# JuliaImageRecon/RegularizedLeastSquares.jl

Measured on AMD Instinct MI355X. Metric: CGNR iterations/sec @4096x2048 CF32; achieved HBM GB/s vs roofline, higher is better.
Workload: dtype c64 (ComplexF32 storage and arithmetic; scalar reductions accumulated in f64); 1 GPU; CGNR matrix-free normal operator, dense column-major ComplexF32 4096x2048, lambda=0, relTol=0, back-to-back solves of 32 iterations (BASELINE configs[1] shape, headline metric run of SURVEY 8d); M=4096, N=2048, problems_per_gpu=1, init_inside_region=True

## Files before the change

### regularizedleastsquares.jl_amd/csrc/api.hip

```cpp
#include "rls_common.hpp"

#include <cstdlib>
#include <map>
#include <mutex>
#include <set>
#include <vector>

namespace {
std::mutex g_mem_mutex;
std::map<const rls_ctx*, uint64_t> g_live_ctx;
uint64_t g_next_ctx_id = 1;
thread_local rls_ctx* tl_alloc_ctx = nullptr;

std::map<int, hipMemPool_t> g_pools;
hipMemPool_t device_pool(int device) {
  static std::mutex m;
  std::lock_guard<std::mutex> lk(m);
  auto it = g_pools.find(device);
  if (it != g_pools.end()) return it->second;
  hipMemPool_t pool = nullptr;
  const char* env = getenv("RLS_ALLOC");
  if (!(env && !strcmp(env, "sync"))) {
    int supported = 0;
    if (hipDeviceGetAttribute(&supported, hipDeviceAttributeMemoryPoolsSupported, device) == hipSuccess && supported) {
// ... 69 lines not shown
      __hip_atomic_store(A.dst[k] + i, A.src[k][i], __ATOMIC_RELAXED, __HIP_MEMORY_SCOPE_SYSTEM);
  rls_system_stores_done();
  if (threadIdx.x == 0) __hip_atomic_store(seq_h, seq, __ATOMIC_RELAXED, __HIP_MEMORY_SCOPE_SYSTEM);
}

int32_t rls_fetch_add(rls_ctx* ctx, const void* src_d, void* dst_pinned, size_t bytes) {
  if (!ctx->tune.status_mailbox || (bytes & 3) || ctx->nfq >= RLS_FETCH_MAX) {
    RLS_HIP(ctx, hipMemcpyAsync(dst_pinned, src_d, bytes, hipMemcpyDeviceToHost, ctx->stream));
    return 0;
  }
  ctx->fq[ctx->nfq++] = {src_d, dst_pinned, (unsigned)(bytes / 4)};
  return 0;
}

int32_t rls_fetch_wait(rls_ctx* ctx) {
  if (ctx->nfq == 0) {
    RLS_HIP(ctx, rls_stream_wait(ctx->stream));
    return 0;
  }
  fetch_args A;
  A.count = ctx->nfq;
  for (int k = 0; k < RLS_FETCH_MAX; ++k) {
    A.src[k] = k < ctx->nfq ? reinterpret_cast<const unsigned*>(ctx->fq[k].src) : nullptr;
    A.dst[k] = k < ctx->nfq ? reinterpret_cast<unsigned*>(ctx->fq[k].dst) : nullptr;
    A.n[k] = k < ctx->nfq ? ctx->fq[k].dwords : 0u;
  }
  ctx->nfq = 0;
  const unsigned seq = ++ctx->mb_seq;
  hipLaunchKernelGGL(mailbox_publish_kernel, dim3(1), dim3(64), 0, ctx->stream, A, ctx->mb_h, seq);
  RLS_HIP(ctx, hipGetLastError());
  return rls_mailbox_wait(ctx, seq);
}

rls_mailbox_slot rls_mailbox_arm(rls_ctx* ctx, void* dst_pinned) {
  rls_mailbox_slot mb;
  if (ctx->tune.status_mailbox < 2) return mb;
  mb.dst = dst_pinned;
  mb.seq_h = ctx->mb_h;
  mb.seq = ++ctx->mb_seq;
  return mb;
}

int32_t rls_mailbox_wait(rls_ctx* ctx, unsigned seq) {
  volatile unsigned* p = ctx->mb_h;
  const auto t0 = std::chrono::steady_clock::now();
  for (unsigned n = 0;; ++n) {
    if (*p == seq) {
      std::atomic_thread_fence(std::memory_order_acquire);
      return 0;
    }
    rls_cpu_relax();
    if ((n & 1023) == 1023 && std::chrono::steady_clock::now() - t0 > std::chrono::milliseconds(250)) break;
  }
  RLS_HIP(ctx, hipStreamSynchronize(ctx->stream));
  std::atomic_thread_fence(std::memory_order_acquire);
  return *p == seq ? 0 : rls_fail(ctx, RLS_E_STATE, "status mailbox: the publishing kernel did not run");
}

rls_alloc_scope::rls_alloc_scope(rls_ctx* ctx) : prev(tl_alloc_ctx) { tl_alloc_ctx = ctx; }
rls_alloc_scope::~rls_alloc_scope() { tl_alloc_ctx = prev; }
hipError_t rls_scoped_malloc(void** p, size_t bytes) { return rls_dev_alloc(tl_alloc_ctx, p, bytes); }
hipError_t rls_scoped_free(void* p) { return rls_dev_free(tl_alloc_ctx, p); }

static int32_t ctx_setup(rls_ctx* ctx) {
  RLS_HIP(ctx, hipEventCreate(&ctx->ev0));
  RLS_HIP(ctx, hipEventCreate(&ctx->ev1));
  RLS_HIP(ctx, hipMalloc((void**)&ctx->red_d, sizeof(double) * RLS_RED_SLOTS));
  RLS_HIP(ctx, hipMalloc((void**)&ctx->res_d, sizeof(float) * RLS_RES_FLOATS));
  RLS_HIP(ctx, hipHostMalloc((void**)&ctx->res_h, sizeof(float) * RLS_RES_FLOATS, hipHostMallocDefault));
  RLS_HIP(ctx, hipHostMalloc((void**)&ctx->mb_h, 64, hipHostMallocPortable | hipHostMallocMapped | hipHostMallocCoherent));
  ctx->mb_h[0] = 0;
  return 0;
}

static int32_t ctx_create_impl(int32_t device, void* stream, bool borrow, rls_ctx** out) {
  if (!out) return RLS_E_INVALID;
  *out = nullptr;
  int ndev = 0;
  hipError_t e = hipGetDeviceCount(&ndev);
  if (e != hipSuccess) return (int32_t)e;
  if (device < 0 || device >= ndev) return RLS_E_INVALID;
  e = hipSetDevice(device);
  if (e != hipSuccess) return (int32_t)e;
  rls_ctx* ctx = new rls_ctx();
  ctx->device = device;
  ctx->pools = device_pools_ok(device);
  if (borrow) {
    ctx->stream = (hipStream_t)stream;
    ctx->own_stream = false;
    ctx->tune.resident_server = 0;
  } else {
    e = hipStreamCreateWithFlags(&ctx->stream, hipStreamNonBlocking);
    if (e != hipSuccess) {
      delete ctx;
      return (int32_t)e;
    }
    ctx->own_stream = true;
  }
  int32_t st = ctx_setup(ctx);
  if (st != 0) {
    rls_ctx_destroy(ctx);
    return st;
  }
  {
    std::lock_guard<std::mutex> lk(g_mem_mutex);
    ctx->id = g_next_ctx_id++;
    g_live_ctx[ctx] = ctx->id;
  }
  *out = ctx;
  return 0;
}

extern "C" {

int32_t rls_abi_version(void) { return RLS_ABI_VERSION; }

int32_t rls_device_count(int32_t* out) {
  if (!out) return RLS_E_INVALID;
  int n = 0;
  hipError_t e = hipGetDeviceCount(&n);
  *out = (e == hipSuccess) ? n : 0;
  return (int32_t)e;
}

int32_t rls_ctx_create(int32_t device, rls_ctx** out) { return ctx_create_impl(device, nullptr, false, out); }
int32_t rls_ctx_create_on_stream(int32_t device, void* hip_stream, rls_ctx** out) {
  return ctx_create_impl(device, hip_stream, true, out);
}

int32_t rls_ctx_destroy(rls_ctx* ctx) {
  RLS_CHECK_CTX(ctx);
  {
    std::lock_guard<std::mutex> lk(g_mem_mutex);
    g_live_ctx.erase(ctx);
  }
  rls_enter(ctx);
  if (ctx->stream) rls_stream_wait(ctx->stream);
  rls_resident_forget(ctx->device, ctx->stream);
  if (ctx->ev0) hipEventDestroy(ctx->ev0);
  if (ctx->ev1) hipEventDestroy(ctx->ev1);
  if (ctx->red_d) hipFree(ctx->red_d);
  if (ctx->res_d) hipFree(ctx->res_d);
  if (ctx->res_h) hipHostFree(ctx->res_h);
  if (ctx->mb_h) hipHostFree(ctx->mb_h);
  if (ctx->own_stream && ctx->stream) hipStreamDestroy(ctx->stream);
  delete ctx;
  return 0;
}

int32_t rls_ctx_sync(rls_ctx* ctx) {
  RLS_CHECK_CTX(ctx);
  RLS_HIP(ctx, rls_enter(ctx));
  RLS_HIP(ctx, rls_stream_wait(ctx->stream));
  return 0;
}

void* rls_ctx_stream(rls_ctx* ctx) { return ctx ? (void*)ctx->stream : nullptr; }
const char* rls_last_error_string(rls_ctx* ctx) { return ctx ? ctx->err : "null context"; }

int32_t rls_tune_set(rls_ctx* ctx, const char* key, int32_t value) {
  RLS_CHECK_CTX(ctx);
  if (!key) return RLS_E_INVALID;
  if (ctx->server) rls_server_stop(ctx);
  ++ctx->tune_epoch;
  if (!strcmp(key, "gemvn_g")) ctx->tune.gemvn_g = value;
  else if (!strcmp(key, "gemvn_waves")) ctx->tune.gemvn_waves = value;
  else if (!strcmp(key, "gemvt_cols")) ctx->tune.gemvt_cols = value;
  else if (!strcmp(key, "gemvt_reverse")) ctx->tune.gemvt_reverse = value;
  else if (!strcmp(key, "graph_chunk")) ctx->tune.graph_chunk = value;
  else if (!strcmp(key, "use_graph")) ctx->tune.use_graph = value;
  else if (!strcmp(key, "fuse_level")) ctx->tune.fuse_level = value;
  else if (!strcmp(key, "fused_normal")) ctx->tune.fused_normal = value;
  else if (!strcmp(key, "cgnr_pipeline")) ctx->tune.cgnr_pipeline = value;
  else if (!strcmp(key, "batched_mfma")) ctx->tune.batched_mfma = value;
  else if (!strcmp(key, "gram_pipeline")) ctx->tune.gram_pipeline = value;
  else if (!strcmp(key, "pipe_hint_mode")) ctx->tune.pipe_hint_mode = value;
  else if (!strcmp(key, "resident")) {
    ctx->tune.resident = value;
    ctx->resident_failures = 0;
  }
  else if (!strcmp(key, "status_mailbox")) ctx->tune.status_mailbox = value;
  else if (!strcmp(key, "small")) ctx->tune.small = value;
  else if (!strcmp(key, "resident_server")) ctx->tune.resident_server = value;
  else if (!strcmp(key, "resident_ahead")) ctx->tune.resident_ahead = value ? 1 : 0;
  else if (!strcmp(key, "resident_l2_rows")) ctx->tune.resident_l2_rows = value;
  else if (!strcmp(key, "fista_defer")) ctx->tune.fista_defer = value;
  else if (!strcmp(key, "resident_server_idle_us")) {
    ctx->tune.resident_server_idle_us = value < 1 ? 1 : (value > 10000 ? 10000 : value);
  }
  else if (!strcmp(key, "resident_spin")) ctx->tune.resident_spin = value;
  else if (!strcmp(key, "resident_preclear")) ctx->tune.resident_preclear = value;
  else if (!strcmp(key, "skinny_t_waves")) ctx->tune.skinny_t_waves = value;
  else if (!strcmp(key, "skinny_v_waves")) ctx->tune.skinny_v_waves = value;
  else if (!strcmp(key, "skinny_v_splits")) ctx->tune.skinny_v_splits = value;
  else if (!strcmp(key, "kaczmarz_nt")) ctx->tune.kaczmarz_nt = value;
  else if (!strcmp(key, "skinny_t_u")) ctx->tune.skinny_t_u = value;
  else if (!strcmp(key, "skinny_v_u")) ctx->tune.skinny_v_u = value;
  else if (!strcmp(key, "skinny_half")) ctx->tune.skinny_half = value;
  else if (!strcmp(key, "skinny_t_roll")) ctx->tune.skinny_t_roll = value;
  else if (!strcmp(key, "skinny_v_roll")) ctx->tune.skinny_v_roll = value;
  else if (!strcmp(key, "skinny_g_roll")) ctx->tune.skinny_g_roll = value;
  else if (!strcmp(key, "gram_lds_kib")) ctx->tune.gram_lds = value * 1024;
  else if (!strcmp(key, "slab_g")) ctx->tune.slab_g = value;
  else if (!strcmp(key, "slab_wv")) {
    if (value != 0 && value != 8) return rls_fail(ctx, RLS_E_INVALID, "tune_set: slab_wv: only 8-wave slabs exist");
  }
  else if (!strcmp(key, "tv_fused_max_n")) ctx->tune.tv_fused_max_n = value;
  else if (!strcmp(key, "tv_fused_2d")) ctx->tune.tv_fused_2d = value;
  else if (!strcmp(key, "slab_order")) ctx->tune.slab_order = value;
  else if (!strcmp(key, "red_threads")) ctx->tune.red_threads = value;
  else if (!strcmp(key, "slab_multi")) ctx->tune.slab_multi = value ? 1 : 0;
  else if (!strcmp(key, "resident_barrier")) ctx->tune.resident_barrier = value == 1 ? 1 : 2;
  else return rls_fail(ctx, RLS_E_INVALID, "tune_set: unknown key");
  return 0;
}

int32_t rls_malloc(rls_ctx* ctx, size_t bytes, void** out) {
  RLS_CHECK_CTX(ctx);
  if (!out) return rls_fail(ctx, RLS_E_INVALID, "malloc: null out");
  *out = nullptr;
  if (bytes == 0) return 0;
  RLS_HIP(ctx, rls_enter(ctx));
  RLS_HIP(ctx, rls_dev_alloc(ctx, out, bytes));
  return 0;
}

int32_t rls_free(rls_ctx* ctx, void* p) {
  if (!p) return 0;
  if (!ctx_alive_by_address(ctx)) {
    const hipError_t e = hipFree(p);
    return e == hipSuccess ? 0 : (int32_t)e;
  }
  if (ctx->pools && ctx->server) {
    RLS_HIP(ctx, hipSetDevice(ctx->device));
    RLS_HIP(ctx, rls_dev_free(ctx, p));
    return 0;
  }
  RLS_HIP(ctx, rls_enter(ctx));
  if (!ctx->pools) RLS_HIP(ctx, rls_stream_wait(ctx->stream));
  RLS_HIP(ctx, rls_dev_free(ctx, p));
  return 0;
}

int32_t rls_memcpy_h2d(rls_ctx* ctx, void* dst, const void* src_h, size_t bytes) {
  RLS_CHECK_CTX(ctx);
  if (bytes == 0) return 0;
  if (!dst || !src_h) return rls_fail(ctx, RLS_E_INVALID, "memcpy_h2d: null pointer");
  RLS_HIP(ctx, rls_enter(ctx));
  RLS_HIP(ctx, hipMemcpyAsync(dst, src_h, bytes, hipMemcpyHostToDevice, ctx->stream));
  RLS_HIP(ctx, rls_stream_wait(ctx->stream));
  return 0;
}

int32_t rls_memcpy_d2h(rls_ctx* ctx, void* dst_h, const void* src, size_t bytes) {
  RLS_CHECK_CTX(ctx);
  if (bytes == 0) return 0;
  if (!dst_h || !src) return rls_fail(ctx, RLS_E_INVALID, "memcpy_d2h: null pointer");
  RLS_HIP(ctx, rls_enter(ctx));
  RLS_HIP(ctx, hipMemcpyAsync(dst_h, src, bytes, hipMemcpyDeviceToHost, ctx->stream));
  RLS_HIP(ctx, rls_stream_wait(ctx->stream));
  return 0;
}

int32_t rls_memcpy_d2d(rls_ctx* ctx, void* dst, const void* src, size_t bytes) {
  RLS_CHECK_CTX(ctx);
  if (bytes == 0) return 0;
  if (!dst || !src) return rls_fail(ctx, RLS_E_INVALID, "memcpy_d2d: null pointer");
  RLS_HIP(ctx, rls_enter(ctx));
  RLS_HIP(ctx, hipMemcpyAsync(dst, src, bytes, hipMemcpyDeviceToDevice, ctx->stream));
  return 0;
}

int32_t rls_timer_start(rls_ctx* ctx) {
  RLS_CHECK_CTX(ctx);
  RLS_HIP(ctx, rls_enter(ctx));
  RLS_HIP(ctx, hipEventRecord(ctx->ev0, ctx->stream));
  return 0;
}

int32_t rls_timer_stop_ms(rls_ctx* ctx, float* ms_out) {
  RLS_CHECK_CTX(ctx);
  if (!ms_out) return rls_fail(ctx, RLS_E_INVALID, "timer_stop: null out");
  RLS_HIP(ctx, rls_enter(ctx));
  RLS_HIP(ctx, hipEventRecord(ctx->ev1, ctx->stream));
  RLS_HIP(ctx, rls_event_wait(ctx->ev1));
  RLS_HIP(ctx, hipEventElapsedTime(ms_out, ctx->ev0, ctx->ev1));
  return 0;
}

int32_t rls_gemv(rls_ctx* ctx, int32_t dtype, int32_t op, int64_t M, int64_t N, float alpha_re, float alpha_im,
                 const void* A, int64_t lda, const void* x, float beta_re, float beta_im, void* y) {
  return rls_launch_gemv(ctx, dtype, op, M, N, alpha_re, alpha_im, A, lda, x, beta_re, beta_im, y, nullptr);
}

}
```

### regularizedleastsquares.jl_amd/csrc/normal.hip

```cpp
#include "rls_common.hpp"
#include "resident_sync.hpp"

#ifdef RLS_STAMPS
__device__ unsigned long long g_stamps[16 * 8];
#define STAMP(slot)                                                                         \
  do {                                                                                      \
    if (threadIdx.x == 0 && (blockIdx.x % 37) == 5 && blockIdx.x / 37 < 8)                  \
      g_stamps[(blockIdx.x / 37) * 16 + (slot)] = __builtin_amdgcn_s_memrealtime();         \
  } while (0)
#define STAMP_R(slot)                                                                    \
  do {                                                                                      \
    if (threadIdx.x == 0 && blockIdx.x == 0) g_stamps[7 * 16 + (slot)] = __builtin_amdgcn_s_memrealtime(); \
  } while (0)
#define STAMP_R_KEEP()                                                                    \
  do {                                                                                      \
    if (threadIdx.x == 0 && blockIdx.x == 5)                                                \
      for (int q = 0; q < 4; ++q) g_stamps[7 * 16 + 4 + q] = g_stamps[7 * 16 + q];          \
  } while (0)
#else
#define STAMP(slot) \
  do {              \
  } while (0)
#define STAMP_R(slot) \
  do {                \
// ... 1776 lines not shown
    constexpr int H = NVAL / 2;
    const bool up = lane & 8;
#pragma unroll
    for (int j = 0; j < H; ++j) {
      const float lo = v[j] + dpp_f(v[j], 0x140), hi = v[H + j] + dpp_f(v[H + j], 0x140);
      v[j] = up ? hi : lo;
    }
    idx += up ? H : 0;
  }
  {
    constexpr int H = NVAL / 4;
    const bool up = lane & 4;
#pragma unroll
    for (int j = 0; j < H; ++j) {
      const float lo = v[j] + dpp_f(v[j], 0x141), hi = v[H + j] + dpp_f(v[H + j], 0x141);
      v[j] = up ? hi : lo;
    }
    idx += up ? H : 0;
  }
  {
    constexpr int H = NVAL / 8;
    const bool up = lane & 2;
#pragma unroll
    for (int j = 0; j < H; ++j) {
      const float lo = v[j] + dpp_f(v[j], 0x4E), hi = v[H + j] + dpp_f(v[H + j], 0x4E);
      v[j] = up ? hi : lo;
    }
    idx += up ? H : 0;
  }
  {
    constexpr int H = NVAL / 16;
    const bool up = lane & 1;
#pragma unroll
    for (int j = 0; j < H; ++j) {
      const float lo = v[j] + dpp_f(v[j], 0xB1), hi = v[H + j] + dpp_f(v[H + j], 0xB1);
      v[j] = up ? hi : lo;
    }
    idx += up ? H : 0;
  }
  float r;
  if constexpr (NVAL == 32) {
    float a = v[0], b = v[1];
    permlane16_swap(a, b);
    r = a + b;
    idx += (lane & 16) ? 1 : 0;
  } else {
    float a = v[0], b = v[0];
    permlane16_swap(a, b);
    r = a + b;
  }
  {
    float a = r, b = r;
    permlane32_swap(a, b);
    r = a + b;
  }
  *idx_out = idx;
  return r;
}

template <typename E, int G, int K, int WV, bool FULL>
__device__ static inline void owner_products(const chunk<E, elem<E>::vec> (&a)[K], const E (&pin)[slab_cfg<E, G, K, WV>::EPT],
                                             float* red, __amdgpu_buffer_rsrc_t slab_rs, int64_t N, bool l2rows = false,
                                             const __amdgpu_buffer_rsrc_t* tt_rs = nullptr) {
  using C = slab_cfg<E, G, K, WV>;
  constexpr int NV = C::NV, EPT = C::EPT, NT = C::NT, RF = owner_cfg<E, G, K, WV>::RF;
  constexpr bool CX = elem<E>::cplx;
  const int tid = threadIdx.x, lane = tid & 63, w = tid >> 6;
  E acc[G * NV];
#pragma unroll
  for (int i = 0; i < G * NV; ++i) acc[i] = elem<E>::zero();
#pragma unroll
  for (int e = 0; e < EPT; ++e) {
    const int q = e / NV, j = e % NV;
#pragma unroll
    for (int i = 0; i < G; ++i)
#pragma unroll
      for (int r = 0; r < NV; ++r) acc[i * NV + r] = elem<E>::fma_pk(a[16 * q + j * G + i].e[r], pin[e], acc[i * NV + r]);
  }
  float v[RF];
#pragma unroll
  for (int i = 0; i < G * NV; ++i) {
    if constexpr (CX) {
      v[2 * i] = elem<E>::re(acc[i]);
      v[2 * i + 1] = elem<E>::im(acc[i]);
    } else {
      v[i] = elem<E>::re(acc[i]);
    }
  }
  int idx;
  const float part = wave_reduce_scatter<RF>(v, lane, &idx);
  if (lane < 32) red[w * RF + idx] = part;
  lds_barrier();
  const float* tw;
  float tsum = 0.f;
  if constexpr (FULL) {
    float* mine = red + (WV + w) * RF;
    if (lane < RF) {
      float sum = red[lane];
#pragma unroll
      for (int ww = 1; ww < WV; ++ww) sum += red[ww * RF + lane];
      mine[lane] = sum;
      tsum = sum;
    }
    __builtin_amdgcn_wave_barrier();
    tw = mine;
  } else {
    if (tid < RF) {
      float sum = red[tid];
#pragma unroll
      for (int ww = 1; ww < WV; ++ww) sum += red[ww * RF + tid];
      red[WV * RF + tid] = sum;
      tsum = sum;
    }
    lds_barrier();
    tw = red + WV * RF;
  }
  if (tt_rs) {
    if (w == 0) {
      const double sq = half_wave_sum((double)tsum * (double)tsum);
      if (lane == 0) {
        typedef unsigned u2 __attribute__((ext_vector_type(2)));
        if (l2rows) __builtin_amdgcn_raw_buffer_store_b64(__builtin_bit_cast(u2, sq), *tt_rs, (uint32_t)blockIdx.x * 8u, 0, 1);
        else __builtin_amdgcn_raw_buffer_store_b64(__builtin_bit_cast(u2, sq), *tt_rs, (uint32_t)blockIdx.x * 8u, 0, 16);
      }
    }
  }
  E tr[G * NV];
#pragma unroll
  for (int i = 0; i < G * NV; ++i) {
    if constexpr (CX) tr[i] = elem<E>::make(tw[2 * i], tw[2 * i + 1]);
    else tr[i] = elem<E>::make(tw[i], 0.f);
  }
#pragma unroll
  for (int q = 0; q < EPT / NV; ++q) {
    chunk<E, NV> out;
#pragma unroll
    for (int j = 0; j < NV; ++j) {
      E sum = elem<E>::zero();
#pragma unroll
      for (int i = 0; i < G; ++i)
#pragma unroll
        for (int r = 0; r < NV; ++r) sum = elem<E>::fmac_pk(a[16 * q + j * G + i].e[r], tr[i * NV + r], sum);
      out.e[j] = sum;
    }
    const int o = q * NT * NV + tid * NV;
    if (FULL || o < N) {
      const uint32_t off = (uint32_t)blockIdx.x * (uint32_t)(N * sizeof(E)) + (uint32_t)(o * sizeof(E));
      if (l2rows) __builtin_amdgcn_raw_buffer_store_b128(__builtin_bit_cast(u4, out), slab_rs, off, 0, 1);
      else __builtin_amdgcn_raw_buffer_store_b128(__builtin_bit_cast(u4, out), slab_rs, off, 0, 16);
    }
  }
}

__device__ static inline unsigned resident_xcc_id() {
  unsigned v;
  asm volatile("s_getreg_b32 %0, hwreg(HW_REG_XCC_ID)" : "=s"(v));
  return v & 0xfu;
}
__device__ static inline void resident_report_placement(resident_sync* sync) {
  if (threadIdx.x == 0 && resident_xcc_id() != (blockIdx.x % RES_GROUPS))
    __hip_atomic_store(&sync->gcnt[1], 1u, __ATOMIC_RELAXED, __HIP_MEMORY_SCOPE_AGENT);
}
__device__ static inline bool resident_rows_at_l2(resident_sync* sync) {
  return uni((int)__hip_atomic_load(&sync->gcnt[1], __ATOMIC_RELAXED, __HIP_MEMORY_SCOPE_AGENT)) == 0;
}

typedef unsigned u2v __attribute__((ext_vector_type(2)));
__device__ static inline double sc1_load_f64(__amdgpu_buffer_rsrc_t r, uint32_t byte_off) {
  return __builtin_bit_cast(double, __builtin_amdgcn_raw_buffer_load_b64(r, byte_off, 0, 16));
}
template <typename E, int G, int K, int WV, int EXCH, bool FULL, bool DPPSUM = true, bool SCAL = false, typename PC, typename PUB>
__device__ static inline bool resident_allreduce(resident_lds<E, G, K, WV>& R, resident_sync* sync,
                                                 __amdgpu_buffer_rsrc_t slab_rs, E* v, int nwg, int64_t N, unsigned& epoch,
                                                 unsigned& xchg, unsigned spin_limit,
                                                 E (&vv)[slab_cfg<E, G, K, WV>::EPT], PC&& per_column, PUB&& publish,
                                                 const __amdgpu_buffer_rsrc_t* d_rs = nullptr, double* tt = nullptr) {
  using C = slab_cfg<E, G, K, WV>;
  constexpr int NV = C::NV, EPT = C::EPT, NT = C::NT;
  const int tid = threadIdx.x;
  if constexpr (EXCH == 1) {
    if (!grid_arrive_wait(sync->cnt, ++epoch, (unsigned)nwg, spin_limit, &R.flag)) return false;
    STAMP(11);
    if constexpr (SCAL) {
      if ((tid >> 6) == WV - 1) {
        const int lane = tid & 63;
        double s = 0.0;
        for (int row = lane; row < nwg; row += 64) s += sc1_load_f64(*d_rs, (uint32_t)row * 8u);
        s = wave_sum(s);
        if (lane == 0) R.tt = s;
      }
    }
    resident_reduce_chunks<E, G, K, WV, FULL>(R, slab_rs, v, nwg, N, per_column);
    publish();
    asm volatile("s_waitcnt vmcnt(0)" ::: "memory");
    __syncthreads();
    STAMP(12);
    if (!grid_arrive_wait(sync->cnt, ++epoch, (unsigned)nwg, spin_limit, &R.flag)) return false;
    STAMP(13);
    const __amdgpu_buffer_rsrc_t v_rs = sc1_rsrc(v);
#pragma unroll
    for (int q = 0; q < EPT / NV; ++q) {
      const int o = q * NT * NV + tid * NV;
      const bool ok = FULL || o < N;
      const chunk<E, NV> c = __builtin_bit_cast(chunk<E, NV>, sc1_load16(v_rs, (uint32_t)((ok ? o : 0) * sizeof(E))));
#pragma unroll
      for (int j = 0; j < NV; ++j) vv[q * NV + j] = ok ? c.e[j] : elem<E>::zero();
    }
    if constexpr (SCAL) *tt = R.tt;
    return true;
  } else {
    const unsigned per = (unsigned)nwg / RES_GROUPS, grp = blockIdx.x % RES_GROUPS, mem = blockIdx.x / RES_GROUPS;
    const uint32_t rowb = (uint32_t)(N * sizeof(E));
    const unsigned q = (rowb / 16u) / per;
    const unsigned lq = (unsigned)__builtin_ctz(q), nrg = (unsigned)NT >> lq;
    const unsigned par = xchg & 1u;
    ++xchg;
    char* xpart = reinterpret_cast<char*>(sync) + sizeof(resident_sync) + (size_t)par * RES_GROUPS * rowb;
    const __amdgpu_buffer_rsrc_t xp_rs = sc1_rsrc(xpart);
    if (!group_arrive_wait(sync->gcnt + grp * 32, per * xchg, spin_limit, &R.flag)) return false;
    STAMP(11);
    const uint32_t gs_off = (2u - par) * RES_GROUPS * rowb + par * (RES_GROUPS * 8u);
    if constexpr (SCAL) {
      if (mem == 0u && tid < 64) {
        double s = (unsigned)tid < per ? sc1_load_f64(*d_rs, (grp + RES_GROUPS * (unsigned)tid) * 8u) : 0.0;
        s = half_wave_sum(s);
        if (tid == 0) __builtin_amdgcn_raw_buffer_store_b64(__builtin_bit_cast(u2v, s), xp_rs, gs_off + grp * 8u, 0, 16);
      }
    }
    if (DPPSUM && nrg == 16u && q == 32u && per == 32u) {
      const unsigned lane = (unsigned)tid & 63u, rg = lane & 15u, piece = 4u * ((unsigned)tid >> 6) + (lane >> 4);
      const uint32_t col = (mem * 32u + piece) * 16u;
      const f4 ta = sc1_load16(slab_rs, (grp + RES_GROUPS * rg) * rowb + col);
      const f4 tb = sc1_load16(slab_rs, (grp + RES_GROUPS * (rg + 16u)) * rowb + col);
      f4 acc = ta + tb;
#pragma unroll
      for (int c = 0; c < 4; ++c) {
        float v = acc[c];
        v += dpp_f(v, 0xB1);
        v += dpp_f(v, 0x4E);
        v += dpp_f(v, 0x141);
        v += dpp_f(v, 0x140);
        acc[c] = v;
      }
      if (rg == 0u) __builtin_amdgcn_raw_buffer_store_b128(__builtin_bit_cast(u4, acc), xp_rs, grp * rowb + (mem * 32u + piece) * 16u, 0, 16);
      asm volatile("s_waitcnt vmcnt(0)" ::: "memory");
      __syncthreads();
    } else {
      const unsigned piece = (unsigned)tid & (q - 1u), rg = (unsigned)tid >> lq;
      const uint32_t col = (mem * q + piece) * 16u;
      f4 acc = {0.f, 0.f, 0.f, 0.f};
      for (unsigned row = rg; row < per; row += 2u * nrg) {
        const unsigned rb = row + nrg;
        const f4 ta = sc1_load16(slab_rs, (grp + RES_GROUPS * row) * rowb + col);
        const f4 tb = sc1_load16(slab_rs, (grp + RES_GROUPS * (rb < per ? rb : row)) * rowb + col);
        acc += ta;
        if (rb < per) acc += tb;
      }
      f4* ex = reinterpret_cast<f4*>(&R.L.xg[0][0]);
      ex[tid] = acc;
      __syncthreads();
      if ((unsigned)tid < q) {
        f4 sum = ex[tid];
        for (unsigned g = 1; g < nrg; ++g) sum += ex[(g << lq) + tid];
        __builtin_amdgcn_raw_buffer_store_b128(__builtin_bit_cast(u4, sum), xp_rs, grp * rowb + (mem * q + (unsigned)tid) * 16u, 0, 16);
      }
      asm volatile("s_waitcnt vmcnt(0)" ::: "memory");
      if (q > 64u) __syncthreads();
    }
    STAMP(12);
    if (!grid_arrive_wait(sync->cnt, ++epoch, (unsigned)nwg, spin_limit, &R.flag)) return false;
    STAMP(13);
    if constexpr (SCAL) {
      double s = sc1_load_f64(xp_rs, gs_off + ((unsigned)tid & 7u) * 8u);
      s += dpp_d(s, 0xB1);
      s += dpp_d(s, 0x4E);
      s += dpp_d(s, 0x141);
      *tt = s;
    }
#pragma unroll
    for (int qq = 0; qq < EPT / NV; ++qq) {
      const int o = qq * NT * NV + tid * NV;
      const bool ok = FULL || o < N;
      const uint32_t off = (uint32_t)((ok ? o : 0) * sizeof(E));
      f4 t[RES_GROUPS];
#pragma unroll
      for (int g = 0; g < RES_GROUPS; ++g) t[g] = sc1_load16(xp_rs, (uint32_t)g * rowb + off);
      f4 sum = t[0];
#pragma unroll
      for (int g = 1; g < RES_GROUPS; ++g) sum += t[g];
      const chunk<E, NV> c = __builtin_bit_cast(chunk<E, NV>, sum);
#pragma unroll
      for (int j = 0; j < NV; ++j) vv[qq * NV + j] = ok ? c.e[j] : elem<E>::zero();
    }
    return true;
  }
}

template <typename E, int G, int K, int WV, int BAR, bool FULL, bool SPEC = false>
__global__ __launch_bounds__(WV * 64) void cgnr_resident_kernel(const E* __restrict__ A, int64_t lda, E* x, E* xw, E* r, E* p,
                                                                 E* v, E* slab, double* dout, cgnr_scalars* sc,
                                                                 resident_sync* sync, int64_t Mc, int64_t N, int pair,
                                                                 int n_steps, unsigned spin_limit, rls_cg_start St) {
  using C = slab_cfg<E, G, K, WV>;
  constexpr int NV = C::NV, EPT = C::EPT, NT = C::NT;
  static_assert(EPT % NV == 0, "16-byte ownership layout");
  extern __shared__ __attribute__((aligned(16))) char smem_raw[];
  resident_lds<E, G, K, WV>& R = *reinterpret_cast<resident_lds<E, G, K, WV>*>(smem_raw);
  slab_lds<E, G, K, WV>& L = R.L;
  const int tid = threadIdx.x;
  const int nwg = gridDim.x;
  STAMP(0);
  if (St.enabled && St.skip && *St.skip) {
    if (blockIdx.x == 0 && tid == 0) {
      cgnr_scalars Z = *sc;
      Z.iteration = 0;
      Z.max_iter = St.maxiter;
      Z.pending = 0;
      Z.cur = 0;
      Z.fresh = 0;
      Z.done = 1;
      *sc = Z;
      sync->completed = 1u;
    }
    return;
  }
  cgnr_scalars S = *sc;
  E pv[EPT], rv[EPT], xv[EPT];
  if constexpr (FULL) {
    load_owned_wide<E, EPT, NT>(pv, p, tid);
    load_owned_wide<E, EPT, NT>(rv, r, tid);
    load_owned_wide<E, EPT, NT>(xv, x, tid);
  } else {
    load_owned_wide_masked<E, EPT, NT>(pv, p, tid, N);
    load_owned_wide_masked<E, EPT, NT>(rv, r, tid, N);
    load_owned_wide_masked<E, EPT, NT>(xv, x, tid, N);
  }
  asm volatile("s_waitcnt vmcnt(0)" ::: "memory");
  __builtin_amdgcn_sched_barrier(0);
  chunk<E, NV> a[K];
  slab_load<E, G, K, WV, FULL>(a, A, lda, Mc, N, pair);
  __builtin_amdgcn_sched_barrier(0);
  if (!St.enabled && (S.done || n_steps <= 0)) return;
  constexpr bool OWN = owner_cfg<E, G, K, WV>::ok;
  if constexpr (OWN) owner_transpose<E, G, K, WV, FULL>(a, smem_raw, Mc, N, pair);
  STAMP(1);
  const __amdgpu_buffer_rsrc_t slab_rs = sc1_rsrc(slab), d_rs = sc1_rsrc(dout);
  unsigned epoch = 0, xchg = 0;
  bool alive = true;
  constexpr bool L2ROWS = BAR == 2 && OWN;
  bool l2rows = false, placed = !L2ROWS;
  if constexpr (L2ROWS) resident_report_placement(sync);
  if (St.enabled) {
    if constexpr (OWN) {
      owner_products<E, G, K, WV, FULL>(a, xv, R.ored, slab_rs, N);
    } else {
#pragma unroll
      for (int e = 0; e < EPT; ++e) L.xs[(int)own_index<E, EPT, NT, true>(tid, e)] = xv[e];
      slab_finish<E, G, K, WV, FULL, true>(a, L, slab, Mc, N, pair);
    }
    asm volatile("s_waitcnt vmcnt(0)" ::: "memory");
    __syncthreads();
    E cv[EPT];
    if (!resident_allreduce<E, G, K, WV, BAR, FULL>(R, sync, slab_rs, v, nwg, N, epoch, xchg, spin_limit, cv, [](int, E) {}, []() {})) {
      resident_give_up(sync, St.enabled ? St.poison : nullptr);
      return;
    }
    if (!placed) {
      l2rows = resident_rows_at_l2(sync);
      placed = true;
    }
    double rr = 0.0;
#pragma unroll
    for (int q = 0; q < EPT / NV; ++q) {
      const int o = q * NT * NV + tid * NV;
      const bool ok = FULL || o < N;
      const int oc = ok ? o : 0;
      chunk<E, NV> cc;
#pragma unroll
      for (int j = 0; j < NV; ++j) cc.e[j] = cv[q * NV + j];
      chunk<E, NV> bi;
      if (St.beta_y) {
        bi = load_chunk<E, NV>(reinterpret_cast<const E*>(St.beta_y) + oc);
        const chunk<E, NV> zc = load_chunk<E, NV>(reinterpret_cast<const E*>(St.z) + oc);
#pragma unroll
        for (int j = 0; j < NV; ++j) bi.e[j] = elem<E>::add(bi.e[j], elem<E>::scale(St.rho_admm, zc.e[j]));
        const chunk<E, NV> uc = load_chunk<E, NV>(reinterpret_cast<const E*>(St.u) + oc);
#pragma unroll
        for (int j = 0; j < NV; ++j) bi.e[j] = elem<E>::add(bi.e[j], elem<E>::scale(-St.rho_admm, uc.e[j]));
        if (blockIdx.x == 0 && ok) {
          chunk<E, NV> xc;
#pragma unroll
          for (int j = 0; j < NV; ++j) xc.e[j] = xv[q * NV + j];
          *reinterpret_cast<f4*>(reinterpret_cast<E*>(St.beta) + o) = __builtin_bit_cast(f4, bi);
          *reinterpret_cast<f4*>(reinterpret_cast<E*>(St.xold) + o) = __builtin_bit_cast(f4, xc);
        }
      } else {
        bi = load_chunk<E, NV>(reinterpret_cast<const E*>(St.b) + oc);
      }
#pragma unroll
      for (int j = 0; j < NV; ++j) {
        const E ci = elem<E>::add(cc.e[j], elem<E>::scale(St.rho, xv[q * NV + j]));
        E ri = elem<E>::sub(bi.e[j], ci);
        if (!ok) ri = elem<E>::zero();
        rv[q * NV + j] = ri;
        pv[q * NV + j] = ri;
        rr += (double)elem<E>::re(ri) * (double)elem<E>::re(ri) + (double)elem<E>::im(ri) * (double)elem<E>::im(ri);
      }
    }
    rr = block_sum_n<NT / 64>(rr, L.red);
    S.rr = rr;
    S.z0 = sqrt(rr);
    S.zeta = 0.0;
    S.alpha_re = S.alpha_im = S.beta_re = S.beta_im = 0.0;
    S.lambda = St.rho;
    S.rel_tol = St.reltol;
    S.iteration = 0;
    S.max_iter = St.maxiter;
    S.pending = 0;
    S.cur = 0;
    S.fresh = 0;
    S.done = (St.maxiter <= 0) || (rr == 0.0) || (1.0f <= St.reltol);
    if (S.done) n_steps = 0;
  }
  auto store_owned = [&](E* dst, const E (&src)[EPT]) {
#pragma unroll
    for (int q = 0; q < EPT / NV; ++q) {
      chunk<E, NV> c;
#pragma unroll
      for (int j = 0; j < NV; ++j) c.e[j] = src[q * NV + j];
      const int64_t o = (int64_t)q * (NT * NV) + (int64_t)tid * NV;
      if (FULL || o < N) *reinterpret_cast<f4*>(dst + o) = __builtin_bit_cast(f4, c);
    }
  };
  const __amdgpu_buffer_rsrc_t xw_rs = sc1_rsrc(xw);
  auto load_owned_sc1 = [&](E (&dst)[EPT], const E*) {
#pragma unroll
    for (int q = 0; q < EPT / NV; ++q) {
      const int o = q * NT * NV + tid * NV;
      const bool ok = FULL || o < N;
      const chunk<E, NV> c = __builtin_bit_cast(chunk<E, NV>, sc1_load16(xw_rs, (uint32_t)((ok ? o : 0) * sizeof(E))));
#pragma unroll
      for (int j = 0; j < NV; ++j) dst[q * NV + j] = ok ? c.e[j] : elem<E>::zero();
    }
  };
  if (blockIdx.x == 0) store_owned(xw, xv);
  rls_mailbox_slot srv_mb = St.srv_mb;
  unsigned srv_seq = St.srv_seq0;
  int credit = 0;
  bool ahead = false;
  STAMP(2);
  for (;;) {
  for (int it = SPEC ? credit : 0; it < n_steps; ++it) {
    if (S.done) break;
    STAMP(8);
#ifdef RLS_STAMPS
    if (it == 1) STAMP(5);
    if (it == 2) STAMP(6);
    if (it == 10) STAMP(7);
#endif
    if constexpr (OWN) {
      owner_products<E, G, K, WV, FULL>(a, pv, R.ored, slab_rs, N, l2rows, &d_rs);
    } else {
#pragma unroll
      for (int e = 0; e < EPT; ++e) L.xs[(int)own_index<E, EPT, NT, true>(tid, e)] = pv[e];
      const double ttw = slab_finish<E, G, K, WV, FULL, true, true>(a, L, slab, Mc, N, pair);
      if (tid == 0) __builtin_amdgcn_raw_buffer_store_b64(__builtin_bit_cast(u2v, ttw), d_rs, (uint32_t)blockIdx.x * 8u, 0, 16);
    }
    STAMP(9);
    double pp = 0.0;
    if (S.lambda > 0.f) {
      if constexpr (!OWN) {
#pragma unroll
        for (int e = 0; e < EPT; ++e) pv[e] = L.xs[(int)own_index<E, EPT, NT, true>(tid, e)];
      }
#pragma unroll
      for (int e = 0; e < EPT; ++e)
        pp += (double)elem<E>::re(pv[e]) * (double)elem<E>::re(pv[e]) + (double)elem<E>::im(pv[e]) * (double)elem<E>::im(pv[e]);
      pp = block_sum_nolead<NT / 64, 0>(pp, L.red);
    }
    asm volatile("s_waitcnt vmcnt(0)" ::: "memory");
    __syncthreads();
    STAMP(10);
    E xq[EPT];
    load_owned_sc1(xq, xw);
    E vv[EPT];
    double tt = 0.0;
    const bool ok_x = resident_allreduce<E, G, K, WV, BAR, FULL, true, true>(R, sync, slab_rs, v, nwg, N, epoch, xchg, spin_limit, vv,
                                                                             [](int, E) {}, []() {}, &d_rs, &tt);
    if (!ok_x) {
      alive = false;
      break;
    }
    if (!placed) {
      l2rows = resident_rows_at_l2(sync);
      placed = true;
    }
    if constexpr (!OWN) {
#pragma unroll
      for (int e = 0; e < EPT; ++e) pv[e] = L.xs[(int)own_index<E, EPT, NT, true>(tid, e)];
    }
    E pn[EPT], rn[EPT];
    float al;
    cgnr_scalars Sn;
#ifdef RLS_STAMPS
    asm volatile("s_waitcnt vmcnt(0)" ::: "memory");
    STAMP(14);
#endif
    const bool done = cg_update_elems_tt<E, EPT, NT, true>(S, tt, pp, pv, rv, vv, N, L.red, pn, rn, al, Sn);
#pragma unroll
    for (int e = 0; e < EPT; ++e) {
      xq[e] = elem<E>::make(fmaf(elem<E>::re(pv[e]), al, elem<E>::re(xq[e])), fmaf(elem<E>::im(pv[e]), al, elem<E>::im(xq[e])));
      rv[e] = rn[e];
      pv[e] = pn[e];
    }
    if (blockIdx.x == 0) {
#pragma unroll
      for (int q = 0; q < EPT / NV; ++q) {
        chunk<E, NV> c;
#pragma unroll
        for (int j = 0; j < NV; ++j) c.e[j] = xq[q * NV + j];
        const int o = q * NT * NV + tid * NV;
        if (FULL || o < N) __builtin_amdgcn_raw_buffer_store_b128(__builtin_bit_cast(u4, c), xw_rs, (uint32_t)(o * sizeof(E)), 0, 0);
      }
    }
    S = Sn;
    RLS_CGNR_UNIFORM(S);
    STAMP(15);
    if (done) break;
  }
  STAMP(3);
  if (!alive) {
    resident_give_up(sync, St.enabled ? St.poison : nullptr);
    if (St.srv_ctl && blockIdx.x == 0 && tid == 0) __hip_atomic_store(St.srv_ctl + 17, 2u, __ATOMIC_RELAXED, __HIP_MEMORY_SCOPE_SYSTEM);
    return;
  }
  if constexpr (SPEC) {
    if (ahead) {
      ahead = false;
      const unsigned cmd = resident_listen(St.srv_ctl, srv_seq, St.srv_idle_us, sync, epoch, (unsigned)nwg, spin_limit, &R.flag, srv_mb, srv_seq - St.srv_seq0 + 1u);
      if (cmd == RLS_SRV_EXIT) return;
      n_steps = (int)cmd;
      credit = 1;
      continue;
    }
  }
  if (blockIdx.x == 0) {
    S.pending = 0;
    S.cur = 0;
    S.fresh = 0;
    if (St.srv_ctl && tid < 64) rls_mailbox_publish(srv_mb, S, tid);
    E xf[EPT];
    load_owned_sc1(xf, xw);
    auto store_buf = [&](E* dst, const E (&src)[EPT]) {
      const __amdgpu_buffer_rsrc_t rs = __builtin_amdgcn_make_buffer_rsrc(dst, 0, 0xffffffff, 0x00020000);
#pragma unroll
      for (int q = 0; q < EPT / NV; ++q) {
        chunk<E, NV> c;
#pragma unroll
        for (int j = 0; j < NV; ++j) c.e[j] = src[q * NV + j];
        const int o = q * NT * NV + tid * NV;
        if (FULL || o < N) __builtin_amdgcn_raw_buffer_store_b128(__builtin_bit_cast(u4, c), rs, (uint32_t)(o * sizeof(E)), 0, 0);
      }
    };
    store_buf(x, xf);
    store_buf(r, rv);
    store_buf(p, pv);
    if (tid == 0) {
      *sc = S;
      sync->completed = 1u;
    }
  }
  if (!St.srv_ctl) break;
  if constexpr (SPEC) {
    credit = 0;
    if (!S.done) {
      ahead = true;
      n_steps = 1;
      continue;
    }
  }
  const unsigned cmd = resident_listen(St.srv_ctl, srv_seq, St.srv_idle_us, sync, epoch, (unsigned)nwg, spin_limit, &R.flag, srv_mb, srv_seq - St.srv_seq0 + 1u);
  if (cmd == RLS_SRV_EXIT) return;
  n_steps = (int)cmd;
  }
}


template <typename E, int K, int BAR, bool FULL, int SRV = 0>
__global__ __launch_bounds__(512) void cgnr_gram_resident_kernel(const E* __restrict__ Gm, int64_t ldg, E* x, E* r, E* p,
                                                                  E* v0, E* v1, double* dots, cgnr_scalars* sc0,
                                                                  cgnr_scalars* sc1, resident_sync* sync, int64_t Mc,
                                                                  int64_t N, int pair, int n_steps, unsigned spin_limit,
                                                                  rls_cg_start St) {
  constexpr int G = 4, WV = 8;
  using C = slab_cfg<E, G, K, WV>;
  constexpr int NV = C::NV, EPT = C::EPT, NT = C::NT;
  __shared__ gram_lds<E, G, K, WV> L;
  __shared__ int flag;
  const int tid = threadIdx.x, lane = tid & 63, w = tid >> 6;
  const int nwg = gridDim.x;
  if (St.enabled && St.skip && *St.skip) {
    if (blockIdx.x == 0 && tid == 0) {
      cgnr_scalars Z = *sc0;
      Z.iteration = 0;
      Z.max_iter = St.maxiter;
      Z.pending = 0;
      Z.cur = 0;
      Z.fresh = 0;
      Z.done = 1;
      *sc0 = Z;
      *sc1 = Z;
      sync->completed = 1u;
    }
    return;
  }
  cgnr_scalars S = *sc0;
  E pv[EPT], rv[EPT], xv[EPT], vv[EPT];
#pragma unroll
  for (int e = 0; e < EPT; ++e) {
    const int64_t i = tid + (int64_t)e * NT;
    const int64_t ic = FULL || i < N ? i : (N - 1);
    pv[e] = p[ic];
    rv[e] = r[ic];
    xv[e] = x[ic];
    vv[e] = elem<E>::zero();
    if (!FULL && i >= N) pv[e] = rv[e] = xv[e] = elem<E>::zero();
  }
  asm volatile("s_waitcnt vmcnt(0)" ::: "memory");
  __builtin_amdgcn_sched_barrier(0);
  chunk<E, NV> a[K];
  slab_load<E, G, K, WV, FULL>(a, Gm, ldg, Mc, N, pair);
  __builtin_amdgcn_sched_barrier(0);
  if (!St.enabled && (S.done || n_steps <= 0)) return;
  const __amdgpu_buffer_rsrc_t d_rs = sc1_rsrc(dots);
  unsigned epoch = 0;
  bool alive = true;
  if (St.enabled) {
#pragma unroll
    for (int e = 0; e < EPT; ++e) L.xs[tid + e * NT] = xv[e];
    gram_rows<E, G, K, WV, FULL>(a, L, Mc, N, pair);
    if (tid < G * NV) {
      const int gg = tid / NV, i = tid % NV;
      E sum = elem<E>::zero();
#pragma unroll
      for (int ww = 0; ww < WV; ++ww) sum = elem<E>::add(sum, L.part[ww][gg][i]);
      const int64_t row = (row_block_of(blockIdx.x, pair) * G + gg) * NV + i;
      if (FULL || row < N) sc1_store_elem<E>(v1 + row, sum);
    }
    asm volatile("s_waitcnt vmcnt(0)" ::: "memory");
    __syncthreads();
    if (!grid_arrive_wait(sync->cnt, ++epoch, (unsigned)nwg, spin_limit, &flag)) {
      resident_give_up(sync, St.enabled ? St.poison : nullptr);
      return;
    }
    const E* bb = reinterpret_cast<const E*>(St.b);
    const E* by = reinterpret_cast<const E*>(St.beta_y);
    const E* zz = reinterpret_cast<const E*>(St.z);
    const E* uu = reinterpret_cast<const E*>(St.u);
    double rr = 0.0;
#pragma unroll
    for (int e = 0; e < EPT; ++e) {
      const int64_t i = tid + (int64_t)e * NT;
      const bool ok = FULL || i < N;
      const int64_t ic = ok ? i : (N - 1);
      const E ci = elem<E>::add(sc1_load_elem<E>(v1 + ic), elem<E>::scale(St.rho, xv[e]));
      E bi;
      if (by) {
        bi = by[ic];
        bi = elem<E>::add(bi, elem<E>::scale(St.rho_admm, zz[ic]));
        bi = elem<E>::add(bi, elem<E>::scale(-St.rho_admm, uu[ic]));
        if (blockIdx.x == 0 && ok) {
          reinterpret_cast<E*>(St.beta)[i] = bi;
          reinterpret_cast<E*>(St.xold)[i] = xv[e];
        }
      } else {
        bi = bb[ic];
      }
      E ri = elem<E>::sub(bi, ci);
      if (!ok) ri = elem<E>::zero();
      rv[e] = ri;
      pv[e] = ri;
      rr += (double)elem<E>::re(ri) * (double)elem<E>::re(ri) + (double)elem<E>::im(ri) * (double)elem<E>::im(ri);
    }
    rr = block_sum_n<NT / 64>(rr, L.red);
    S.rr = rr;
    S.z0 = sqrt(rr);
    S.zeta = 0.0;
    S.alpha_re = S.alpha_im = S.beta_re = S.beta_im = 0.0;
    S.lambda = St.rho;
    S.rel_tol = St.reltol;
    S.iteration = 0;
    S.max_iter = St.maxiter;
    S.pending = 0;
    S.cur = 0;
    S.fresh = 0;
    S.done = (St.maxiter <= 0) || (rr == 0.0) || (1.0f <= St.reltol);
    if (S.done) n_steps = 0;
  }
  rls_mailbox_slot srv_mb = St.srv_mb;
  unsigned srv_seq = St.srv_seq0;
  unsigned itg = 0;
  int credit = 0;
  bool ahead = false;
  for (;;) {
  for (int it = SRV ? credit : 0; it < n_steps; ++it) {
    if (SRV && S.done) break;
    const int q = (int)(itg++ & 1u);
    E* vq = q ? v1 : v0;
#pragma unroll
    for (int e = 0; e < EPT; ++e) L.xs[tid + e * NT] = pv[e];
    gram_rows<E, G, K, WV, FULL>(a, L, Mc, N, pair);
    double dre = 0.0, dim_ = 0.0, pp = 0.0;
    if (tid < G * NV) {
      const int gg = tid / NV, i = tid % NV;
      E sum = elem<E>::zero();
#pragma unroll
      for (int ww = 0; ww < WV; ++ww) sum = elem<E>::add(sum, L.part[ww][gg][i]);
      const int64_t row = (row_block_of(blockIdx.x, pair) * G + gg) * NV + i;
      if (FULL || row < N) {
        sc1_store_elem<E>(vq + row, sum);
        const E pj = L.xs[row];
        dre = (double)elem<E>::re(pj) * (double)elem<E>::re(sum) + (double)elem<E>::im(pj) * (double)elem<E>::im(sum);
        dim_ = (double)elem<E>::re(pj) * (double)elem<E>::im(sum) - (double)elem<E>::im(pj) * (double)elem<E>::re(sum);
        pp = (double)elem<E>::re(pj) * (double)elem<E>::re(pj) + (double)elem<E>::im(pj) * (double)elem<E>::im(pj);
      }
    }
    if (w == 0) {
#pragma unroll
      for (int off = 8; off > 0; off >>= 1) {
        dre += __shfl_xor(dre, off, 64);
        dim_ += __shfl_xor(dim_, off, 64);
        pp += __shfl_xor(pp, off, 64);
      }
      if (lane < 3) {
        const double dv = lane == 0 ? dre : (lane == 1 ? dim_ : pp);
        __hip_atomic_store(reinterpret_cast<unsigned long long*>(dots + (size_t)q * 4 * nwg + 4 * blockIdx.x + lane),
                           __builtin_bit_cast(unsigned long long, dv), __ATOMIC_RELAXED, __HIP_MEMORY_SCOPE_AGENT);
      }
    }
// ... 984 lines not shown
    });
  });
}

template <typename E>
static int32_t fista_iteration_typed(rls_ctx* ctx, const rls_fista_pipe& P) {
  fused_cfg c;
  if (!pick_cfg<E>(ctx->tune, P.N, &c)) return rls_fail(ctx, RLS_E_UNSUPPORTED, "fista pipeline: N too large");
  const int nwg = (int)fused_nwg<E>(ctx->tune, P.M, P.N);
  const int rows = slab_grid(ctx, c.K, nwg);
  RLS_TRY(with_cfg(c, [&](auto S) { return launch_fista_a<E, S.G, S.K, S.WV>(ctx, P, nwg, rows); }));
  hipLaunchKernelGGL(fista_pipe_r_kernel<E>, dim3((unsigned)((P.N + 15) / 16)), dim3(ctx->tune.red_threads), 0, ctx->stream,
                     (const E*)P.slab, rows, P.N, (E*)P.res_raw, P.sc, P.scn);
  return launch_status(ctx);
}

template <typename E>
static int32_t fista_finish_typed(rls_ctx* ctx, const rls_fista_pipe& P) {
  return with_ept(P.N, [&](auto EPT) {
    return rls_launch<fista_pipe_f_kernel<E, EPT>>(ctx, dim3(1), dim3(FIN_THREADS), 0, (E*)P.b0, (E*)P.b1, (const E*)P.x0,
                                                   (E*)P.res, (E*)P.y0, (E*)P.y1, (const E*)P.res_raw, P.sc, P.N, P.mb);
  });
}

template <typename E>
static bool gram_pick(int64_t N, int* K) {
  const int64_t cpr = 8 * (64 / 4);
  for (int k : {8, 16, 32}) {
    if (N <= k * cpr) {
      *K = k;
      return true;
    }
  }
  return false;
}

template <typename E>
static int gram_grid(rls_ctx* ctx, int K, int nwg) {
  return elem<E>::cplx ? slab_grid(ctx, K, nwg) : nwg;
}

template <typename E, int K>
constexpr bool gram_walks() {
  return K == 32 && elem<E>::cplx;
}

template <typename E, int K>
static int32_t launch_gram(rls_ctx* ctx, const rls_gram_pipe& P, int q, int nwg) {
  using C = slab_cfg<E, 4, K, 8>;
  const int64_t Mc = P.N / C::NV;
  const int pair = slab_pairing(4, nwg);
  const int grid = gram_grid<E>(ctx, K, nwg);
  return with_bool(slab_full<E, 4, K, 8>(P.N, P.N, nwg), [&](auto FULL) {
    return with_bool(gram_walks<E, K>() && grid < nwg, [&](auto MULTI) {
      if constexpr (MULTI && !gram_walks<E, K>())
        return not_instantiated(ctx);
      else
        return rls_launch<cgnr_gram_kernel<E, 4, K, 8, FULL, MULTI>>(
            ctx, dim3(MULTI ? grid : nwg), dim3(C::NT), 0, (const E*)P.G, P.ldg, (E*)P.x, (const E*)P.r[q], (const E*)P.p[q],
            (E*)P.r[q ^ 1], (E*)P.p[q ^ 1], (const E*)P.v[q], (E*)P.v[q ^ 1], P.dots + (size_t)q * 4 * nwg,
            P.dots + (size_t)(q ^ 1) * 4 * nwg, MULTI ? grid : nwg, P.sc[q], P.sc[q ^ 1], Mc, P.N, pair, ctx->tune.slab_order, nwg);
    });
  });
}

template <typename E>
static int32_t gram_iteration_typed(rls_ctx* ctx, const rls_gram_pipe& P, int q) {
  int K = 0;
  if (!gram_pick<E>(P.N, &K)) return rls_fail(ctx, RLS_E_UNSUPPORTED, "gram pipeline: N too large");
  const int nwg = rls_gram_pipe_nwg(elem<E>::cplx ? RLS_C32 : RLS_F32, P.N);
  return rls_with<8, 16, 32>(K, [&](auto KC) { return launch_gram<E, KC>(ctx, P, q, nwg); });
}

template <typename E>
static int32_t gram_finish_typed(rls_ctx* ctx, const rls_gram_pipe& P, int q) {
  const int nwg = rls_gram_pipe_nwg(elem<E>::cplx ? RLS_C32 : RLS_F32, P.N);
  int Kp = 0;
  gram_pick<E>(P.N, &Kp);
  const int ndots = gram_grid<E>(ctx, Kp, nwg);
  return with_ept(P.N, [&](auto EPT) {
    return rls_launch<cgnr_gram_f_kernel<E, EPT>>(ctx, dim3(1), dim3(FIN_THREADS), 0, (E*)P.x, (const E*)P.r[q], (const E*)P.p[q],
                                                  (E*)P.r[0], (E*)P.p[0], (const E*)P.v[q], (E*)P.v[0], P.dots + (size_t)q * 4 * nwg,
                                                  ndots, P.sc[q], P.sc[0], P.sc[1], P.N);
  });
}

template <typename E, int K>
static int32_t launch_fista_gram(rls_ctx* ctx, const rls_fista_gram& P, int q, int nwg) {
  using C = slab_cfg<E, 4, K, 8>;
  const int64_t Mc = P.N / C::NV;
  const int pair = slab_pairing(4, nwg);
  const int grid = gram_grid<E>(ctx, K, nwg);
  return with_bool(slab_full<E, 4, K, 8>(P.N, P.N, nwg), [&](auto FULL) {
    return with_bool(P.par_hint >= 0, [&](auto HINT) {
      return with_bool(gram_walks<E, K>() && grid < nwg, [&](auto MULTI) {
        if constexpr (MULTI && !gram_walks<E, K>())
          return not_instantiated(ctx);
        else
          return rls_launch<fista_gram_kernel<E, 4, K, 8, FULL, HINT, MULTI>>(
              ctx, dim3(MULTI ? grid : nwg), dim3(C::NT), 0, (const E*)P.G, P.ldg, (E*)P.b0, (E*)P.b1, (const E*)P.x0, (E*)P.res,
              (E*)P.y0, (E*)P.y1, (const E*)P.rr[q], (E*)P.rr[q ^ 1], P.sc[q], P.sc[q ^ 1], Mc, P.N, pair, P.par_hint, nwg);
      });
    });
  });
}

template <typename E>
static int32_t fista_gram_iteration_typed(rls_ctx* ctx, const rls_fista_gram& P, int q) {
  int K = 0;
  if (!gram_pick<E>(P.N, &K)) return rls_fail(ctx, RLS_E_UNSUPPORTED, "gram pipeline: N too large");
  const int nwg = rls_gram_pipe_nwg(elem<E>::cplx ? RLS_C32 : RLS_F32, P.N);
  return rls_with<8, 16, 32>(K, [&](auto KC) { return launch_fista_gram<E, KC>(ctx, P, q, nwg); });
}

template <typename E>
static int32_t fista_gram_finish_typed(rls_ctx* ctx, const rls_fista_gram& P, int q) {
  return with_ept(P.N, [&](auto EPT) {
    return rls_launch<fista_gram_f_kernel<E, EPT>>(ctx, dim3(1), dim3(FIN_THREADS), 0, (E*)P.b0, (E*)P.b1, (const E*)P.x0,
                                                   (E*)P.res, (E*)P.y0, (E*)P.y1, (const E*)P.rr[q], P.sc[q], P.sc[0], P.sc[1], P.N);
  });
}


template <typename E>
static bool resident_two_level_ok(const rls_tuning& T, int nwg, int64_t N, int nt) {
  if (T.resident_barrier != 2 || nwg % RES_GROUPS != 0) return false;
  const int64_t pieces = N * (int64_t)sizeof(E) / 16, per = nwg / RES_GROUPS;
  if (N * (int64_t)sizeof(E) % 16 != 0 || pieces % per != 0) return false;
  const int64_t q = pieces / per;
  return q >= 1 && q <= nt && (q & (q - 1)) == 0;
}

template <typename E, int G, int K, int WV>
constexpr bool resident_shape() {
  return (K == 32 || K == 16) && WV == 8 && slab_cfg<E, G, K, WV>::EPT % elem<E>::vec == 0 && !(elem<E>::cplx && G == 4);
}
template <typename E, int G, int K, int WV>
constexpr bool pgm_resident_shape() {
  return resident_shape<E, G, K, WV>() && owner_cfg_ok<E, G, K, WV>();
}

static int resident_pairing(int G, int nwg) { return (G == 4 && nwg % 16 == 0) ? 1 : 0; }

template <typename E, int G, int K, int WV>
static int32_t launch_resident(rls_ctx* ctx, const rls_cgnr_pipe& P, double* dout, void* sync, int nwg, int n_steps,
                               unsigned spin_limit, const rls_cg_start& St) {
  if constexpr (!resident_shape<E, G, K, WV>()) {
    return rls_fail(ctx, RLS_E_UNSUPPORTED, "resident CGNR: slab shape not instantiated");
  } else {
    using C = slab_cfg<E, G, K, WV>;
    const int64_t Mc = P.M / C::NV;
    const int pair = resident_pairing(G, nwg);
    constexpr size_t lds = resident_lds_bytes<E, G, K, WV>();
    const bool spec = St.srv_ctl != nullptr && ctx->tune.resident_ahead != 0;
    return with_bool(resident_two_level_ok<E>(ctx->tune, nwg, P.N, C::NT), [&](auto TWO) {
      return with_bool(slab_full<E, G, K, WV>(P.M, P.N, nwg), [&](auto FULL) {
        return with_bool(spec, [&](auto SPEC) {
          return rls_launch<cgnr_resident_kernel<E, G, K, WV, TWO ? 2 : 1, FULL, SPEC>>(
              ctx, dim3(nwg), dim3(C::NT), lds, (const E*)P.A, P.lda, (E*)P.x, (E*)P.r1, (E*)P.r0, (E*)P.p0, (E*)P.v, (E*)P.slab,
              dout, P.sc, (resident_sync*)sync, Mc, P.N, pair, n_steps, spin_limit, St);
        });
      });
    });
  }
}

template <typename E>
static bool resident_ok_typed(const rls_tuning& T, int device, int64_t M, int64_t N, const void* A, int64_t lda) {
  if (!fused_ok<E>(T, M, N, A, lda)) return false;
  fused_cfg c;
  if (!pick_cfg<E>(T, N, &c)) return false;
  return with_cfg(c, [&](auto S) {
    if constexpr (!resident_shape<E, S.G, S.K, S.WV>()) {
      return false;
    } else {
      const int64_t nwg = fused_nwg<E>(T, M, N);
      if (N % elem<E>::vec) return false;
      int cus = 0;
      if (hipDeviceGetAttribute(&cus, hipDeviceAttributeMultiprocessorCount, device) != hipSuccess) return false;
      if (!(nwg <= cus && nwg <= 256 && nwg * N * (int64_t)sizeof(E) < (int64_t)0xffffffffll)) return false;
      return rls_occupancy<cgnr_resident_kernel<E, S.G, S.K, S.WV, 1, false>>(device, S.WV * 64,
                                                                              resident_lds_bytes<E, S.G, S.K, S.WV>()) >= 1;
    }
  });
}

template <typename E>
static int32_t resident_typed(rls_ctx* ctx, const rls_cgnr_pipe& P, double* dout, void* sync, int n_steps,
                              unsigned spin_limit, const rls_cg_start& St) {
  fused_cfg c;
  if (!pick_cfg<E>(ctx->tune, P.N, &c)) return rls_fail(ctx, RLS_E_UNSUPPORTED, "resident CGNR: N too large");
  const int nwg = (int)fused_nwg<E>(ctx->tune, P.M, P.N);
  return with_cfg(c, [&](auto S) {
    return launch_resident<E, S.G, S.K, S.WV>(ctx, P, dout, sync, nwg, n_steps, spin_limit, St);
  });
}

template <typename E, int G, int K, int WV>
static int32_t launch_fista_resident(rls_ctx* ctx, const rls_fista_pipe& P, void* sync, int nwg, int n_steps,
                                     unsigned spin_limit, const rls_srv_args& Sv) {
  if constexpr (!resident_shape<E, G, K, WV>()) {
    return rls_fail(ctx, RLS_E_UNSUPPORTED, "resident FISTA: slab shape not instantiated");
  } else {
    using C = slab_cfg<E, G, K, WV>;
    const int64_t Mc = P.M / C::NV;
    const int pair = resident_pairing(G, nwg);
    constexpr size_t lds = resident_lds_bytes<E, G, K, WV>();
    const bool spec = Sv.ctl != nullptr && ctx->tune.resident_ahead != 0;
    return with_bool(resident_two_level_ok<E>(ctx->tune, nwg, P.N, C::NT), [&](auto TWO) {
      return with_bool(slab_full<E, G, K, WV>(P.M, P.N, nwg), [&](auto FULL) {
        return with_bool(spec, [&](auto SPEC) {
          return rls_launch<fista_resident_kernel<E, G, K, WV, TWO ? 2 : 1, FULL, SPEC>>(
              ctx, dim3(nwg), dim3(C::NT), lds, (const E*)P.A, P.lda, (E*)P.b0, (E*)P.b1, (const E*)P.x0, (E*)P.res, (E*)P.y0,
              (E*)P.y1, (E*)P.res_raw, (E*)P.slab, P.sc, (resident_sync*)sync, Mc, P.N, pair | (ctx->tune.fista_defer ? 0 : 2),
              n_steps, spin_limit, Sv);
        });
      });
    });
  }
}

template <typename E>
static int32_t fista_resident_typed(rls_ctx* ctx, const rls_fista_pipe& P, void* sync, int n_steps, unsigned spin_limit,
                                    const rls_srv_args& Sv) {
  fused_cfg c;
  if (!pick_cfg<E>(ctx->tune, P.N, &c)) return rls_fail(ctx, RLS_E_UNSUPPORTED, "resident FISTA: N too large");
  const int nwg = (int)fused_nwg<E>(ctx->tune, P.M, P.N);
  return with_cfg(c, [&](auto S) {
    return launch_fista_resident<E, S.G, S.K, S.WV>(ctx, P, sync, nwg, n_steps, spin_limit, Sv);
  });
}

static int gram_srv_mode(const rls_ctx* ctx, bool listens) { return !listens ? 0 : ctx->tune.resident_ahead ? 2 : 1; }

template <typename E, int K>
static int32_t launch_gram_resident(rls_ctx* ctx, const rls_gram_pipe& P, void* sync, int nwg, int n_steps,
                                    unsigned spin_limit, const rls_cg_start& St) {
  using C = slab_cfg<E, 4, K, 8>;
  const int64_t Mc = P.N / C::NV;
  const int pair = resident_pairing(4, nwg);
  return with_bool(slab_full<E, 4, K, 8>(P.N, P.N, nwg), [&](auto FULL) {
    return rls_with<0, 1, 2>(gram_srv_mode(ctx, St.srv_ctl != nullptr), [&](auto SRV) {
      if constexpr (K == 32 && SRV != 0)
        return rls_fail(ctx, RLS_E_UNSUPPORTED, "resident Gram CGNR: no listening instantiation for this shape");
      else
        return rls_launch<cgnr_gram_resident_kernel<E, K, 1, FULL, SRV>>(
            ctx, dim3(nwg), dim3(C::NT), 0, (const E*)P.G, P.ldg, (E*)P.x, (E*)P.r[0], (E*)P.p[0], (E*)P.v[0], (E*)P.v[1], P.dots,
            P.sc[0], P.sc[1], (resident_sync*)sync, Mc, P.N, pair, n_steps, spin_limit, St);
    });
  });
}

template <typename E>
static bool gram_resident_ok_typed(int device, int64_t N) {
  int K = 0;
  if (!gram_pick<E>(N, &K)) return false;
  const int nwg = rls_gram_pipe_nwg(elem<E>::cplx ? RLS_C32 : RLS_F32, N);
  int cus = 0;
  if (hipDeviceGetAttribute(&cus, hipDeviceAttributeMultiprocessorCount, device) != hipSuccess) return false;
  if (!(nwg <= cus && nwg <= 256)) return false;
  return rls_with<8, 16, 32>(K, [&](auto KC) {
    if constexpr (elem<E>::cplx && KC == 32)
      return false;
    else
      return rls_occupancy<cgnr_gram_resident_kernel<E, KC, 1, false>>(device, 512, 0) >= 1;
  });
}

template <typename E>
static int32_t gram_resident_typed(rls_ctx* ctx, const rls_gram_pipe& P, void* sync, int n_steps, unsigned spin_limit,
                                   const rls_cg_start& St) {
  int K = 0;
  if (!gram_pick<E>(P.N, &K)) return rls_fail(ctx, RLS_E_UNSUPPORTED, "resident Gram CGNR: N too large");
  const int nwg = rls_gram_pipe_nwg(elem<E>::cplx ? RLS_C32 : RLS_F32, P.N);
  return rls_with<8, 16, 32>(K, [&](auto KC) {
    if constexpr (elem<E>::cplx && KC == 32)
      return rls_fail(ctx, RLS_E_UNSUPPORTED, "resident Gram CGNR: shape not resident");
    else
      return launch_gram_resident<E, KC>(ctx, P, sync, nwg, n_steps, spin_limit, St);
  });
}

template <typename E, int K>
static int32_t launch_fista_gram_resident(rls_ctx* ctx, const rls_fista_gram& P, void* sync, int nwg, int n_steps,
                                          unsigned spin_limit, const rls_srv_args& Sv) {
  using C = slab_cfg<E, 4, K, 8>;
  const int64_t Mc = P.N / C::NV;
  const int pair = resident_pairing(4, nwg);
  return with_bool(slab_full<E, 4, K, 8>(P.N, P.N, nwg), [&](auto FULL) {
    return rls_with<0, 1, 2>(gram_srv_mode(ctx, Sv.ctl != nullptr), [&](auto SRV) {
      if constexpr (K == 32 && SRV != 0)
        return rls_fail(ctx, RLS_E_UNSUPPORTED, "resident Gram FISTA: no listening instantiation for this shape");
      else
        return rls_launch<fista_gram_resident_kernel<E, K, 1, FULL, SRV>>(
            ctx, dim3(nwg), dim3(C::NT), 0, (const E*)P.G, P.ldg, (E*)P.b0, (E*)P.b1, (const E*)P.x0, (E*)P.res, (E*)P.y0,
            (E*)P.y1, (E*)P.rr[0], (E*)P.rr[1], P.sc[0], P.sc[1], (resident_sync*)sync, Mc, P.N, pair, n_steps, spin_limit, Sv);
    });
  });
}

template <typename E>
static int32_t fista_gram_resident_typed(rls_ctx* ctx, const rls_fista_gram& P, void* sync, int n_steps,
                                         unsigned spin_limit, const rls_srv_args& Sv) {
  int K = 0;
  if (!gram_pick<E>(P.N, &K)) return rls_fail(ctx, RLS_E_UNSUPPORTED, "resident Gram FISTA: N too large");
  const int nwg = rls_gram_pipe_nwg(elem<E>::cplx ? RLS_C32 : RLS_F32, P.N);
// ... 14 lines not shown
    using C = slab_cfg<E, G, K, WV>;
    const int64_t Mc = D.M / C::NV;
    const int pair = resident_pairing(G, nwg);
    constexpr size_t lds = resident_lds_bytes<E, G, K, WV>();
    return with_bool(resident_two_level_ok<E>(ctx->tune, nwg, D.N, C::NT), [&](auto TWO) {
      return with_bool(slab_full<E, G, K, WV>(D.M, D.N, nwg), [&](auto FULL) {
        return rls_with<0, 1, 2>(D.kind, [&](auto KIND) {
          return rls_launch<pgm_resident_kernel<E, G, K, WV, TWO ? 2 : 1, FULL, KIND>>(
              ctx, dim3(nwg), dim3(C::NT), lds, (const E*)D.A, D.lda, (E*)D.v0, (E*)D.v1, (E*)D.v2, (E*)D.v3, (E*)D.o0, (E*)D.res,
              (const E*)D.x0, (E*)D.raw, (E*)D.slab, D.st, CF, D.norm_x0, D.rel_tol, D.reg_kind, D.proj_kind, (resident_sync*)sync,
              Mc, D.N, pair | (ctx->tune.fista_defer ? 0 : 2), n_steps, D.first_it, spin_limit);
        });
      });
    });
  }
}

template <typename E>
static int32_t pgm_resident_typed(rls_ctx* ctx, const rls_pgm_desc& D, const rls_pgm_coefs& CF, void* sync, int n_steps,
                                  unsigned spin_limit) {
  fused_cfg c;
  if (!pick_cfg<E>(ctx->tune, D.N, &c)) return rls_fail(ctx, RLS_E_UNSUPPORTED, "resident OptISTA / POGM: N too large");
  const int nwg = (int)fused_nwg<E>(ctx->tune, D.M, D.N);
  return with_cfg(c, [&](auto S) { return launch_pgm_resident<E, S.G, S.K, S.WV>(ctx, D, CF, sync, nwg, n_steps, spin_limit); });
}

template <typename E>
static bool pgm_resident_ok_typed(const rls_tuning& T, int device, int64_t M, int64_t N, const void* A, int64_t lda) {
  if (!resident_ok_typed<E>(T, device, M, N, A, lda)) return false;
  fused_cfg c;
  if (!pick_cfg<E>(T, N, &c)) return false;
  return with_cfg(c, [](auto S) { return pgm_resident_shape<E, S.G, S.K, S.WV>(); });
}
}

int32_t rls_fista_gram_iteration(rls_ctx* ctx, int32_t dtype, const rls_fista_gram& P, int parity) {
  if (dtype == RLS_F32) return fista_gram_iteration_typed<float>(ctx, P, parity & 1);
  return fista_gram_iteration_typed<float2>(ctx, P, parity & 1);
}
int32_t rls_fista_gram_finish(rls_ctx* ctx, int32_t dtype, const rls_fista_gram& P, int parity) {
  if (dtype == RLS_F32) return fista_gram_finish_typed<float>(ctx, P, parity & 1);
  return fista_gram_finish_typed<float2>(ctx, P, parity & 1);
}

int rls_gram_pipe_nwg(int32_t dtype, int64_t N) {
  const int V = dtype == RLS_C32 ? 2 : 4;
  const int64_t Mc = N / V;
  return (int)((Mc + 3) / 4);
}
bool rls_gram_pipe_ok(int32_t dtype, int64_t N, const void* G, int64_t ldg) {
  const int V = dtype == RLS_C32 ? 2 : 4;
  if (!G || N <= 0 || N % V || ldg % V || (reinterpret_cast<uintptr_t>(G) % 16)) return false;
  if (N > 32 * 128 || N > 4 * FIN_THREADS) return false;
  if (rls_gram_pipe_nwg(dtype, N) > 512) return false;
  return 128 * ldg * (int64_t)(dtype == RLS_C32 ? 8 : 4) + (N / V) * 16 < (int64_t)0xffffffffll;
}
int32_t rls_gram_pipe_iteration(rls_ctx* ctx, int32_t dtype, const rls_gram_pipe& P, int parity) {
  if (dtype == RLS_F32) return gram_iteration_typed<float>(ctx, P, parity & 1);
  return gram_iteration_typed<float2>(ctx, P, parity & 1);
}
int32_t rls_gram_pipe_finish(rls_ctx* ctx, int32_t dtype, const rls_gram_pipe& P, int parity) {
  if (dtype == RLS_F32) return gram_finish_typed<float>(ctx, P, parity & 1);
  return gram_finish_typed<float2>(ctx, P, parity & 1);
}

int32_t rls_fista_gram_resident_launch(rls_ctx* ctx, int32_t dtype, const rls_fista_gram& P, void* sync, int n_steps,
                                       unsigned spin_limit, const rls_srv_args& Sv) {
  if (dtype == RLS_F32) return fista_gram_resident_typed<float>(ctx, P, sync, n_steps, spin_limit, Sv);
  return fista_gram_resident_typed<float2>(ctx, P, sync, n_steps, spin_limit, Sv);
}
bool rls_gram_resident_ok(rls_ctx* ctx, int32_t dtype, int64_t N, const void* G, int64_t ldg) {
  if (!rls_gram_pipe_ok(dtype, N, G, ldg)) return false;
  return dtype == RLS_F32 ? gram_resident_ok_typed<float>(ctx->device, N) : gram_resident_ok_typed<float2>(ctx->device, N);
}
bool rls_gram_resident_server_ok(int32_t dtype, int64_t N) {
  int K = 0;
  const bool ok = dtype == RLS_F32 ? gram_pick<float>(N, &K) : gram_pick<float2>(N, &K);
  return ok && K != 32;
}
int32_t rls_gram_resident_launch(rls_ctx* ctx, int32_t dtype, const rls_gram_pipe& P, void* sync, int n_steps,
                                 unsigned spin_limit, const rls_cg_start& St) {
  if (dtype == RLS_F32) return gram_resident_typed<float>(ctx, P, sync, n_steps, spin_limit, St);
  return gram_resident_typed<float2>(ctx, P, sync, n_steps, spin_limit, St);
}


int32_t rls_fista_pipe_iteration(rls_ctx* ctx, int32_t dtype, const rls_fista_pipe& P) {
  if (dtype == RLS_F32) return fista_iteration_typed<float>(ctx, P);
  return fista_iteration_typed<float2>(ctx, P);
}
int32_t rls_fista_pipe_finish(rls_ctx* ctx, int32_t dtype, const rls_fista_pipe& P) {
  if (dtype == RLS_F32) return fista_finish_typed<float>(ctx, P);
  return fista_finish_typed<float2>(ctx, P);
}

#ifdef RLS_STAMPS
extern "C" int32_t rls_debug_stamps(unsigned long long* out_h) {
  return (int32_t)hipMemcpyFromSymbol(out_h, HIP_SYMBOL(g_stamps), sizeof(unsigned long long) * 16 * 8);
}
#endif

int32_t rls_cgnr_pipe_iteration(rls_ctx* ctx, int32_t dtype, const rls_cgnr_pipe& P) {
  if (dtype == RLS_F32) return pipe_iteration_typed<float>(ctx, P);
  return pipe_iteration_typed<float2>(ctx, P);
}
int32_t rls_cgnr_pipe_launch(rls_ctx* ctx, int32_t dtype, const rls_cgnr_pipe& P, int which) {
  if (dtype == RLS_F32) return pipe_iteration_typed<float>(ctx, P, which);
  return pipe_iteration_typed<float2>(ctx, P, which);
}
int32_t rls_cgnr_pipe_finish(rls_ctx* ctx, int32_t dtype, const rls_cgnr_pipe& P) {
  if (dtype == RLS_F32) return pipe_finish_typed<float>(ctx, P);
  return pipe_finish_typed<float2>(ctx, P);
}

size_t rls_normal_fused_workspace(rls_ctx* ctx, int32_t dtype, int64_t M, int64_t N, const void* A, int64_t lda) {
  if (!ctx) return 0;
  if (dtype == RLS_F32) return fused_ok<float>(ctx->tune, M, N, A, lda) ? (size_t)fused_nwg<float>(ctx->tune, M, N) * N * 4 : 0;
  if (dtype == RLS_C32) return fused_ok<float2>(ctx->tune, M, N, A, lda) ? (size_t)fused_nwg<float2>(ctx->tune, M, N) * N * 8 : 0;
  return 0;
}

int32_t rls_launch_normal_fused(rls_ctx* ctx, int32_t dtype, int64_t M, int64_t N, const void* A, int64_t lda,
                                const void* p, void* v, void* slab, const int* skip) {
  RLS_CHECK_CTX(ctx);
  if (!A || !p || !v || !slab) return rls_fail(ctx, RLS_E_INVALID, "normal_fused: null pointer");
  RLS_HIP(ctx, rls_enter(ctx));
  if (dtype == RLS_F32)
    return normal_typed<float>(ctx, M, N, (const float*)A, lda, (const float*)p, (float*)v, (float*)slab, skip);
  return normal_typed<float2>(ctx, M, N, (const float2*)A, lda, (const float2*)p, (float2*)v, (float2*)slab, skip);
}

size_t rls_cgnr_resident_sync_bytes() { return sizeof(resident_sync); }
size_t rls_resident_sync_alloc_bytes(int32_t dtype, int64_t N) {
  return sizeof(resident_sync) + (size_t)2 * RES_GROUPS * (size_t)N * rls_elem_size(dtype) + (size_t)2 * RES_GROUPS * sizeof(double);
}
size_t rls_resident_sync_clear_bytes() { return offsetof(resident_sync, failed); }
size_t rls_resident_sync_flags_offset() { return offsetof(resident_sync, fail); }
size_t rls_resident_sync_placement_offset() { return offsetof(resident_sync, gcnt) + sizeof(unsigned); }
bool rls_cgnr_resident_ok(rls_ctx* ctx, int32_t dtype, int64_t M, int64_t N, const void* A, int64_t lda) {
  if (!ctx) return false;
  if (dtype == RLS_F32) return resident_ok_typed<float>(ctx->tune, ctx->device, M, N, A, lda);
  if (dtype == RLS_C32) return resident_ok_typed<float2>(ctx->tune, ctx->device, M, N, A, lda);
  return false;
}
int rls_cgnr_resident_nwg(rls_ctx* ctx, int32_t dtype, int64_t M, int64_t N) {
  return dtype == RLS_F32 ? (int)fused_nwg<float>(ctx->tune, M, N) : (int)fused_nwg<float2>(ctx->tune, M, N);
}
int32_t rls_cgnr_resident_launch(rls_ctx* ctx, int32_t dtype, const rls_cgnr_pipe& P, double* dout, void* sync,
                                 int n_steps, unsigned spin_limit, const rls_cg_start& St) {
  if (dtype == RLS_F32) return resident_typed<float>(ctx, P, dout, sync, n_steps, spin_limit, St);
  return resident_typed<float2>(ctx, P, dout, sync, n_steps, spin_limit, St);
}

int32_t rls_fista_resident_launch(rls_ctx* ctx, int32_t dtype, const rls_fista_pipe& P, void* sync, int n_steps,
                                  unsigned spin_limit, const rls_srv_args& Sv) {
  if (dtype == RLS_F32) return fista_resident_typed<float>(ctx, P, sync, n_steps, spin_limit, Sv);
  return fista_resident_typed<float2>(ctx, P, sync, n_steps, spin_limit, Sv);
}

bool rls_pgm_resident_ok(rls_ctx* ctx, int32_t dtype, int64_t M, int64_t N, const void* A, int64_t lda) {
  if (!ctx) return false;
  if (dtype == RLS_F32) return pgm_resident_ok_typed<float>(ctx->tune, ctx->device, M, N, A, lda);
  if (dtype == RLS_C32) return pgm_resident_ok_typed<float2>(ctx->tune, ctx->device, M, N, A, lda);
  return false;
}
int32_t rls_pgm_resident_launch(rls_ctx* ctx, int32_t dtype, const rls_pgm_desc& D, const rls_pgm_coefs& C, void* sync,
                                int n_steps, unsigned spin_limit) {
  if (n_steps > RLS_PGM_MAX_IT) return rls_fail(ctx, RLS_E_INVALID, "pgm_resident: more iterations than coefficient slots");
  if (dtype == RLS_F32) return pgm_resident_typed<float>(ctx, D, C, sync, n_steps, spin_limit);
  return pgm_resident_typed<float2>(ctx, D, C, sync, n_steps, spin_limit);
}
```

### regularizedleastsquares.jl_amd/csrc/resident_sync.hpp

```cpp
#pragma once
#include "rls_common.hpp"

typedef unsigned u4 __attribute__((ext_vector_type(4)));
__device__ static inline __amdgpu_buffer_rsrc_t sc1_rsrc(const void* base) {
  return __builtin_amdgcn_make_buffer_rsrc(const_cast<void*>(base), 0, 0xffffffff, 0x00020000);
}
__device__ static inline f4 sc1_load16(__amdgpu_buffer_rsrc_t r, uint32_t byte_off) {
  return __builtin_bit_cast(f4, __builtin_amdgcn_raw_buffer_load_b128(r, byte_off, 0, 16));
}
template <typename E>
__device__ static inline void sc1_store_elem(E* p, E v) {
  if constexpr (sizeof(E) == 8)
    __hip_atomic_store(reinterpret_cast<unsigned long long*>(p), __builtin_bit_cast(unsigned long long, v), __ATOMIC_RELAXED,
                       __HIP_MEMORY_SCOPE_AGENT);
  else
    __hip_atomic_store(reinterpret_cast<unsigned*>(p), __builtin_bit_cast(unsigned, v), __ATOMIC_RELAXED,
                       __HIP_MEMORY_SCOPE_AGENT);
}


template <typename E>
__device__ static inline E sc1_load_elem(const E* p) {
  if constexpr (sizeof(E) == 8)
    return __builtin_bit_cast(E, __hip_atomic_load(reinterpret_cast<const unsigned long long*>(p), __ATOMIC_RELAXED,
                                                   __HIP_MEMORY_SCOPE_AGENT));
  else
    return __builtin_bit_cast(E, __hip_atomic_load(reinterpret_cast<const unsigned*>(p), __ATOMIC_RELAXED,
                                                   __HIP_MEMORY_SCOPE_AGENT));
}


struct resident_sync {
  unsigned cnt[8 * 32];
  unsigned gcnt[8 * 32];
  unsigned fail;
  unsigned completed;
  unsigned failed;
  unsigned srv_n, srv_mb;
  unsigned pad[27];
};
static_assert(sizeof(resident_sync) == (2 * 8 * 32 + 32) * sizeof(unsigned), "resident_sync layout");
constexpr int RES_GROUPS = 8;

__device__ static inline void resident_give_up(resident_sync* sync, int* poison) {
  if (threadIdx.x == 0) {
    __hip_atomic_store(&sync->fail, 1u, __ATOMIC_RELAXED, __HIP_MEMORY_SCOPE_AGENT);
    if (blockIdx.x == 0) {
      __hip_atomic_fetch_add(&sync->failed, 1u, __ATOMIC_RELAXED, __HIP_MEMORY_SCOPE_AGENT);
      if (poison) __hip_atomic_store(poison, 2, __ATOMIC_RELAXED, __HIP_MEMORY_SCOPE_AGENT);
    }
  }
}


#ifndef RLS_POLL_SLEEP
#define RLS_POLL_SLEEP 1
#endif
__device__ static inline bool grid_arrive_wait_t(unsigned* cnt, unsigned epoch, unsigned nwg, unsigned spin_limit, int* lds_flag,
                                                 const int tid) {
  if (tid < 64) {
    int ok = 0;
    const unsigned target = nwg * epoch;
    if (tid == 0) __hip_atomic_fetch_add(cnt + (blockIdx.x & 7) * 32, 1u, __ATOMIC_RELAXED, __HIP_MEMORY_SCOPE_AGENT);
    for (unsigned spins = 0; spins < spin_limit; ++spins) {
      unsigned c = __hip_atomic_load(cnt + (tid & 7) * 32, __ATOMIC_RELAXED, __HIP_MEMORY_SCOPE_AGENT);
      c += (unsigned)__builtin_amdgcn_update_dpp(0, (int)c, 0xB1, 0xF, 0xF, true);
      c += (unsigned)__builtin_amdgcn_update_dpp(0, (int)c, 0x4E, 0xF, 0xF, true);
      c += (unsigned)__builtin_amdgcn_update_dpp(0, (int)c, 0x141, 0xF, 0xF, true);
      if (__builtin_amdgcn_readfirstlane((int)c) >= (int)target) {
        ok = 1;
        break;
      }
      __builtin_amdgcn_s_sleep(RLS_POLL_SLEEP);
    }
    if (tid == 0) *lds_flag = ok;
  }
  __syncthreads();
  return *lds_flag != 0;
}
__device__ static inline bool grid_arrive_wait(unsigned* cnt, unsigned epoch, unsigned nwg, unsigned spin_limit, int* lds_flag) {
  return grid_arrive_wait_t(cnt, epoch, nwg, spin_limit, lds_flag, (int)threadIdx.x);
}
__device__ static inline bool group_arrive_wait(unsigned* word, unsigned target, unsigned spin_limit, int* lds_flag) {
  const int tid = threadIdx.x;
  if (tid < 64) {
    int ok = 0;
    if (tid == 0) __hip_atomic_fetch_add(word, 1u, __ATOMIC_RELAXED, __HIP_MEMORY_SCOPE_AGENT);
    for (unsigned spins = 0; spins < spin_limit; ++spins) {
      const unsigned c = __hip_atomic_load(word, __ATOMIC_RELAXED, __HIP_MEMORY_SCOPE_AGENT);
      if (__builtin_amdgcn_readfirstlane((int)c) >= (int)target) {
        ok = 1;
        break;
      }
      __builtin_amdgcn_s_sleep(RLS_POLL_SLEEP);
    }
    if (tid == 0) *lds_flag = ok;
  }
  __syncthreads();
  return *lds_flag != 0;
}

constexpr unsigned RLS_SRV_MAX_COMMANDS = 2048u;
struct srv_head {
  unsigned seq, n, mbseq, pad;
};
__device__ static inline srv_head srv_read_head(const unsigned* ctl) {
  typedef unsigned u4h __attribute__((ext_vector_type(4)));
  u4h w;
  asm volatile("global_load_dwordx4 %0, %1, off sc0 sc1\n\ts_waitcnt vmcnt(0)" : "=v"(w) : "v"(ctl) : "memory");
  return srv_head{w.x, w.y, w.z, w.w};
}
__device__ static inline unsigned resident_listen(unsigned* ctl, unsigned& srv_seq, unsigned idle_us, resident_sync* sync, unsigned& epoch,
                                                  unsigned nwg, unsigned spin_limit, int* lds_flag, rls_mailbox_slot& mb,
                                                  unsigned served) {
  const int tid = threadIdx.x;
  if (blockIdx.x == 0 && tid == 0) {
    asm volatile("s_waitcnt vmcnt(0)" ::: "memory");
    const unsigned long long t0 = wall_clock64(), idle = (unsigned long long)idle_us * 100ull;
    unsigned n = RLS_SRV_EXIT;
    srv_head hd{srv_seq, 0u, 0u, 0u};
    for (; served < RLS_SRV_MAX_COMMANDS;) {
      hd = srv_read_head(ctl);
      if (hd.seq != srv_seq) break;
      if (wall_clock64() - t0 > idle) {
        __hip_atomic_store(ctl + 16, 1u, __ATOMIC_RELAXED, __HIP_MEMORY_SCOPE_SYSTEM);
        asm volatile("s_waitcnt vmcnt(0)" ::: "memory");
        hd = srv_read_head(ctl);
        if (hd.seq != srv_seq) __hip_atomic_store(ctl + 16, 0u, __ATOMIC_RELAXED, __HIP_MEMORY_SCOPE_SYSTEM);
        break;
      }
      __builtin_amdgcn_s_sleep(8);
    }
    if (hd.seq != srv_seq) n = hd.n;
    __hip_atomic_store(&sync->srv_n, n, __ATOMIC_RELAXED, __HIP_MEMORY_SCOPE_AGENT);
    __hip_atomic_store(&sync->srv_mb, hd.mbseq, __ATOMIC_RELAXED, __HIP_MEMORY_SCOPE_AGENT);
    asm volatile("s_waitcnt vmcnt(0)" ::: "memory");
  }
  __syncthreads();
  if (!grid_arrive_wait(sync->cnt, ++epoch, nwg, spin_limit, lds_flag)) {
    resident_give_up(sync, nullptr);
    if (blockIdx.x == 0 && tid == 0) __hip_atomic_store(ctl + 17, 2u, __ATOMIC_RELAXED, __HIP_MEMORY_SCOPE_SYSTEM);
    return RLS_SRV_EXIT;
  }
  const unsigned cmd = __hip_atomic_load(&sync->srv_n, __ATOMIC_RELAXED, __HIP_MEMORY_SCOPE_AGENT);
  if (cmd == RLS_SRV_EXIT) {
    if (blockIdx.x == 0 && tid == 0) __hip_atomic_store(ctl + 17, 1u, __ATOMIC_RELAXED, __HIP_MEMORY_SCOPE_SYSTEM);
    return RLS_SRV_EXIT;
  }
  mb.seq = __hip_atomic_load(&sync->srv_mb, __ATOMIC_RELAXED, __HIP_MEMORY_SCOPE_AGENT);
  srv_seq += 1;
  return cmd;
}
```

### regularizedleastsquares.jl_amd/csrc/rls_common.hpp

```cpp
#pragma once
#include <hip/hip_runtime.h>

#include <chrono>
#include <mutex>
#include <cstdint>
#include <cstdio>
#include <cstring>
#include <type_traits>

#include "../../include/rls_mi355x.h"

#define RLS_WAVE 64

struct rls_tuning {
  int gemvn_g = 0;
  int gemvn_waves = 0;
  int gemvt_cols = 0;
  int gemvt_reverse = -1;
  int graph_chunk = 16;
  int use_graph = 1;
  int fuse_level = 1;
  int fused_normal = 1;
  int cgnr_pipeline = 1;
  int batched_mfma = 1;
  int gram_pipeline = 1;
  int pipe_hint_mode = 0;
  int resident = 1;
  int resident_preclear = 1;
  int resident_server = 1;
  int resident_server_idle_us = 300;
  int resident_ahead = 1;
  int fista_defer = 1;
  int resident_l2_rows = 1;
  int small = 1;
  int status_mailbox = 2;
  int slab_g = 0;
  int slab_order = 1;
  int resident_barrier = 2;
  int red_threads = 1024;
  int slab_multi = 1;
  int skinny_t_waves = 4, skinny_t_u = 4, skinny_v_waves = 4, skinny_v_u = 1, skinny_v_splits = 0;
  int skinny_t_roll = 8, skinny_v_roll = 2, skinny_g_roll = 8;
  int skinny_half = 1;
  int gram_lds = 96 * 1024;
  int64_t tv_fused_max_n = 2048;
  int tv_fused_2d = 1;
  int kaczmarz_nt = 0;
  int resident_spin = 100000;
};

constexpr int RLS_FETCH_MAX = 24;
struct rls_ctx {
  int device = 0;
  void* server = nullptr;
  uint64_t id = 0;
  hipStream_t stream = nullptr;
  bool own_stream = false;
  hipEvent_t ev0 = nullptr, ev1 = nullptr;
  char err[512] = {0};
  double* red_d = nullptr;
  float* res_d = nullptr;
  float* res_h = nullptr;
  rls_tuning tune;
  uint64_t tune_epoch = 0;
  int cus = 0;
  int resident_failures = 0;
  bool pools = false;
  struct fetch_item {
    const void* src;
    void* dst;
    unsigned dwords;
  } fq[RLS_FETCH_MAX];
  int nfq = 0;
  unsigned* mb_h = nullptr;
  unsigned mb_seq = 0;
};

int32_t rls_fetch_add(rls_ctx* ctx, const void* src_d, void* dst_pinned, size_t bytes);
int32_t rls_fetch_wait(rls_ctx* ctx);
struct rls_mailbox_slot {
  void* dst = nullptr;
  unsigned* seq_h = nullptr;
  unsigned seq = 0;
};
rls_mailbox_slot rls_mailbox_arm(rls_ctx* ctx, void* dst_pinned);
constexpr unsigned RLS_SRV_EXIT = 0xffffffffu;
constexpr unsigned RLS_SRV_AHEAD = 0x80000000u;
struct rls_srv_args {
  unsigned* ctl = nullptr;
  unsigned seq0 = 0, idle_us = 0;
  rls_mailbox_slot mb;
};
int32_t rls_mailbox_wait(rls_ctx* ctx, unsigned seq);
#ifdef __HIPCC__
__device__ static inline void rls_system_stores_done() { asm volatile("s_waitcnt vmcnt(0)" ::: "memory"); }
template <typename S>
__device__ static inline void rls_mailbox_publish(const rls_mailbox_slot& mb, const S& v, int lane) {
  constexpr unsigned ND = sizeof(S) / 4;
  static_assert(sizeof(S) % 4 == 0 && ND <= 64, "status structs are published dword by dword by one wave");
  if (!mb.dst) return;
  const unsigned* src = reinterpret_cast<const unsigned*>(&v);
  unsigned mine = 0;
#pragma unroll
  for (unsigned i = 0; i < ND; ++i) mine = lane == (int)i ? src[i] : mine;
  if (lane < (int)ND) __hip_atomic_store(reinterpret_cast<unsigned*>(mb.dst) + lane, mine, __ATOMIC_RELAXED, __HIP_MEMORY_SCOPE_SYSTEM);
  rls_system_stores_done();
  if (lane == 0) __hip_atomic_store(mb.seq_h, mb.seq, __ATOMIC_RELAXED, __HIP_MEMORY_SCOPE_SYSTEM);
}
#endif

hipError_t rls_dev_alloc(rls_ctx* ctx, void** p, size_t bytes);
hipError_t rls_dev_free(rls_ctx* ctx, void* p);
hipError_t rls_pinned_alloc(void** p, size_t bytes);
void rls_pinned_free(void* p);
void rls_server_stop(rls_ctx* ctx);
static inline hipError_t rls_enter(rls_ctx* ctx) {
  if (ctx->server) rls_server_stop(ctx);
  return hipSetDevice(ctx->device);
}
bool rls_ctx_alive(const rls_ctx* ctx, uint64_t id);
struct rls_alloc_scope {
  rls_ctx* prev;
  explicit rls_alloc_scope(rls_ctx* ctx);
  ~rls_alloc_scope();
};
hipError_t rls_scoped_malloc(void** p, size_t bytes);
hipError_t rls_scoped_free(void* p);

static inline void rls_cpu_relax() {
#if defined(__x86_64__) || defined(__i386__)
  __builtin_ia32_pause();
#elif defined(__aarch64__)
  asm volatile("yield");
#endif
}
template <typename Q, typename B>
static inline hipError_t rls_bounded_spin(Q&& query, B&& block) {
  const auto t0 = std::chrono::steady_clock::now();
  for (unsigned n = 0;; ++n) {
    const hipError_t e = query();
    if (e != hipErrorNotReady) return e;
    rls_cpu_relax();
    if ((n & 63) == 63 && std::chrono::steady_clock::now() - t0 > std::chrono::milliseconds(250)) break;
  }
  return block();
}
static inline hipError_t rls_stream_wait(hipStream_t s) {
  return rls_bounded_spin([s] { return hipStreamQuery(s); }, [s] { return hipStreamSynchronize(s); });
}
static inline hipError_t rls_event_wait(hipEvent_t ev) {
  return rls_bounded_spin([ev] { return hipEventQuery(ev); }, [ev] { return hipEventSynchronize(ev); });
}

void rls_resident_forget(int device, hipStream_t stream);
inline std::mutex& rls_capture_mutex() {
  static std::mutex m;
  return m;
}

#include <atomic>
struct rls_device_once {
  std::atomic<uint64_t> done{0};
  std::mutex mu;
  struct guard {
    rls_device_once* o;
    uint64_t bit;
    bool run;
    bool ok = true;
    guard(rls_device_once* o_, uint64_t bit_, bool run_) : o(o_), bit(bit_), run(run_) {}
    guard(const guard&) = delete;
    guard(guard&& g) : o(g.o), bit(g.bit), run(g.run), ok(g.ok) { g.run = false; }
    ~guard() {
      if (run) {
        if (ok) o->done.fetch_or(bit, std::memory_order_release);
        o->mu.unlock();
      }
    }
    explicit operator bool() const { return run; }
    void failed() { ok = false; }
  };
  guard first(int device) {
    const uint64_t bit = 1ull << (device & 63);
    if (done.load(std::memory_order_acquire) & bit) return guard(this, bit, false);
    mu.lock();
    if (done.load(std::memory_order_acquire) & bit) {
      mu.unlock();
      return guard(this, bit, false);
    }
    return guard(this, bit, true);
  }
};

constexpr int RLS_RED_SLOTS = 4096;
constexpr int RLS_RES_FLOATS = 64;

#define RLS_CHECK_CTX(ctx)            \
  do {                                \
    if (!(ctx)) return RLS_E_INVALID; \
  } while (0)

static inline int32_t rls_fail(rls_ctx* ctx, int32_t code, const char* what) {
  if (ctx) snprintf(ctx->err, sizeof(ctx->err), "%s (code %d)", what, (int)code);
  return code;
}

#define RLS_HIP(ctx, expr)                                                                       \
  do {                                                                                           \
    hipError_t _e = (expr);                                                                      \
    if (_e != hipSuccess) {                                                                      \
      if (ctx)                                                                                   \
        snprintf((ctx)->err, sizeof((ctx)->err), "%s failed: %s (%s:%d)", #expr,                 \
                 hipGetErrorString(_e), __FILE__, __LINE__);                                     \
      return (int32_t)_e;                                                                        \
    }                                                                                            \
  } while (0)

#define RLS_TRY(expr)            \
  do {                           \
    int32_t _s = (expr);         \
    if (_s != 0) return _s;      \
  } while (0)

static inline int32_t launch_status(rls_ctx* ctx) {
  hipError_t e = hipGetLastError();
  if (e != hipSuccess) return rls_fail(ctx, (int32_t)e, hipGetErrorString(e));
  return 0;
}

template <auto Kern>
static inline hipError_t rls_allow_lds(int device, size_t bytes) {
  static rls_device_once once;
  hipError_t e = hipSuccess;
  if (auto g = once.first(device)) {
    e = hipFuncSetAttribute(reinterpret_cast<const void*>(Kern), hipFuncAttributeMaxDynamicSharedMemorySize, (int)bytes);
    if (e != hipSuccess) g.failed();
  }
  return e;
}

template <auto Kern, typename... A>
// ... 353 lines not shown
  } else {
    static_assert(NV == 1, "scalar chunk");
    c.e[0] = *p;
  }
  return c;
}
template <typename E, int NV>
__device__ static inline chunk<E, NV> zero_chunk() {
  chunk<E, NV> c;
#pragma unroll
  for (int i = 0; i < NV; ++i) c.e[i] = elem<E>::zero();
  return c;
}

#endif

struct cgnr_scalars {
  double rr;
  double z0;
  double zeta;
  double alpha_re, alpha_im, beta_re, beta_im;
  float lambda, rel_tol;
  int iteration, max_iter, done;
  int pending;
  int cur;
  int fresh;
};

struct fista_scalars {
  double norm_x0, res_norm, rel_res_norm;
  float rho, theta, theta_old, rel_tol, lambda;
  int iteration, max_iter, done, restart, reg_kind, proj_kind;
  long long l21_slices;
  int pending;
  int ycur;
  int fresh;
};
#define RLS_FISTA_COPY(dst, src)        \
  do {                                  \
    (dst).norm_x0 = (src).norm_x0;      \
    (dst).res_norm = (src).res_norm;    \
    (dst).rel_res_norm = (src).rel_res_norm; \
    (dst).rho = (src).rho;              \
    (dst).theta = (src).theta;          \
    (dst).theta_old = (src).theta_old;  \
    (dst).rel_tol = (src).rel_tol;      \
    (dst).lambda = (src).lambda;        \
    (dst).iteration = (src).iteration;  \
    (dst).max_iter = (src).max_iter;    \
    (dst).done = (src).done;            \
    (dst).restart = (src).restart;      \
    (dst).reg_kind = (src).reg_kind;    \
    (dst).proj_kind = (src).proj_kind;  \
    (dst).l21_slices = (src).l21_slices; \
    (dst).pending = (src).pending;      \
    (dst).ycur = (src).ycur;            \
    (dst).fresh = (src).fresh;          \
  } while (0)

#ifdef __HIPCC__
__device__ static inline int uni(int v) { return __builtin_amdgcn_readfirstlane(v); }
__device__ static inline float uni(float v) { return __builtin_bit_cast(float, __builtin_amdgcn_readfirstlane(__builtin_bit_cast(int, v))); }
__device__ static inline double uni(double v) {
  const long long b = __builtin_bit_cast(long long, v);
  const unsigned lo = (unsigned)__builtin_amdgcn_readfirstlane((int)(b & 0xffffffffll));
  const unsigned hi = (unsigned)__builtin_amdgcn_readfirstlane((int)(b >> 32));
  return __builtin_bit_cast(double, ((long long)hi << 32) | (long long)lo);
}
__device__ static inline long long uni(long long v) {
  const unsigned lo = (unsigned)__builtin_amdgcn_readfirstlane((int)(v & 0xffffffffll));
  const unsigned hi = (unsigned)__builtin_amdgcn_readfirstlane((int)(v >> 32));
  return ((long long)hi << 32) | (long long)lo;
}
#define RLS_CGNR_UNIFORM(S)                                                       \
  do {                                                                            \
    (S).rr = uni((S).rr); (S).z0 = uni((S).z0); (S).zeta = uni((S).zeta);         \
    (S).alpha_re = uni((S).alpha_re); (S).alpha_im = uni((S).alpha_im);           \
    (S).beta_re = uni((S).beta_re); (S).beta_im = uni((S).beta_im);               \
    (S).lambda = uni((S).lambda); (S).rel_tol = uni((S).rel_tol);                 \
    (S).iteration = uni((S).iteration); (S).max_iter = uni((S).max_iter);         \
    (S).done = uni((S).done); (S).pending = uni((S).pending);                     \
    (S).cur = uni((S).cur); (S).fresh = uni((S).fresh);                           \
  } while (0)
#define RLS_FISTA_UNIFORM(S)                                                      \
  do {                                                                            \
    (S).norm_x0 = uni((S).norm_x0); (S).res_norm = uni((S).res_norm);             \
    (S).rel_res_norm = uni((S).rel_res_norm); (S).rho = uni((S).rho);             \
    (S).theta = uni((S).theta); (S).theta_old = uni((S).theta_old);               \
    (S).rel_tol = uni((S).rel_tol); (S).lambda = uni((S).lambda);                 \
    (S).iteration = uni((S).iteration); (S).max_iter = uni((S).max_iter);         \
    (S).done = uni((S).done); (S).restart = uni((S).restart);                     \
    (S).reg_kind = uni((S).reg_kind); (S).proj_kind = uni((S).proj_kind);         \
    (S).l21_slices = uni((S).l21_slices); (S).pending = uni((S).pending);         \
    (S).ycur = uni((S).ycur); (S).fresh = uni((S).fresh);                         \
  } while (0)
#endif

struct rls_fista_pipe {
  const void* A;
  int64_t lda, M, N;
  void *b0, *b1;
  void *x0, *res;
  void *y0, *y1;
  void *res_raw, *slab;
  fista_scalars *sc, *scn;
  int par_hint = -1;
  rls_mailbox_slot mb;
};
int32_t rls_fista_pipe_iteration(rls_ctx* ctx, int32_t dtype, const rls_fista_pipe& P);
int32_t rls_fista_pipe_finish(rls_ctx* ctx, int32_t dtype, const rls_fista_pipe& P);
int32_t rls_fista_resident_launch(rls_ctx* ctx, int32_t dtype, const rls_fista_pipe& P, void* sync, int n_steps,
                                  unsigned spin_limit, const rls_srv_args& Sv = rls_srv_args());

struct rls_cgnr_pipe {
  const void* A;
  int64_t lda, M, N;
  void *x, *r0, *p0, *r1, *p1, *v, *slab;
  double* dots;
  double* ttw = nullptr;
  int ndots;
  cgnr_scalars *sc, *scn;
  int nrhs = 1;
  int64_t vstride = 0;
  int cur_hint = -1;
  rls_mailbox_slot mb;
};
int32_t rls_cgnr_pipe_iteration(rls_ctx* ctx, int32_t dtype, const rls_cgnr_pipe& P);
int32_t rls_cgnr_pipe_finish(rls_ctx* ctx, int32_t dtype, const rls_cgnr_pipe& P);
int32_t rls_cgnr_pipe_launch(rls_ctx* ctx, int32_t dtype, const rls_cgnr_pipe& P, int which);
size_t rls_cgnr_resident_sync_bytes();
size_t rls_resident_sync_alloc_bytes(int32_t dtype, int64_t N);
size_t rls_resident_sync_clear_bytes();
size_t rls_resident_sync_flags_offset();
size_t rls_resident_sync_placement_offset();
bool rls_cgnr_resident_ok(rls_ctx* ctx, int32_t dtype, int64_t M, int64_t N, const void* A, int64_t lda);
int rls_cgnr_resident_nwg(rls_ctx* ctx, int32_t dtype, int64_t M, int64_t N);
struct rls_cg_start {
  int enabled = 0;
  const void* b = nullptr;
  const void *beta_y = nullptr, *z = nullptr, *u = nullptr;
  void *beta = nullptr, *xold = nullptr;
  float rho_admm = 0.f, rho = 0.f, reltol = 0.f;
  int maxiter = 0;
  const int* skip = nullptr;
  int* poison = nullptr;
  unsigned* srv_ctl = nullptr;
  unsigned srv_seq0 = 0;
  unsigned srv_idle_us = 0;
  rls_mailbox_slot srv_mb;
};

int32_t rls_cgnr_resident_launch(rls_ctx* ctx, int32_t dtype, const rls_cgnr_pipe& P, double* dout, void* sync,
                                 int n_steps, unsigned spin_limit, const rls_cg_start& start = rls_cg_start());

struct pgm_state {
  int iteration, done;
  float res_norm, pad;
};
struct pogm_auto_state {
  int iteration, done;
  float res_norm, pad;
  float theta, theta_old, sigma, gamma;
};
constexpr int RLS_PGM_MAX_IT = 48;
struct rls_pgm_coefs {
  float c[RLS_PGM_MAX_IT][8];
};
struct rls_pgm_desc {
  const void* A;
  int64_t lda, M, N;
  int kind;
  void *v0, *v1, *v2;
  void* v3 = nullptr;
  void *o0, *res;
  const void* x0;
  void *slab, *raw;
  pgm_state* st;
  float norm_x0, rel_tol;
  int reg_kind, proj_kind;
  int first_it;
};
bool rls_pgm_resident_ok(rls_ctx* ctx, int32_t dtype, int64_t M, int64_t N, const void* A, int64_t lda);
int32_t rls_pgm_resident_launch(rls_ctx* ctx, int32_t dtype, const rls_pgm_desc& D, const rls_pgm_coefs& C, void* sync,
                                int n_steps, unsigned spin_limit);

struct rls_gram_pipe {
  const void* G;
  int64_t ldg, N;
  void* x;
  void *r[2], *p[2], *v[2];
  double* dots;
  cgnr_scalars* sc[2];
};
bool rls_gram_pipe_ok(int32_t dtype, int64_t N, const void* G, int64_t ldg);
int rls_gram_pipe_nwg(int32_t dtype, int64_t N);
int32_t rls_gram_pipe_iteration(rls_ctx* ctx, int32_t dtype, const rls_gram_pipe& P, int parity);
int32_t rls_gram_pipe_finish(rls_ctx* ctx, int32_t dtype, const rls_gram_pipe& P, int parity);
bool rls_gram_resident_ok(rls_ctx* ctx, int32_t dtype, int64_t N, const void* G, int64_t ldg);
bool rls_gram_resident_server_ok(int32_t dtype, int64_t N);
int32_t rls_gram_resident_launch(rls_ctx* ctx, int32_t dtype, const rls_gram_pipe& P, void* sync, int n_steps,
                                 unsigned spin_limit, const rls_cg_start& start = rls_cg_start());

struct rls_fista_gram {
  const void* G;
  int64_t ldg, N;
  void *b0, *b1, *x0, *res, *y0, *y1;
  void* rr[2];
  fista_scalars* sc[2];
  int par_hint = -1;
};
int32_t rls_fista_gram_iteration(rls_ctx* ctx, int32_t dtype, const rls_fista_gram& P, int parity);
int32_t rls_fista_gram_finish(rls_ctx* ctx, int32_t dtype, const rls_fista_gram& P, int parity);
int32_t rls_fista_gram_resident_launch(rls_ctx* ctx, int32_t dtype, const rls_fista_gram& P, void* sync, int n_steps,
                                       unsigned spin_limit, const rls_srv_args& Sv = rls_srv_args());

#ifdef __HIPCC__
template <typename E>
struct panel_col {
  E* full;
  float* half;
  __device__ inline void put(int64_t i, E v) const {
    if (half) {
      half[16 * i] = elem<E>::re(v);
      half[16 * i + 8] = elem<E>::im(v);
    } else {
      full[16 * i] = v;
    }
  }
};
template <typename E>
__device__ static inline panel_col<E> panel_column(E* panel, int64_t n, int b, int half) {
  panel_col<E> c;
  c.full = half ? nullptr : panel + (int64_t)(b >> 4) * n * 16 + (b & 15);
  c.half = half ? reinterpret_cast<float*>(panel) + (b & 7) : nullptr;
  return c;
}
#endif

struct rls_skinny {
  const void* A;
  int64_t lda, M, N;
  const void* G = nullptr;
  int64_t ldg = 0;
  int nrhs, ngroups, splits;
  int half = 0;
  void *X, *R, *P, *V;
  int64_t ldv;
  float *Ppack, *Tpack;
  void* Vpart;
  int64_t ldvp;
  cgnr_scalars* sc;
};
bool rls_skinny_ok(int32_t dtype, int64_t M, int64_t N, const void* A, int64_t lda);
int rls_skinny_half(const rls_ctx* ctx, int32_t dtype, int nrhs);
static inline int rls_skinny_groups(int nrhs, int half) { return half ? 1 : (nrhs + 15) / 16; }
static inline int rls_skinny_pad(int nrhs, int half) { return half ? 8 : ((nrhs + 15) / 16) * 16; }
void rls_skinny_sizes(const rls_ctx* ctx, int32_t dtype, int64_t M, int64_t N, int nrhs, size_t* p_bytes, size_t* t_bytes,
                      size_t* v_bytes, int* splits);
int32_t rls_skinny_init(rls_ctx* ctx, int32_t dtype, const rls_skinny& K, const void* B, int64_t ldb, float lambda,
                        float rel_tol, int max_iter);
int32_t rls_skinny_launch(rls_ctx* ctx, int32_t dtype, const rls_skinny& K, int which);
int32_t rls_skinny_atb(rls_ctx* ctx, int32_t dtype, const rls_skinny& K, const void* B, int64_t ldb);
bool rls_gram_tiles_ok(int64_t M, int64_t N);
int32_t rls_gram_tiles(rls_ctx* ctx, int32_t dtype, int64_t M, int64_t N, const void* A, int64_t lda, void* G,
                       int64_t ldg);
int32_t rls_skinny_gram(rls_ctx* ctx, int32_t dtype, int64_t M, int64_t N, const void* A, int64_t lda, void* G,
                        int64_t ldg, void* panels);

struct rls_small {
  const void* A;
  int64_t lda, M, N;
  void *x, *r, *p, *v;
  cgnr_scalars* sc;
  rls_mailbox_slot mb;
  const void* b = nullptr;
  float lambda = 0.f, rel_tol = 0.f;
  int max_iter = 0;
  rls_srv_args srv;
};
constexpr int RLS_SMALL_GROUP_MAX = 24;
struct rls_small_group {
  int count = 0;
  rls_small d[RLS_SMALL_GROUP_MAX];
};
static_assert(sizeof(rls_small_group) + 64 <= 4096, "rls_small_group no longer fits the 4 KiB kernarg segment: shrink rls_small or RLS_SMALL_GROUP_MAX");
int32_t rls_small_group_launch(rls_ctx* ctx, int32_t dtype, const rls_small_group& G, int n_steps);
bool rls_small_ok(int32_t dtype, int64_t M, int64_t N, const void* A, int64_t lda);
int32_t rls_small_launch(rls_ctx* ctx, int32_t dtype, const rls_small& D, int n_steps);
struct rls_fista_pipe;
int32_t rls_fista_small_launch(rls_ctx* ctx, int32_t dtype, const rls_fista_pipe& P, int n_steps,
                               const rls_srv_args& Sv = rls_srv_args());

struct rls_gramk {
  const void* G;
  int64_t ldg, N;
  int nrhs;
  void *X, *R, *P, *V;
  int64_t ldv;
  cgnr_scalars* sc;
  float* Vx;
  void* Xx;
  double* dots;
  float* Ppack;
};
void rls_gramk_sizes(int64_t N, size_t* vx_bytes, size_t* xx_bytes, size_t* dots_bytes);
bool rls_gramk_resident_ok(rls_ctx* ctx, int32_t dtype, int64_t N, int nrhs, const void* G, int64_t ldg);
// ... 33 lines not shown
```

### regularizedleastsquares.jl_amd/csrc/solvers.hip

```cpp
#include "rls_common.hpp"

#include <algorithm>
#include <mutex>
#include <vector>


template <typename T>
static hipError_t dmalloc(T** p, size_t bytes) { return rls_scoped_malloc(reinterpret_cast<void**>(p), bytes); }
static hipError_t dfree(void* p) { return rls_scoped_free(p); }
template <typename T>
static hipError_t hmalloc(T** p, size_t bytes) { return rls_pinned_alloc(reinterpret_cast<void**>(p), bytes); }
static void hfree(void* p) { rls_pinned_free(p); }
static rls_ctx* alloc_ctx_of(rls_ctx* ctx, uint64_t id) { return rls_ctx_alive(ctx, id) ? ctx : nullptr; }

struct rls_operator {
  rls_ctx* ctx;
  uint64_t ctx_id = 0;
  int32_t dtype;
  int64_t M, N;
  const void* A;
  int64_t lda;
  const void* G;
  int64_t ldg;
  void* t;
  void* slab;
};

static int32_t op_normal(rls_operator* op, const void* p, void* v, const int* skip) {
  rls_ctx* ctx = op->ctx;
  if (op->G) return rls_launch_gemv(ctx, op->dtype, RLS_OP_N, op->N, op->N, 1.f, 0.f, op->G, op->ldg, p, 0.f, 0.f, v, skip);
  if (!op->A) return rls_fail(ctx, RLS_E_STATE, "operator has neither A nor a Gram matrix");
  if (op->slab && ctx->tune.fused_normal)
    return rls_launch_normal_fused(ctx, op->dtype, op->M, op->N, op->A, op->lda, p, v, op->slab, skip);
  RLS_TRY(rls_launch_gemv(ctx, op->dtype, RLS_OP_N, op->M, op->N, 1.f, 0.f, op->A, op->lda, p, 0.f, 0.f, op->t, skip));
  return rls_launch_gemv(ctx, op->dtype, RLS_OP_C, op->M, op->N, 1.f, 0.f, op->A, op->lda, op->t, 0.f, 0.f, v, skip);
}

struct step_graph {
  hipGraphExec_t exec = nullptr;
  int steps = 0;
  void* x_bound = nullptr;
  int mode = 0;
  bool failed = false;
  uint64_t epoch = 0;
};

template <typename F, typename R>
static int32_t run_steps(rls_ctx* ctx, step_graph* big, int n_steps, F&& enqueue_one, R&& rewind) {
  const int chunk = ctx->tune.graph_chunk;
  while (n_steps > 0) {
    if (ctx->tune.use_graph && chunk > 1 && n_steps >= chunk && !big->failed) {
      if (!big->exec || big->steps != chunk || big->epoch != ctx->tune_epoch) {
        if (big->exec) {
          hipGraphExecDestroy(big->exec);
          big->exec = nullptr;
        }
        hipGraph_t graph = nullptr;
        std::unique_lock<std::mutex> capture_lock(rls_capture_mutex());
        hipError_t e = hipStreamBeginCapture(ctx->stream, hipStreamCaptureModeRelaxed);
        int32_t st = 0;
        int calls = 0;
        if (e == hipSuccess) {
          for (int i = 0; i < chunk && st == 0; ++i, ++calls) st = enqueue_one();
          e = hipStreamEndCapture(ctx->stream, &graph);
        }
        capture_lock.unlock();
        if (e != hipSuccess || st != 0 || !graph ||
            hipGraphInstantiate(&big->exec, graph, nullptr, nullptr, 0) != hipSuccess) {
          big->failed = true;
          big->exec = nullptr;
          (void)hipGetLastError();
          rewind(calls);
        } else {
          big->steps = chunk;
          big->epoch = ctx->tune_epoch;
        }
        if (graph) hipGraphDestroy(graph);
        if (big->failed) continue;
      }
      RLS_HIP(ctx, hipGraphLaunch(big->exec, ctx->stream));
      n_steps -= chunk;
    } else {
      RLS_TRY(enqueue_one());
      n_steps -= 1;
    }
  }
  return 0;
}

template <typename F>
static int32_t run_steps(rls_ctx* ctx, step_graph* big, int n_steps, F&& enqueue_one) {
  return run_steps(ctx, big, n_steps, enqueue_one, [](int) {});
}

static inline int pipe_cur_hint(const rls_ctx* ctx, int k) {
  const int chunk = ctx->tune.graph_chunk;
  if (ctx->tune.pipe_hint_mode == 1) return -1;
  if (ctx->tune.pipe_hint_mode == 2) return k == 0 ? 1 : (k & 1);
  if (k == 0) return (ctx->tune.use_graph && chunk > 1) ? -1 : 0;
  if (ctx->tune.use_graph && chunk > 1 && (chunk % 2 != 0 || k % chunk == 0)) return -1;
  return (k - 1) & 1;
}

struct srv_state {
  unsigned* ctl = nullptr;
  bool alive = false;
  bool fresh = false;
  bool off = false;
  int served = 0, short_lives = 0;
  unsigned seq = 0;
  bool* resident_used = nullptr;
};

struct rls_cgnr {
  rls_operator* op;
  rls_ctx* actx;
  uint64_t actx_id = 0;
  int device;
  void *x, *r, *p, *v;
  cgnr_scalars* sc;
  cgnr_scalars* sc_h;
  step_graph graph;
  bool initialised;
  void *r1, *p1;
  double* dots;
  double* ttw = nullptr;
  cgnr_scalars* scn;
  int nrhs;
  int64_t ldv;
  void* slab_b;
  bool gram_pipe;
  void* v1;
  double* gdots;
  bool skinny;
  float *Ppack, *Tpack;
  void* Vpart;
  int splits;
  int half;
  void* rsync;
  double* rdots;
  unsigned* rsync_h;
  bool resident_used;
  rls_mailbox_slot mb_arm;
  srv_state srv;
  bool mb_sent = false;
  bool gram_resident;
  bool resident_off;
  int fallbacks;
  long long requested;
  bool rsync_clean = false;
  bool small = false;
  bool gramk = false;
  float* gk_vx = nullptr;
  void* gk_xx = nullptr;
  double* gk_dots = nullptr;
  void* q_b = nullptr;
  void* q_bh = nullptr;
  void* q_xh = nullptr;
};

static bool cgnr_use_gram_pipeline(const rls_cgnr* s) {
  return s->gram_pipe && s->op->G && s->op->ctx->tune.gram_pipeline;
}

static rls_gram_pipe cgnr_gram_desc(const rls_cgnr* s) {
  rls_gram_pipe P;
  P.G = s->op->G;
  P.ldg = s->op->ldg;
  P.N = s->op->N;
  P.x = s->x;
  P.r[0] = s->r;
  P.r[1] = s->r1;
  P.p[0] = s->p;
  P.p[1] = s->p1;
  P.v[0] = s->v;
  P.v[1] = s->v1;
  P.dots = s->gdots;
  P.sc[0] = s->sc;
  P.sc[1] = s->scn;
  return P;
}

static rls_skinny cgnr_skinny_desc(const rls_cgnr* s) {
  rls_skinny K;
  K.A = s->op->A;
  K.lda = s->op->lda;
  K.M = s->op->M;
  K.N = s->op->N;
  K.G = s->op->G;
  K.ldg = s->op->ldg;
  K.nrhs = s->nrhs;
  K.half = s->half;
  K.ngroups = rls_skinny_groups(s->nrhs, s->half);
  K.splits = s->splits;
  K.X = s->x;
  K.R = s->r;
  K.P = s->p;
  K.V = s->v;
  K.ldv = s->ldv;
  K.Ppack = s->Ppack;
  K.Tpack = s->Tpack;
  K.Vpart = s->Vpart;
  K.ldvp = s->op->N;
  K.sc = s->sc;
  return K;
}

static bool cgnr_use_small(const rls_cgnr* s) {
  return s->small && s->nrhs == 1 && !s->op->G && s->op->ctx->tune.small && s->op->ctx->tune.resident;
}

static bool cgnr_use_gramk(const rls_cgnr* s, int n_steps) {
  return s->gramk && s->rsync && !s->resident_off && s->op->ctx->tune.resident &&
         (n_steps != 1 || s->op->ctx->tune.resident == 2);
}

static rls_gramk cgnr_gramk_desc(const rls_cgnr* s) {
  rls_gramk D;
  D.G = s->op->G;
  D.ldg = s->op->ldg;
  D.N = s->op->N;
  D.nrhs = s->nrhs;
  D.X = s->x;
  D.R = s->r;
  D.P = s->p;
  D.V = s->v;
  D.ldv = s->ldv;
  D.sc = s->sc;
  D.Vx = s->gk_vx;
  D.Xx = s->gk_xx;
  D.dots = s->gk_dots;
  D.Ppack = s->half ? s->Ppack : nullptr;
  return D;
}

static bool cgnr_use_gram_resident(const rls_cgnr* s) {
  return s->gram_resident && s->rsync && !s->resident_off && s->nrhs == 1 && cgnr_use_gram_pipeline(s) &&
         s->op->ctx->tune.resident;
}

static bool cgnr_use_pipeline(const rls_cgnr* s) {
  const rls_ctx* ctx = s->op->ctx;
  return s->r1 && s->op->slab && !s->op->G && ctx->tune.fused_normal && ctx->tune.cgnr_pipeline;
}

static bool cgnr_use_resident(const rls_cgnr* s) {
  const rls_ctx* ctx = s->op->ctx;
  auto al16 = [](const void* q) { return (reinterpret_cast<uintptr_t>(q) & 15) == 0; };
  return s->rsync && !s->resident_off && s->nrhs == 1 && cgnr_use_pipeline(s) && ctx->tune.resident && al16(s->x) &&
         al16(s->r) && al16(s->p) && al16(s->v);
}

static hipEvent_t g_resident_ev[64];
static resident_chain_state g_resident_chain;
void rls_resident_forget(int device, hipStream_t stream) {
  resident_chain_forget(rls_capture_mutex(), g_resident_chain, device, (void*)stream);
}
template <typename F>
static int32_t resident_chain(rls_ctx* ctx, void* rsync, F&& launch, bool* clean = nullptr) {
  const int d = ctx->device < 64 ? ctx->device : 63;
  return resident_chain_step(
      rls_capture_mutex(), g_resident_chain, ctx->device, (void*)ctx->stream,
      [&](void* prev) -> int32_t {
        if (!g_resident_ev[d]) RLS_HIP(ctx, hipEventCreateWithFlags(&g_resident_ev[d], hipEventDisableTiming));
        RLS_HIP(ctx, hipEventRecord(g_resident_ev[d], (hipStream_t)prev));
        RLS_HIP(ctx, hipStreamWaitEvent(ctx->stream, g_resident_ev[d], 0));
        return 0;
      },
      [&]() -> int32_t {
        if (clean && *clean && ctx->tune.resident_preclear) *clean = false;
        else RLS_HIP(ctx, hipMemsetAsync(rsync, 0, rls_resident_sync_clear_bytes(), ctx->stream));
        if (!ctx->tune.resident_l2_rows)
          RLS_HIP(ctx, hipMemsetAsync((char*)rsync + rls_resident_sync_placement_offset(), 1, 1, ctx->stream));
        return launch();
      });
}
static int32_t resident_chain_launch(rls_ctx* ctx, rls_cgnr* s, const rls_cgnr_pipe& P, int n_steps) {
  return resident_chain(ctx, s->rsync, [&]() {
    return rls_cgnr_resident_launch(ctx, s->op->dtype, P, s->rdots, s->rsync, n_steps, (unsigned)ctx->tune.resident_spin);
  }, &s->rsync_clean);
}
static hipError_t resident_alloc(rls_ctx* ctx, const rls_operator* op, void** rsync, unsigned** rsync_h) {
  hipError_t e = dmalloc(rsync, rls_resident_sync_alloc_bytes(op->dtype, op->N));
  if (e == hipSuccess) e = hipMemsetAsync(*rsync, 0, rls_cgnr_resident_sync_bytes(), ctx->stream);
  if (e == hipSuccess && rsync_h && !*rsync_h) {
    e = hmalloc(rsync_h, 4 * sizeof(unsigned));
    if (e == hipSuccess) memset(*rsync_h, 0, 4 * sizeof(unsigned));
  }
  return e;
}
static int32_t resident_fetch_flags(rls_ctx* ctx, const void* rsync, unsigned* rsync_h) {
  return rls_fetch_add(ctx, (const char*)rsync + rls_resident_sync_flags_offset(), rsync_h, 3 * sizeof(unsigned));
}
static unsigned resident_lost(rls_ctx* ctx, void* rsync, unsigned* rsync_h, bool* off, int* fallbacks) {
  const unsigned lost = rsync_h[2];
  if (!lost) return 0;
  (void)hipMemsetAsync((char*)rsync + rls_resident_sync_flags_offset() + 2 * sizeof(unsigned), 0, sizeof(unsigned), ctx->stream);
  rsync_h[2] = 0;
  *off = true;
  *fallbacks += (int)lost;
  if (++ctx->resident_failures >= 2) ctx->tune.resident = 0;
  return lost;
}

static rls_cgnr_pipe cgnr_pipe_desc(const rls_cgnr* s) {
  rls_cgnr_pipe P;
  P.A = s->op->A;
  P.lda = s->op->lda;
  P.M = s->op->M;
  P.N = s->op->N;
  P.x = s->x;
// ... 1484 lines not shown
  }
  *out = op;
  return 0;
}

int32_t rls_operator_set_gram(rls_operator* op, const void* AHA, int64_t ld) {
  if (!op) return RLS_E_INVALID;
  if (AHA && ld < op->N) return rls_fail(op->ctx, RLS_E_INVALID, "operator_set_gram: ld < N");
  op->G = AHA;
  op->ldg = ld;
  return 0;
}

int32_t rls_operator_destroy(rls_operator* op) {
  if (!op) return RLS_E_INVALID;
  rls_alloc_scope alloc_scope(alloc_ctx_of(op->ctx, op->ctx_id));
  if (op->slab) dfree(op->slab);
  if (op->t) dfree(op->t);
  delete op;
  return 0;
}

int32_t rls_operator_mul(rls_operator* op, const void* x, void* y) {
  if (!op) return RLS_E_INVALID;
  if (!op->A) return rls_fail(op->ctx, RLS_E_STATE, "operator_mul: operator has no forward matrix");
  return rls_launch_gemv(op->ctx, op->dtype, RLS_OP_N, op->M, op->N, 1.f, 0.f, op->A, op->lda, x, 0.f, 0.f, y, nullptr);
}
int32_t rls_operator_mul_adj(rls_operator* op, const void* y, void* x) {
  if (!op) return RLS_E_INVALID;
  if (!op->A) return rls_fail(op->ctx, RLS_E_STATE, "operator_mul_adj: operator has no forward matrix");
  return rls_launch_gemv(op->ctx, op->dtype, RLS_OP_C, op->M, op->N, 1.f, 0.f, op->A, op->lda, y, 0.f, 0.f, x, nullptr);
}
int32_t rls_operator_mul_normal_skip(rls_operator* op, const void* p, void* v, const void* skip_d) {
  if (!op) return RLS_E_INVALID;
  rls_ctx* ctx = op->ctx;
  if (!p || !v) return rls_fail(ctx, RLS_E_INVALID, "operator_mul_normal_skip: null pointer");
  RLS_HIP(ctx, rls_enter(ctx));
  return op_normal(op, p, v, (const int*)skip_d);
}

int32_t rls_operator_mul_normal(rls_operator* op, const void* p, void* v) {
  if (!op || !p || !v) return RLS_E_INVALID;
  return op_normal(op, p, v, nullptr);
}

int32_t rls_gram(rls_ctx* ctx, int32_t dtype, int64_t M, int64_t N, const void* A, int64_t lda, void* G, int64_t ld) {
  RLS_CHECK_CTX(ctx);
  if (!rls_dtype_ok(dtype) || M <= 0 || N <= 0 || !A || !G || lda < M || ld < N)
    return rls_fail(ctx, RLS_E_INVALID, "gram: bad argument");
  RLS_HIP(ctx, rls_enter(ctx));
  if (ctx->tune.batched_mfma && rls_gram_tiles_ok(M, N) && rls_skinny_ok(dtype, M, N, A, lda))
    return rls_gram_tiles(ctx, dtype, M, N, A, lda, G, ld);
  if (ctx->tune.batched_mfma && N <= 65535 * 16 && rls_skinny_ok(dtype, M, N, A, lda)) {
    void* panels = nullptr;
    rls_alloc_scope alloc_scope(ctx);
    RLS_HIP(ctx, dmalloc(&panels, (size_t)M * (size_t)N * rls_elem_size(dtype)));
    int32_t st = rls_skinny_gram(ctx, dtype, M, N, A, lda, G, ld, panels);
    if (st == 0) st = gram_hermitianize(ctx, dtype, N, G, ld);
    hipError_t e = rls_stream_wait(ctx->stream);
    dfree(panels);
    if (st == 0 && e != hipSuccess) st = rls_fail(ctx, (int32_t)e, hipGetErrorString(e));
    return st;
  }
  dim3 grid((unsigned)((N + 63) / 64), (unsigned)((N + 63) / 64));
  if (dtype == RLS_F32)
    hipLaunchKernelGGL(gram_kernel<float>, grid, dim3(256), 0, ctx->stream, (const float*)A, lda, M, N, (float*)G, ld);
  else
    hipLaunchKernelGGL(gram_kernel<float2>, grid, dim3(256), 0, ctx->stream, (const float2*)A, lda, M, N, (float2*)G, ld);
  RLS_TRY(launch_status(ctx));
  return gram_hermitianize(ctx, dtype, N, G, ld);
}

static int32_t cgnr_create_impl(rls_operator* op, int32_t nrhs, void* x, void* r, void* p, void* v, int64_t ldv,
                                rls_cgnr** out) {
  if (!op) return RLS_E_INVALID;
  rls_ctx* ctx = op->ctx;
  if (!x || !r || !p || !v || !out || nrhs < 1 || ldv < op->N)
    return rls_fail(ctx, RLS_E_INVALID, "cgnr_create: bad argument");
  RLS_HIP(ctx, rls_enter(ctx));
  const bool skinny = nrhs > 1 && ctx->tune.batched_mfma && rls_skinny_ok(op->dtype, op->M, op->N, op->A, op->lda) &&
                      (!op->G || rls_skinny_ok(op->dtype, op->N, op->N, op->G, op->ldg));
  if (nrhs > 1 && !skinny)
    return rls_fail(ctx, RLS_E_UNSUPPORTED, "batched CGNR runs on the matrix cores: A (and AHA, when explicit) with M, N multiples "
                                            "of 16 and 16-byte aligned columns (other shapes: one plan per column)");
  rls_alloc_scope alloc_scope(ctx);
  rls_cgnr* s = new rls_cgnr();
  s->actx = ctx;
  s->actx_id = ctx->id;
  s->skinny = skinny;
  s->gram_pipe = false;
  s->v1 = nullptr;
  s->gdots = nullptr;
  s->Ppack = s->Tpack = nullptr;
  s->Vpart = nullptr;
  s->splits = 1;
  s->op = op;
  s->device = ctx->device;
  s->x = x;
  s->r = r;
  s->p = p;
  s->v = v;
  s->initialised = false;
  s->r1 = s->p1 = nullptr;
  s->dots = nullptr;
  s->scn = nullptr;
  s->sc = nullptr;
  s->sc_h = nullptr;
  s->nrhs = nrhs;
  s->ldv = ldv;
  s->slab_b = nullptr;
  s->rsync = nullptr;
  s->rdots = nullptr;
  s->rsync_h = nullptr;
  s->resident_used = false;
  s->gram_resident = false;
  s->resident_off = false;
  s->fallbacks = 0;
  s->requested = 0;
  const size_t sb = sizeof(cgnr_scalars) * (size_t)nrhs;
  hipError_t e = dmalloc(&s->sc, sb);
  if (e == hipSuccess) e = hipMemsetAsync(s->sc, 0, sb, ctx->stream);
  if (e == hipSuccess) e = hmalloc(&s->sc_h, sb);
  if (e == hipSuccess) memset(s->sc_h, 0, sb);
  if (e == hipSuccess && op->slab) {
    const size_t vb = (size_t)ldv * nrhs * rls_elem_size(op->dtype);
    const size_t nd = (size_t)((op->N + 15) / 16) * 4 * sizeof(double) * nrhs;
    e = dmalloc(&s->r1, vb);
    if (e == hipSuccess) e = dmalloc(&s->p1, vb);
    if (e == hipSuccess) e = hipMemsetAsync(s->r1, 0, vb, ctx->stream);
    if (e == hipSuccess) e = hipMemsetAsync(s->p1, 0, vb, ctx->stream);
    if (e == hipSuccess) e = dmalloc(&s->dots, nd);
    if (e == hipSuccess && op->A && !op->G) {
      const size_t tb = (size_t)rls_cgnr_resident_nwg(op->ctx, op->dtype, op->M, op->N) * sizeof(double) * nrhs;
      e = dmalloc(&s->ttw, tb);
      if (e == hipSuccess) e = hipMemsetAsync(s->ttw, 0, tb, ctx->stream);
    }
    if (e == hipSuccess) e = dmalloc(&s->scn, sb);
    if (e == hipSuccess) e = hipMemsetAsync(s->dots, 0, nd, ctx->stream);
    if (e == hipSuccess) e = hipMemsetAsync(s->scn, 0, sb, ctx->stream);
    if (e == hipSuccess && nrhs > 1 && !skinny)
      e = dmalloc(&s->slab_b, rls_normal_fused_workspace(op->ctx, op->dtype, op->M, op->N, op->A, op->lda) * (size_t)nrhs);
  }
  s->small = nrhs == 1 && op->A && !op->G && rls_small_ok(op->dtype, op->M, op->N, op->A, op->lda);
  if (e == hipSuccess && s->small && !s->srv.ctl && hmalloc(&s->srv.ctl, 32 * sizeof(unsigned)) == hipSuccess) {
    memset(s->srv.ctl, 0, 32 * sizeof(unsigned));
    s->srv.resident_used = nullptr;
  }
  if (e == hipSuccess && nrhs == 1 && op->slab && op->A && !op->G &&
      rls_cgnr_resident_ok(ctx, op->dtype, op->M, op->N, op->A, op->lda)) {
    const size_t db = (size_t)rls_cgnr_resident_nwg(op->ctx, op->dtype, op->M, op->N) * 4 * sizeof(double);
    e = resident_alloc(ctx, op, &s->rsync, &s->rsync_h);
    if (e == hipSuccess) e = dmalloc(&s->rdots, db);
    if (e == hipSuccess) e = hipMemsetAsync(s->rdots, 0, db, ctx->stream);
    if (e == hipSuccess && !s->srv.ctl) e = hmalloc(&s->srv.ctl, 32 * sizeof(unsigned));
    if (e == hipSuccess) memset(s->srv.ctl, 0, 32 * sizeof(unsigned));
    s->srv.resident_used = &s->resident_used;
  }
  if (e == hipSuccess && nrhs == 1 && op->G && rls_gram_pipe_ok(op->dtype, op->N, op->G, op->ldg)) {
    const size_t vb = (size_t)op->N * rls_elem_size(op->dtype);
    const size_t nd = (size_t)2 * rls_gram_pipe_nwg(op->dtype, op->N) * 4 * sizeof(double);
    if (!s->r1) e = dmalloc(&s->r1, vb);
    if (e == hipSuccess && !s->p1) e = dmalloc(&s->p1, vb);
    if (e == hipSuccess) e = dmalloc(&s->v1, vb);
    if (e == hipSuccess) e = dmalloc(&s->gdots, nd);
    if (e == hipSuccess && !s->scn) e = dmalloc(&s->scn, sb);
    if (e == hipSuccess) e = hipMemsetAsync(s->r1, 0, vb, ctx->stream);
    if (e == hipSuccess) e = hipMemsetAsync(s->p1, 0, vb, ctx->stream);
    if (e == hipSuccess) e = hipMemsetAsync(s->v1, 0, vb, ctx->stream);
    if (e == hipSuccess) e = hipMemsetAsync(s->gdots, 0, nd, ctx->stream);
    if (e == hipSuccess) e = hipMemsetAsync(s->scn, 0, sb, ctx->stream);
    s->gram_pipe = e == hipSuccess;
    if (e == hipSuccess && !s->rsync && rls_gram_resident_ok(ctx, op->dtype, op->N, op->G, op->ldg)) {
      e = resident_alloc(ctx, op, &s->rsync, &s->rsync_h);
      s->gram_resident = e == hipSuccess;
      if (e == hipSuccess && !s->srv.ctl && rls_gram_resident_server_ok(op->dtype, op->N) &&
          hmalloc(&s->srv.ctl, 32 * sizeof(unsigned)) == hipSuccess) {
        memset(s->srv.ctl, 0, 32 * sizeof(unsigned));
        s->srv.resident_used = &s->resident_used;
      }
    }
  }
  if (e == hipSuccess && skinny) {
    size_t pb, tb, vb;
    rls_skinny_sizes(op->ctx, op->dtype, op->M, op->N, nrhs, &pb, &tb, &vb, &s->splits);
    s->half = rls_skinny_half(op->ctx, op->dtype, nrhs);
    e = dmalloc(&s->Ppack, pb);
    if (e == hipSuccess) e = hipMemsetAsync(s->Ppack, 0, pb, ctx->stream);
    if (e == hipSuccess) e = dmalloc(&s->Tpack, tb);
    if (e == hipSuccess) e = dmalloc(&s->Vpart, vb);
    if (e == hipSuccess && op->G && s->half && rls_gramk_resident_ok(ctx, op->dtype, op->N, nrhs, op->G, op->ldg)) {
      size_t xb, xxb, db;
      rls_gramk_sizes(op->N, &xb, &xxb, &db);
      e = resident_alloc(ctx, op, &s->rsync, &s->rsync_h);
      if (e == hipSuccess) e = dmalloc(&s->gk_vx, xb);
      if (e == hipSuccess) e = hipMemsetAsync(s->gk_vx, 0, xb, ctx->stream);
      if (e == hipSuccess) e = dmalloc(&s->gk_xx, xxb);
      if (e == hipSuccess) e = dmalloc(&s->gk_dots, db);
      if (e == hipSuccess) e = hipMemsetAsync(s->gk_dots, 0, db, ctx->stream);
      s->gramk = e == hipSuccess;
    }
  }
  if (e != hipSuccess) {
    rls_cgnr_destroy(s);
    return rls_fail(ctx, (int32_t)e, "cgnr_create: allocation failed");
  }
  *out = s;
  return 0;
}

int32_t rls_cgnr_create(rls_operator* op, void* x, void* r, void* p, void* v, rls_cgnr** out) {
  if (!op) return RLS_E_INVALID;
  return cgnr_create_impl(op, 1, x, r, p, v, op->N, out);
}

int32_t rls_cgnr_create_batched(rls_operator* op, int32_t nrhs, void* X, void* R, void* P, void* V, int64_t ldv,
                                rls_cgnr** out) {
  return cgnr_create_impl(op, nrhs, X, R, P, V, ldv, out);
}

int32_t rls_cgnr_destroy(rls_cgnr* s) {
  if (!s) return RLS_E_INVALID;
  if (rls_ctx_alive(s->actx, s->actx_id) && s->actx->server == &s->srv) rls_server_stop(s->actx);
  hipSetDevice(s->device);
  rls_alloc_scope alloc_scope(alloc_ctx_of(s->actx, s->actx_id));
  if (s->graph.exec) hipGraphExecDestroy(s->graph.exec);
  if (s->r1) dfree(s->r1);
  if (s->p1) dfree(s->p1);
  if (s->dots) dfree(s->dots);
  if (s->ttw) dfree(s->ttw);
  if (s->scn) dfree(s->scn);
  if (s->slab_b) dfree(s->slab_b);
  if (s->v1) dfree(s->v1);
  if (s->gdots) dfree(s->gdots);
  if (s->Ppack) dfree(s->Ppack);
  if (s->Tpack) dfree(s->Tpack);
  if (s->Vpart) dfree(s->Vpart);
  if (s->gk_vx) dfree(s->gk_vx);
  if (s->gk_xx) dfree(s->gk_xx);
  if (s->gk_dots) dfree(s->gk_dots);
  if (s->q_b) dfree(s->q_b);
  if (s->q_bh) hfree(s->q_bh);
  if (s->q_xh) hfree(s->q_xh);
  if (s->rsync) dfree(s->rsync);
  if (s->rdots) dfree(s->rdots);
  if (s->rsync_h) hfree(s->rsync_h);
  if (s->srv.ctl) hfree(s->srv.ctl);
  if (s->sc) dfree(s->sc);
  if (s->sc_h) hfree(s->sc_h);
  delete s;
  return 0;
}

int32_t rls_cgnr_init_local_a(rls_cgnr* s, const void* b, float lambda, float rel_tol, int32_t iterations) {
  if (!s) return RLS_E_INVALID;
  rls_operator* op = s->op;
  rls_ctx* ctx = op->ctx;
  if (!b) return rls_fail(ctx, RLS_E_INVALID, "cgnr_init: null b");
  if (s->nrhs != 1) return rls_fail(ctx, RLS_E_STATE, "cgnr_init on a batched plan: use rls_cgnr_init_batched");
  RLS_HIP(ctx, rls_enter(ctx));
  if (op->A)
    RLS_TRY(rls_launch_gemv(ctx, op->dtype, RLS_OP_C, op->M, op->N, 1.f, 0.f, op->A, op->lda, b, 0.f, 0.f, s->r, nullptr));
  else
    RLS_HIP(ctx, hipMemcpyAsync(s->r, b, (size_t)op->N * rls_elem_size(op->dtype), hipMemcpyDeviceToDevice, ctx->stream));
  s->sc_h->lambda = lambda;
  s->sc_h->rel_tol = rel_tol;
  s->sc_h->max_iter = cgnr_effective_iterations(s, iterations);
  return 0;
}

int32_t rls_cgnr_init_local_b(rls_cgnr* s) {
  if (!s) return RLS_E_INVALID;
  rls_ctx* ctx = s->op->ctx;
  RLS_HIP(ctx, rls_enter(ctx));
  if (s->op->dtype == RLS_F32)
    cgnr_launch_init<float>(s, s->sc_h->lambda, s->sc_h->rel_tol, s->sc_h->max_iter);
  else
    cgnr_launch_init<float2>(s, s->sc_h->lambda, s->sc_h->rel_tol, s->sc_h->max_iter);
  s->initialised = true;
  s->requested = 0;
  s->srv.off = false;
  s->srv.short_lives = 0;
  return launch_status(ctx);
}

static int32_t cgnr_group(rls_cgnr* const* plans, const void* const* b, int32_t count, float lambda, float rel_tol, int32_t iterations,
                          int32_t n_steps);
int32_t rls_cgnr_init(rls_cgnr* s, const void* b, float lambda, float rel_tol, int32_t iterations) {
  if (s && b && s->nrhs == 1 && s->op->A && cgnr_use_small(s)) return cgnr_group(&s, &b, 1, lambda, rel_tol, iterations, 0);
  RLS_TRY(rls_cgnr_init_local_a(s, b, lambda, rel_tol, iterations));
  return rls_cgnr_init_local_b(s);
}

int32_t rls_cgnr_init_batched(rls_cgnr* s, const void* B, int64_t ldb, float lambda, float rel_tol, int32_t iterations) {
  if (!s) return RLS_E_INVALID;
  rls_operator* op = s->op;
  rls_ctx* ctx = op->ctx;
  if (!B || !op->A || ldb < op->M) return rls_fail(ctx, RLS_E_INVALID, "cgnr_init_batched: bad argument");
  RLS_HIP(ctx, rls_enter(ctx));
  const size_t es = rls_elem_size(op->dtype);
  const int max_iter = cgnr_effective_iterations(s, iterations);
  if (s->skinny) {
    RLS_TRY(rls_skinny_init(ctx, op->dtype, cgnr_skinny_desc(s), B, ldb, lambda, rel_tol, max_iter));
    s->sc_h->lambda = lambda;
    s->sc_h->rel_tol = rel_tol;
    s->sc_h->max_iter = max_iter;
    s->initialised = true;
    s->requested = 0;
    return 0;
  }
  if (!cgnr_use_pipeline(s)) return rls_fail(ctx, RLS_E_UNSUPPORTED, "cgnr_init_batched: fused pipeline not active");
  for (int b = 0; b < s->nrhs; ++b) {
    char* rb = (char*)s->r + (size_t)b * s->ldv * es;
    RLS_TRY(rls_launch_gemv(ctx, op->dtype, RLS_OP_C, op->M, op->N, 1.f, 0.f, op->A, op->lda,
                            (const char*)B + (size_t)b * ldb * es, 0.f, 0.f, rb, nullptr));
    char* xb = (char*)s->x + (size_t)b * s->ldv * es;
    char* pb = (char*)s->p + (size_t)b * s->ldv * es;
    char* vb = (char*)s->v + (size_t)b * s->ldv * es;
    if (op->dtype == RLS_F32)
      hipLaunchKernelGGL(cgnr_init_kernel<float>, dim3(1), dim3(UPD_THREADS), 0, ctx->stream, (float*)xb,
                         (const float*)rb, (float*)pb, (float*)vb, op->N, s->sc + b, lambda, rel_tol, max_iter);
    else
      hipLaunchKernelGGL(cgnr_init_kernel<float2>, dim3(1), dim3(UPD_THREADS), 0, ctx->stream, (float2*)xb,
                         (const float2*)rb, (float2*)pb, (float2*)vb, op->N, s->sc + b, lambda, rel_tol, max_iter);
  }
  s->sc_h->lambda = lambda;
  s->sc_h->rel_tol = rel_tol;
  s->sc_h->max_iter = max_iter;
  s->initialised = true;
  return launch_status(ctx);
}

static int32_t cgnr_step_impl(rls_cgnr* s, int32_t n_steps);
static void cgnr_status_out(const rls_cgnr* s, const cgnr_scalars& h, rls_cgnr_status* out);
int32_t rls_cgnr_get_status_batched(rls_cgnr* s, rls_cgnr_status* out) {
  if (!s || !out) return RLS_E_INVALID;
  rls_ctx* ctx = s->op->ctx;
  if (!s->initialised) return rls_fail(ctx, RLS_E_STATE, "cgnr_get_status before cgnr_init");
  RLS_HIP(ctx, rls_enter(ctx));
  if (s->resident_used) RLS_TRY(resident_fetch_flags(ctx, s->rsync, s->rsync_h));
  RLS_TRY(rls_fetch_add(ctx, s->sc, s->sc_h, sizeof(cgnr_scalars) * (size_t)s->nrhs));
  RLS_TRY(rls_fetch_wait(ctx));
  if (s->resident_used && resident_lost(ctx, s->rsync, s->rsync_h, &s->resident_off, &s->fallbacks)) {
    long long at = 0;
    bool live = false;
    for (int b = 0; b < s->nrhs; ++b) {
      if (s->sc_h[b].iteration > at) at = s->sc_h[b].iteration;
      live = live || !s->sc_h[b].done;
    }
    const long long missing = s->requested - at;
    if (live && missing > 0) {
      RLS_TRY(cgnr_step_impl(s, (int32_t)(missing > 0x7fffffff ? 0x7fffffff : missing)));
      RLS_TRY(rls_fetch_add(ctx, s->sc, s->sc_h, sizeof(cgnr_scalars) * (size_t)s->nrhs));
      RLS_TRY(rls_fetch_wait(ctx));
    }
  }
  s->resident_used = false;
  for (int b = 0; b < s->nrhs; ++b) {
    const cgnr_scalars& h = s->sc_h[b];
    out[b].iteration = h.iteration;
    out[b].done = h.done;
    out[b].alpha_re = (float)h.alpha_re;
    out[b].alpha_im = (float)h.alpha_im;
    out[b].beta_re = (float)h.beta_re;
    out[b].beta_im = (float)h.beta_im;
    out[b].zeta = (float)h.zeta;
    out[b].residual = (float)sqrt(h.rr);
    out[b].z0 = (float)h.z0;
    out[b].fallbacks = s->fallbacks;
  }
  return 0;
}

static int32_t cgnr_step_impl(rls_cgnr* s, int32_t n_steps) {
  rls_ctx* ctx = s->op->ctx;
  if (cgnr_use_small(s)) {
    if (n_steps == 0) return 0;
    rls_small D;
    D.A = s->op->A;
    D.lda = s->op->lda;
    D.M = s->op->M;
    D.N = s->op->N;
    D.x = s->x;
    D.r = s->r;
    D.p = s->p;
    D.v = s->v;
    D.sc = s->sc;
    D.mb = s->mb_arm;
    s->mb_sent = s->mb_arm.dst != nullptr;
    return rls_small_launch(ctx, s->op->dtype, D, n_steps);
  }
  if (s->skinny && cgnr_use_gramk(s, n_steps)) {
    if (n_steps == 0) return 0;
    const rls_gramk D = cgnr_gramk_desc(s);
    s->resident_used = true;
    return resident_chain(ctx, s->rsync, [&]() {
      return rls_gramk_resident_launch(ctx, D, s->rsync, n_steps, (unsigned)ctx->tune.resident_spin);
    }, &s->rsync_clean);
  }
  if (s->skinny) {
    const rls_skinny K = cgnr_skinny_desc(s);
    const int32_t dtype = s->op->dtype;
    if (s->graph.steps && s->graph.mode != 2) {
      hipGraphExecDestroy(s->graph.exec);
      s->graph = step_graph();
    }
    s->graph.mode = 2;
    return run_steps(ctx, &s->graph, n_steps, [ctx, dtype, &K]() { return rls_skinny_launch(ctx, dtype, K, 7); });
  }
  if (cgnr_use_gram_pipeline(s)) {
    const rls_gram_pipe P = cgnr_gram_desc(s);
    const int32_t dtype = s->op->dtype;
    if (cgnr_use_gram_resident(s)) {
      if (n_steps == 0) return 0;
      s->resident_used = true;
      return resident_chain(ctx, s->rsync, [&]() {
        return rls_gram_resident_launch(ctx, dtype, P, s->rsync, n_steps, (unsigned)ctx->tune.resident_spin);
      }, &s->rsync_clean);
    }
    if (s->graph.steps && s->graph.mode != 3) {
      hipGraphExecDestroy(s->graph.exec);
      s->graph = step_graph();
    }
    s->graph.mode = 3;
    int parity = 0;
    auto one = [ctx, dtype, &P, &parity]() {
      const int32_t st = rls_gram_pipe_iteration(ctx, dtype, P, parity);
      parity ^= 1;
      return st;
    };
    if (ctx->tune.graph_chunk % 2) {
      for (int i = 0; i < n_steps; ++i) RLS_TRY(one());
    } else {
      RLS_TRY(run_steps(ctx, &s->graph, n_steps, one, [&parity](int c) { parity ^= c & 1; }));
    }
    return rls_gram_pipe_finish(ctx, dtype, P, n_steps & 1);
  }
  if (cgnr_use_resident(s) && n_steps != 1) {
    if (n_steps == 0) return 0;
    const rls_cgnr_pipe P = cgnr_pipe_desc(s);
    s->resident_used = true;
    return resident_chain_launch(ctx, s, P, n_steps);
  }
  if (cgnr_use_pipeline(s)) {
    rls_cgnr_pipe P = cgnr_pipe_desc(s);
    const int32_t dtype = s->op->dtype;
    if (s->graph.steps && s->graph.mode != 1) {
      hipGraphExecDestroy(s->graph.exec);
      s->graph = step_graph();
    }
    s->graph.mode = 1;
    int k = 0;
    RLS_TRY(run_steps(ctx, &s->graph, n_steps, [ctx, dtype, &P, &k]() {
      P.cur_hint = pipe_cur_hint(ctx, k++);
      return rls_cgnr_pipe_iteration(ctx, dtype, P);
    }, [&k](int c) { k -= c; }));
    if (s->nrhs == 1) {
      P.mb = s->mb_arm;
      s->mb_sent = s->mb_arm.dst != nullptr;
    }
    return rls_cgnr_pipe_finish(ctx, dtype, P);
  }
  if (s->nrhs != 1) return rls_fail(ctx, RLS_E_UNSUPPORTED, "batched CGNR: fused pipeline switched off");
  if (s->graph.steps && s->graph.mode != 0) {
    hipGraphExecDestroy(s->graph.exec);
    s->graph = step_graph();
  }
  s->graph.mode = 0;
  return run_steps(ctx, &s->graph, n_steps, [s]() { return cgnr_enqueue_iteration(s); });
}

int32_t rls_cgnr_step(rls_cgnr* s, int32_t n_steps) {
  if (!s) return RLS_E_INVALID;
  rls_ctx* ctx = s->op->ctx;
  if (!s->initialised) return rls_fail(ctx, RLS_E_STATE, "cgnr_step before cgnr_init");
  if (n_steps < 0) return rls_fail(ctx, RLS_E_INVALID, "cgnr_step: n_steps < 0");
  RLS_HIP(ctx, rls_enter(ctx));
  s->requested += n_steps;
  return cgnr_step_impl(s, n_steps);
}

static int32_t cgnr_group(rls_cgnr* const* plans, const void* const* b, int32_t count, float lambda, float rel_tol, int32_t iterations,
                          int32_t n_steps) {
  if (!plans || count < 1 || !plans[0]) return RLS_E_INVALID;
  rls_ctx* ctx = plans[0]->op->ctx;
  if (n_steps < 0) return rls_fail(ctx, RLS_E_INVALID, "cgnr group: n_steps < 0");
  const int32_t dtype = plans[0]->op->dtype;
  RLS_HIP(ctx, rls_enter(ctx));
  for (int32_t k = 0; k < count; ++k) {
    rls_cgnr* s = plans[k];
    if (!s || s->op->ctx != ctx || s->op->dtype != dtype) return rls_fail(ctx, RLS_E_INVALID, "cgnr group: plans of one context and one element type");
    if (!cgnr_use_small(s)) return rls_fail(ctx, RLS_E_UNSUPPORTED, "cgnr group: a plan is not on the small-system path (rls_cgnr_path 8)");
    if (!b && !s->initialised) return rls_fail(ctx, RLS_E_STATE, "cgnr group: step before init");
    if (b && !b[k]) return rls_fail(ctx, RLS_E_INVALID, "cgnr group: null right-hand side");
  }
  for (int32_t k0 = 0; k0 < count; k0 += RLS_SMALL_GROUP_MAX) {
    rls_small_group G;
    G.count = count - k0 < RLS_SMALL_GROUP_MAX ? count - k0 : RLS_SMALL_GROUP_MAX;
    for (int j = 0; j < G.count; ++j) {
      rls_cgnr* s = plans[k0 + j];
      rls_small& D = G.d[j];
      D.A = s->op->A;
      D.lda = s->op->lda;
      D.M = s->op->M;
      D.N = s->op->N;
      D.x = s->x;
      D.r = s->r;
      D.p = s->p;
      D.v = s->v;
      D.sc = s->sc;
      if (b) {
        D.b = b[k0 + j];
        D.lambda = lambda;
        D.rel_tol = rel_tol;
        D.max_iter = cgnr_effective_iterations(s, iterations);
        s->sc_h->lambda = lambda;
        s->sc_h->rel_tol = rel_tol;
        s->sc_h->max_iter = D.max_iter;
        s->initialised = true;
        s->requested = 0;
      }
      s->requested += n_steps;
    }
    if (b || n_steps > 0) RLS_TRY(rls_small_group_launch(ctx, dtype, G, n_steps));
  }
  return 0;
}

int32_t rls_cgnr_get_status_group(rls_cgnr* const* plans, int32_t count, rls_cgnr_status* out) {
  if (!plans || !out || count < 1 || !plans[0]) return RLS_E_INVALID;
  rls_ctx* ctx = plans[0]->op->ctx;
  RLS_HIP(ctx, rls_enter(ctx));
  for (int32_t k = 0; k < count; ++k) {
    rls_cgnr* s = plans[k];
    if (!s || s->op->ctx != ctx || s->nrhs != 1) return rls_fail(ctx, RLS_E_INVALID, "cgnr status group: single-column plans of one context");
    if (!s->initialised) return rls_fail(ctx, RLS_E_STATE, "cgnr_get_status before cgnr_init");
    if (s->resident_used) return rls_fail(ctx, RLS_E_UNSUPPORTED, "cgnr status group: a plan has resident launches to account for (use rls_cgnr_get_status)");
  }
  for (int32_t k0 = 0; k0 < count; k0 += RLS_FETCH_MAX) {
    const int32_t k1 = k0 + RLS_FETCH_MAX < count ? k0 + RLS_FETCH_MAX : count;
    for (int32_t k = k0; k < k1; ++k) RLS_TRY(rls_fetch_add(ctx, plans[k]->sc, plans[k]->sc_h, sizeof(cgnr_scalars)));
    RLS_TRY(rls_fetch_wait(ctx));
  }
  for (int32_t k = 0; k < count; ++k) cgnr_status_out(plans[k], *plans[k]->sc_h, out + k);
  return 0;
}

static int32_t cgnr_queue_validate(rls_cgnr* const* plans, int32_t count, rls_ctx** ctx_out) {
  if (!plans || count < 1 || !plans[0]) return RLS_E_INVALID;
  rls_ctx* ctx = plans[0]->op->ctx;
  for (int32_t k = 0; k < count; ++k) {
    const rls_cgnr* s = plans[k];
    if (!s || s->op->ctx != ctx || s->nrhs != 1)
      return rls_fail(ctx, RLS_E_INVALID, "cgnr solve queue: single right-hand-side plans of one context");
    for (int32_t j = 0; j < k; ++j)
      if (plans[j] == s) return rls_fail(ctx, RLS_E_INVALID, "cgnr solve queue: a plan appears twice (one plan per problem)");
  }
  *ctx_out = ctx;
  return 0;
}

static int32_t cgnr_queue_statuses(rls_ctx* ctx, rls_cgnr* const* plans, int32_t count, rls_cgnr_status* out) {
  constexpr int32_t PER = RLS_FETCH_MAX / 2;
  for (int32_t k0 = 0; k0 < count; k0 += PER) {
    const int32_t k1 = k0 + PER < count ? k0 + PER : count;
    for (int32_t k = k0; k < k1; ++k) {
      rls_cgnr* s = plans[k];
      if (s->resident_used) RLS_TRY(resident_fetch_flags(ctx, s->rsync, s->rsync_h));
      RLS_TRY(rls_fetch_add(ctx, s->sc, s->sc_h, sizeof(cgnr_scalars)));
    }
    RLS_TRY(rls_fetch_wait(ctx));
  }
  for (int32_t k = 0; k < count; ++k) {
    rls_cgnr* s = plans[k];
    if (s->resident_used && resident_lost(ctx, s->rsync, s->rsync_h, &s->resident_off, &s->fallbacks)) {
      const long long missing = s->requested - (long long)s->sc_h->iteration;
      if (!s->sc_h->done && missing > 0) {
        RLS_TRY(cgnr_step_impl(s, (int32_t)(missing > 0x7fffffff ? 0x7fffffff : missing)));
        RLS_TRY(fetch_scalars(ctx, s->sc, s->sc_h));
      }
    }
    s->resident_used = false;
    if (out) cgnr_status_out(s, *s->sc_h, out + k);
  }
  return 0;
}

int32_t rls_cgnr_solve_queue(rls_cgnr* const* plans, const void* const* b, int32_t count, float lambda, float rel_tol,
                             int32_t iterations, rls_cgnr_status* out) {
  rls_ctx* ctx = nullptr;
  RLS_TRY(cgnr_queue_validate(plans, count, &ctx));
  if (!b || iterations < 0) return rls_fail(ctx, RLS_E_INVALID, "cgnr solve queue: bad argument");
  for (int32_t k = 0; k < count; ++k) {
    RLS_TRY(rls_cgnr_init(plans[k], b[k], lambda, rel_tol, iterations));
    RLS_TRY(rls_cgnr_step(plans[k], iterations));
  }
  return cgnr_queue_statuses(ctx, plans, count, out);
}

int32_t rls_cgnr_solve_queue_host(rls_cgnr* const* plans, const void* const* b_h, void* const* x_h, int32_t count, float lambda,
                                  float rel_tol, int32_t iterations, rls_cgnr_status* out) {
  rls_ctx* ctx = nullptr;
  RLS_TRY(cgnr_queue_validate(plans, count, &ctx));
  if (!b_h || !x_h || iterations < 0) return rls_fail(ctx, RLS_E_INVALID, "cgnr solve queue: bad argument");
  RLS_HIP(ctx, rls_enter(ctx));
  for (int32_t k = 0; k < count; ++k) {
    rls_cgnr* s = plans[k];
    const rls_operator* op = s->op;
    const size_t es = rls_elem_size(op->dtype);
    const size_t bb = (size_t)(op->A ? op->M : op->N) * es, xb = (size_t)op->N * es;
    if (!b_h[k] || !x_h[k]) return rls_fail(ctx, RLS_E_INVALID, "cgnr solve queue: null buffer");
    if (!s->q_b) {
      rls_alloc_scope alloc_scope(ctx);
      RLS_HIP(ctx, dmalloc(&s->q_b, bb));
      RLS_HIP(ctx, hmalloc(&s->q_bh, bb));
      RLS_HIP(ctx, hmalloc(&s->q_xh, xb));
    }
    memcpy(s->q_bh, b_h[k], bb);
    RLS_HIP(ctx, hipMemcpyAsync(s->q_b, s->q_bh, bb, hipMemcpyHostToDevice, ctx->stream));
    RLS_TRY(rls_cgnr_init(s, s->q_b, lambda, rel_tol, iterations));
    RLS_TRY(rls_cgnr_step(s, iterations));
    RLS_HIP(ctx, hipMemcpyAsync(s->q_xh, s->x, xb, hipMemcpyDeviceToHost, ctx->stream));
  }
  RLS_TRY(cgnr_queue_statuses(ctx, plans, count, out));
  bool any = false;
  for (int32_t k = 0; k < count; ++k) {
    rls_cgnr* s = plans[k];
    if (s->resident_off && s->fallbacks > 0) {
      RLS_HIP(ctx, hipMemcpyAsync(s->q_xh, s->x, (size_t)s->op->N * rls_elem_size(s->op->dtype), hipMemcpyDeviceToHost, ctx->stream));
      any = true;
    }
  }
  if (any) RLS_HIP(ctx, rls_stream_wait(ctx->stream));
// ... 54 lines not shown
         RLS_TRY(rls_cgnr_init_local_a(plans[r], b_parts[r], lambda, rel_tol, iterations));
         return rls_comm_publish(comm, r, plans[r]->r, N, dtype, round0);
       }, true},
      {[&](int r, int) {
         RLS_TRY(rls_comm_collect(comm, r, plans[r]->r, N, dtype, round0));
         return rls_cgnr_init_local_b(plans[r]);
       }, false}};
  return rls_comm_run(comm, phases, 1);
}

int32_t rls_cgnr_step_rowsharded(rls_comm* comm, rls_cgnr* const* plans, int32_t n_steps) {
  RLS_TRY(rowsharded_check<rls_cgnr>(comm, plans, cgnr_op, cgnr_single));
  if (n_steps < 0) return RLS_E_INVALID;
  const int64_t N = plans[0]->op->N;
  const int32_t dtype = plans[0]->op->dtype;
  int round0 = 0;
  RLS_TRY(rls_comm_next_rounds(comm, n_steps, N, dtype, &round0));
  const std::vector<rls_comm_phase> phases = {
      {[&](int r, int k) {
         RLS_TRY(rls_cgnr_step_local_a(plans[r]));
         return rls_comm_publish(comm, r, plans[r]->v, N, dtype, round0 + k);
       }, true},
      {[&](int r, int k) {
         RLS_TRY(rls_comm_collect(comm, r, plans[r]->v, N, dtype, round0 + k));
         return rls_cgnr_step_local_b(plans[r]);
       }, false}};
  return rls_comm_run(comm, phases, n_steps);
}

int32_t rls_fista_init_rowsharded(rls_comm* comm, rls_fista* const* plans, const void* const* b_parts, float rho, float theta,
                                  float rel_tol, int32_t iterations, int32_t restart_gradient) {
  RLS_TRY(rowsharded_check<rls_fista>(comm, plans, fista_op, fista_single));
  if (!b_parts) return RLS_E_INVALID;
  const int64_t N = plans[0]->op->N;
  const int32_t dtype = plans[0]->op->dtype;
  int round0 = 0;
  RLS_TRY(rls_comm_next_rounds(comm, 1, N, dtype, &round0));
  const std::vector<rls_comm_phase> phases = {
      {[&](int r, int) {
         RLS_TRY(rls_fista_init_local_a(plans[r], b_parts[r]));
         return rls_comm_publish(comm, r, plans[r]->x0, N, dtype, round0);
       }, true},
      {[&](int r, int) {
         RLS_TRY(rls_comm_collect(comm, r, plans[r]->x0, N, dtype, round0));
         return rls_fista_init_local_b(plans[r], rho, theta, rel_tol, iterations, restart_gradient);
       }, false}};
  return rls_comm_run(comm, phases, 1);
}

int32_t rls_fista_step_rowsharded(rls_comm* comm, rls_fista* const* plans, int32_t n_steps) {
  RLS_TRY(rowsharded_check<rls_fista>(comm, plans, fista_op, fista_single));
  if (n_steps < 0) return RLS_E_INVALID;
  const int64_t N = plans[0]->op->N;
  const int32_t dtype = plans[0]->op->dtype;
  int round0 = 0;
  RLS_TRY(rls_comm_next_rounds(comm, n_steps, N, dtype, &round0));
  const std::vector<rls_comm_phase> phases = {
      {[&](int r, int k) {
         RLS_TRY(rls_fista_step_local_a(plans[r]));
         return rls_comm_publish(comm, r, plans[r]->res, N, dtype, round0 + k);
       }, true},
      {[&](int r, int k) {
         RLS_TRY(rls_comm_collect(comm, r, plans[r]->res, N, dtype, round0 + k));
         return rls_fista_step_local_b(plans[r]);
       }, false}};
  return rls_comm_run(comm, phases, n_steps);
}

int32_t rls_cgnr_path(rls_cgnr* s, int32_t* out) {
  if (!s || !out) return RLS_E_INVALID;
  *out = cgnr_use_small(s) ? 8 : s->skinny ? (cgnr_use_gramk(s, 0) ? 7 : s->op->G ? 6 : 3) : cgnr_use_gram_resident(s) ? 5 : cgnr_use_gram_pipeline(s) ? 2 : cgnr_use_resident(s) ? 4 : cgnr_use_pipeline(s) ? 1 : 0;
  return 0;
}

int32_t rls_cgnr_step_local_a(rls_cgnr* s) {
  if (!s) return RLS_E_INVALID;
  if (!s->initialised) return rls_fail(s->op->ctx, RLS_E_STATE, "cgnr_step before cgnr_init");
  RLS_HIP(s->op->ctx, hipSetDevice(s->op->ctx->device));
  return op_normal(s->op, s->p, s->v, &s->sc->done);
}
int32_t rls_cgnr_step_local_b(rls_cgnr* s) {
  if (!s) return RLS_E_INVALID;
  if (!s->initialised) return rls_fail(s->op->ctx, RLS_E_STATE, "cgnr_step before cgnr_init");
  RLS_HIP(s->op->ctx, hipSetDevice(s->op->ctx->device));
  return cgnr_enqueue_update(s);
}

static int32_t cgnr_fetch_status(rls_cgnr* s) {
  rls_ctx* ctx = s->op->ctx;
  if (s->resident_used) RLS_TRY(resident_fetch_flags(ctx, s->rsync, s->rsync_h));
  RLS_TRY(fetch_scalars(ctx, s->sc, s->sc_h));
  if (s->resident_used && resident_lost(ctx, s->rsync, s->rsync_h, &s->resident_off, &s->fallbacks)) {
    const long long missing = s->requested - (long long)s->sc_h->iteration;
    if (!s->sc_h->done && missing > 0) {
      RLS_TRY(cgnr_step_impl(s, (int32_t)(missing > 0x7fffffff ? 0x7fffffff : missing)));
      RLS_TRY(fetch_scalars(ctx, s->sc, s->sc_h));
    }
  }
  s->resident_used = false;
  return 0;
}

int32_t rls_cgnr_get_status(rls_cgnr* s, rls_cgnr_status* out) {
  if (!s || !out) return RLS_E_INVALID;
  rls_ctx* ctx = s->op->ctx;
  if (!s->initialised) return rls_fail(ctx, RLS_E_STATE, "cgnr_get_status before cgnr_init");
  if (ctx->server == &s->srv && s->srv.alive && s->srv.fresh) {
    cgnr_status_out(s, *s->sc_h, out);
    return 0;
  }
  RLS_HIP(ctx, rls_enter(ctx));
  RLS_TRY(cgnr_fetch_status(s));
  cgnr_status_out(s, *s->sc_h, out);
  return 0;
}

static void cgnr_status_out(const rls_cgnr* s, const cgnr_scalars& h, rls_cgnr_status* out) {
  out->iteration = h.iteration;
  out->done = h.done;
  out->alpha_re = (float)h.alpha_re;
  out->alpha_im = (float)h.alpha_im;
  out->beta_re = (float)h.beta_re;
  out->beta_im = (float)h.beta_im;
  out->zeta = (float)h.zeta;
  out->residual = (float)sqrt(h.rr);
  out->z0 = (float)h.z0;
  out->fallbacks = s->fallbacks;
}

extern "C++" {
static bool server_usable(const rls_ctx* ctx, const srv_state* v) {
  return ctx->tune.resident_server && ctx->tune.status_mailbox && v->ctl && !v->off && (ctx->server == nullptr || ctx->server == v);
}
static bool cgnr_use_server(const rls_cgnr* s) {
  return server_usable(s->op->ctx, &s->srv) &&
         (cgnr_use_small(s) || cgnr_use_resident(s) || (cgnr_use_gram_resident(s) && s->nrhs == 1));
}

static void server_life_over(rls_ctx* ctx, srv_state* v) {
  const bool gave_up = v->ctl[17] == 2;
  if (v->alive) {
    if (v->served < 3) {
      if (++v->short_lives >= 2) v->off = true;
    } else {
      v->short_lives = 0;
    }
  }
  v->alive = false;
  v->fresh = false;
  if (gave_up && v->resident_used) *v->resident_used = true;
  if (ctx->server == v) ctx->server = nullptr;
}

void rls_server_stop(rls_ctx* ctx) {
  srv_state* v = static_cast<srv_state*>(ctx->server);
  if (!v) return;
  if (v->alive) {
    volatile unsigned* ctl = v->ctl;
    if (!ctl[17]) {
      ctl[1] = RLS_SRV_EXIT;
      std::atomic_thread_fence(std::memory_order_release);
      ctl[0] = ++v->seq;
      const auto t0 = std::chrono::steady_clock::now();
      for (unsigned n = 0; !ctl[17]; ++n) {
        rls_cpu_relax();
        if ((n & 1023) == 1023 && std::chrono::steady_clock::now() - t0 > std::chrono::milliseconds(500)) {
          (void)hipSetDevice(ctx->device);
          (void)hipStreamSynchronize(ctx->stream);
          break;
        }
      }
    }
  }
  server_life_over(ctx, v);
}

static int server_wait(rls_ctx* ctx, srv_state* v, unsigned mbseq) {
  volatile unsigned* mb = ctx->mb_h;
  volatile unsigned* ctl = v->ctl;
  const auto t0 = std::chrono::steady_clock::now();
  for (unsigned n = 0;; ++n) {
    if (*mb == mbseq) break;
    const unsigned ex = ctl[17];
    if (ex) {
      std::atomic_thread_fence(std::memory_order_acquire);
      if (*mb == mbseq) break;
      return (int)ex;
    }
    rls_cpu_relax();
    if ((n & 1023) == 1023 && std::chrono::steady_clock::now() - t0 > std::chrono::seconds(2)) {
      (void)hipStreamSynchronize(ctx->stream);
      if (*mb == mbseq) break;
      return ctl[17] == 1 ? 1 : 2;
    }
  }
  std::atomic_thread_fence(std::memory_order_acquire);
  return 0;
}

template <typename L>
static int32_t server_command(rls_ctx* ctx, srv_state* v, void* mirror, int32_t n_steps, bool usable_again, L&& launch) {
  volatile unsigned* ctl = v->ctl;
  for (int attempt = 0; attempt < 2; ++attempt) {
    const unsigned mbseq = ++ctx->mb_seq;
    if (v->alive) {
      ctl[1] = (unsigned)n_steps;
      ctl[2] = mbseq;
      std::atomic_thread_fence(std::memory_order_release);
      ctl[0] = ++v->seq;
      std::atomic_thread_fence(std::memory_order_seq_cst);
    } else {
      ctl[16] = ctl[17] = 0;
      ctl[0] = v->seq;
      rls_srv_args a;
      a.ctl = v->ctl;
      a.seq0 = v->seq;
      a.idle_us = (unsigned)(ctx->tune.resident_server_idle_us > 0 ? ctx->tune.resident_server_idle_us : 1);
      if (ctx->tune.resident_ahead) a.idle_us |= RLS_SRV_AHEAD;
      a.mb.dst = mirror;
      a.mb.seq_h = ctx->mb_h;
      a.mb.seq = mbseq;
      const int32_t st = launch(a);
      if (st != 0) return st < 0 ? st : -1;
      v->alive = true;
      v->served = 0;
      ctx->server = v;
    }
    const int r = server_wait(ctx, v, mbseq);
    if (r == 0) {
      v->served += 1;
      v->fresh = true;
      return 0;
    }
    server_life_over(ctx, v);
    if (r == 2) {
      if (v->resident_used) *v->resident_used = true;
      return 2;
    }
    if (attempt == 1 || !usable_again || v->off) {
      v->off = true;
      return 1;
    }
  }
  return 1;
}

extern "C" int32_t rls_cgnr_step_status(rls_cgnr* s, int32_t n_steps, rls_cgnr_status* out);
static int32_t cgnr_step_status_server(rls_cgnr* s, int32_t n_steps, rls_cgnr_status* out) {
  rls_ctx* ctx = s->op->ctx;
  RLS_HIP(ctx, hipSetDevice(s->device));
  s->requested += n_steps;
  const int32_t r = server_command(ctx, &s->srv, s->sc_h, n_steps, true, [&](const rls_srv_args& a) {
    rls_cg_start St;
    St.srv_ctl = a.ctl;
    St.srv_seq0 = a.seq0;
    St.srv_idle_us = a.idle_us & ~RLS_SRV_AHEAD;
    St.srv_mb = a.mb;
    if (cgnr_use_small(s)) {
      rls_small D;
      D.A = s->op->A;
      D.lda = s->op->lda;
      D.M = s->op->M;
      D.N = s->op->N;
      D.x = s->x;
      D.r = s->r;
      D.p = s->p;
      D.v = s->v;
      D.sc = s->sc;
      D.mb = a.mb;
      D.srv = a;
      return rls_small_launch(ctx, s->op->dtype, D, n_steps);
    }
    if (cgnr_use_gram_resident(s)) {
      const rls_gram_pipe G = cgnr_gram_desc(s);
      return resident_chain(ctx, s->rsync, [&]() {
        return rls_gram_resident_launch(ctx, s->op->dtype, G, s->rsync, n_steps, (unsigned)ctx->tune.resident_spin, St);
      }, &s->rsync_clean);
    }
    const rls_cgnr_pipe P = cgnr_pipe_desc(s);
    return resident_chain(ctx, s->rsync, [&]() {
      return rls_cgnr_resident_launch(ctx, s->op->dtype, P, s->rdots, s->rsync, n_steps, (unsigned)ctx->tune.resident_spin, St);
    }, &s->rsync_clean);
  });
  if (r < 0) return r;
  if (r == 0) {
    cgnr_status_out(s, *s->sc_h, out);
    return 0;
  }
  if (r == 1) {
    s->requested -= n_steps;
    return rls_cgnr_step_status(s, n_steps, out);
  }
  return rls_cgnr_get_status(s, out);
}
}

int32_t rls_cgnr_step_status(rls_cgnr* s, int32_t n_steps, rls_cgnr_status* out) {
  if (!s || !out) return RLS_E_INVALID;
  rls_ctx* ctx = s->op->ctx;
  if (s->initialised && n_steps > 0 && n_steps <= 8 && !s->resident_used && cgnr_use_server(s)) return cgnr_step_status_server(s, n_steps, out);
  if (s->initialised && s->nrhs == 1 && n_steps > 0 && !s->resident_used) {
    RLS_HIP(ctx, rls_enter(ctx));
    s->mb_arm = rls_mailbox_arm(ctx, s->sc_h);
  }
  s->mb_sent = false;
  const int32_t st = rls_cgnr_step(s, n_steps);
  const rls_mailbox_slot mb = s->mb_arm;
  s->mb_arm = rls_mailbox_slot();
  if (st != 0) return st;
  if (!s->mb_sent) return rls_cgnr_get_status(s, out);
  RLS_TRY(rls_mailbox_wait(ctx, mb.seq));
  cgnr_status_out(s, *s->sc_h, out);
  return 0;
}

int32_t rls_fista_create(rls_operator* op, void* x, void* x0, void* xold, void* res, rls_fista** out) {
  if (!op) return RLS_E_INVALID;
  rls_ctx* ctx = op->ctx;
  if (!x || !x0 || !xold || !res || !out) return rls_fail(ctx, RLS_E_INVALID, "fista_create: null pointer");
  RLS_HIP(ctx, rls_enter(ctx));
  rls_alloc_scope alloc_scope(ctx);
  rls_fista* s = new rls_fista();
  s->op = op;
  s->actx = ctx;
  s->actx_id = ctx->id;
  s->device = op->ctx->device;
  s->buf[0] = x;
  s->buf[1] = xold;
  s->x0 = x0;
  s->res = res;
  s->y = nullptr;
  s->reg_kind = RLS_REG_L1;
  s->proj_kind = RLS_PROJ_NONE;
  s->lambda = 0.f;
  s->l21_slices = 1;
  s->initialised = false;
  s->y1 = s->res_raw = nullptr;
  s->scn = nullptr;
  s->use_pipe = false;
  s->res_raw1 = nullptr;
  s->use_gram = false;
  s->small = op->A && !op->G && rls_small_ok(op->dtype, op->M, op->N, op->A, op->lda);
  if (s->small && hmalloc(&s->srv.ctl, 32 * sizeof(unsigned)) == hipSuccess) memset(s->srv.ctl, 0, 32 * sizeof(unsigned));
  const size_t vb = (size_t)op->N * rls_elem_size(op->dtype);
  hipError_t e = dmalloc(&s->y, vb);
  const bool gram = op->G && rls_gram_pipe_ok(op->dtype, op->N, op->G, op->ldg);
  if (e == hipSuccess && gram) {
    e = dmalloc(&s->res_raw1, vb);
    if (e == hipSuccess) e = hipMemsetAsync(s->res_raw1, 0, vb, ctx->stream);
  }
  if (e == hipSuccess && (op->slab || gram)) {
    e = dmalloc(&s->y1, vb);
    if (e == hipSuccess) e = dmalloc(&s->res_raw, 2 * vb);
    if (e == hipSuccess) e = dmalloc(&s->scn, sizeof(fista_scalars));
    if (e == hipSuccess) e = hipMemsetAsync(s->y1, 0, vb, ctx->stream);
    if (e == hipSuccess) e = hipMemsetAsync(s->res_raw, 0, 2 * vb, ctx->stream);
    if (e == hipSuccess) e = hipMemsetAsync(s->scn, 0, sizeof(fista_scalars), ctx->stream);
  }
  if (e != hipSuccess) {
    if (s->y) dfree(s->y);
    if (s->y1) dfree(s->y1);
    if (s->res_raw) dfree(s->res_raw);
    if (s->res_raw1) dfree(s->res_raw1);
    if (s->scn) dfree(s->scn);
    delete s;
    return rls_fail(ctx, (int32_t)e, "fista_create: hipMalloc failed");
  }
  if ((op->slab && op->A && !op->G && rls_cgnr_resident_ok(ctx, op->dtype, op->M, op->N, op->A, op->lda)) ||
      (gram && rls_gram_resident_ok(ctx, op->dtype, op->N, op->G, op->ldg))) {
    if (resident_alloc(ctx, op, &s->rsync, &s->rsync_h) != hipSuccess) {
      if (s->rsync) dfree(s->rsync);
      s->rsync = nullptr;
      (void)hipGetLastError();
    } else if ((!gram || rls_gram_resident_server_ok(op->dtype, op->N)) &&
               (s->srv.ctl || hmalloc(&s->srv.ctl, 32 * sizeof(unsigned)) == hipSuccess)) {
      memset(s->srv.ctl, 0, 32 * sizeof(unsigned));
      s->srv.resident_used = &s->resident_used;
    }
  }
  int32_t st = alloc_scalars(ctx, &s->sc, &s->sc_h);
  if (st != 0) {
    dfree(s->y);
    if (s->y1) dfree(s->y1);
    if (s->res_raw) dfree(s->res_raw);
    if (s->res_raw1) dfree(s->res_raw1);
    if (s->scn) dfree(s->scn);
    delete s;
    return st;
  }
  *out = s;
  return 0;
}

int32_t rls_fista_destroy(rls_fista* s) {
  if (!s) return RLS_E_INVALID;
  if (rls_ctx_alive(s->actx, s->actx_id) && s->actx->server == &s->srv) rls_server_stop(s->actx);
  hipSetDevice(s->device);
  if (s->srv.ctl) hfree(s->srv.ctl);
  rls_alloc_scope alloc_scope(alloc_ctx_of(s->actx, s->actx_id));
  if (s->graph.exec) hipGraphExecDestroy(s->graph.exec);
  dfree(s->y);
  if (s->y1) dfree(s->y1);
  if (s->res_raw) dfree(s->res_raw);
  if (s->res_raw1) dfree(s->res_raw1);
  if (s->scn) dfree(s->scn);
  if (s->Ypack) dfree(s->Ypack);
  if (s->Tpack) dfree(s->Tpack);
  if (s->Vpart) dfree(s->Vpart);
  if (s->scb_h) hfree(s->scb_h);
  if (s->rsync) dfree(s->rsync);
  if (s->rsync_h) hfree(s->rsync_h);
  if (s->fk_yx) dfree(s->fk_yx);
  if (s->fk_xx) dfree(s->fk_xx);
  if (s->fk_dots) dfree(s->fk_dots);
  if (s->tv_in) dfree(s->tv_in);
  if (s->tv_out) dfree(s->tv_out);
  dfree(s->sc);
  hfree(s->sc_h);
  delete s;
  return 0;
}

static void fista_drop_graph(rls_fista* s) {
  if (s->graph.exec) hipGraphExecDestroy(s->graph.exec);
  s->graph = step_graph();
}

int32_t rls_fista_set_reg(rls_fista* s, int32_t reg_kind, float lambda, int64_t l21_slices, int32_t proj_kind) {
  if (!s) return RLS_E_INVALID;
  rls_ctx* ctx = s->op->ctx;
  if (reg_kind == RLS_REG_TV)
    return rls_fail(ctx, RLS_E_UNSUPPORTED, "fused FISTA: TV prox is not fused; drive FISTA from the primitives");
  if (reg_kind < RLS_REG_NONE || reg_kind > RLS_REG_L21 || proj_kind < RLS_PROJ_NONE || proj_kind > RLS_PROJ_POSITIVE)
    return rls_fail(ctx, RLS_E_INVALID, "fista_set_reg: unknown kind");
  if (reg_kind == RLS_REG_L21 && (l21_slices <= 0 || s->op->N / l21_slices == 0))
    return rls_fail(ctx, RLS_E_INVALID, "fista_set_reg: slices must be in 1..N");
  if (s->reg_kind == RLS_REG_TV || reg_kind != s->reg_kind) fista_drop_graph(s);
  s->reg_kind = reg_kind;
  s->proj_kind = proj_kind;
  s->lambda = lambda;
  s->l21_slices = l21_slices > 0 ? l21_slices : 1;
  return 0;
}

int32_t rls_fista_set_reg_tv(rls_fista* s, float lambda, int32_t ndims, const int64_t* shape, int32_t ntv, const int32_t* dims,
                             int32_t iterations_tv, int32_t proj_kind) {
  if (!s) return RLS_E_INVALID;
  rls_ctx* ctx = s->op->ctx;
  if (proj_kind < RLS_PROJ_NONE || proj_kind > RLS_PROJ_POSITIVE || iterations_tv < 0 || ndims < 1 || ndims > 4 || ntv < 0 || ntv > 4 ||
      !shape || (ntv > 0 && !dims))
    return rls_fail(ctx, RLS_E_INVALID, "fista_set_reg_tv: bad argument");
  int64_t n = 1;
  for (int k = 0; k < ndims; ++k) n *= shape[k];
  if (n != s->op->N) return rls_fail(ctx, RLS_E_INVALID, "fista_set_reg_tv: prod(shape) != N");
  if (s->nrhs != 1) return rls_fail(ctx, RLS_E_UNSUPPORTED, "fista_set_reg_tv: single right-hand side plans only");
  if (!rls_tv_single_ok(s->op->ctx, s->op->dtype, ndims, shape, ntv, dims))
    return rls_fail(ctx, RLS_E_UNSUPPORTED, "fista_set_reg_tv: the image does not fit the single-workgroup FGP kernel; drive FISTA from the primitives");
  RLS_HIP(ctx, rls_enter(ctx));
  if (!s->tv_in) {
// ... 1247 lines not shown
```

Before: 111,300 iterations/s.

## Add command-queue mode to persistent resident CGNR server kernel

```diff
diff --git a/regularizedleastsquares.jl_amd/csrc/api.hip b/regularizedleastsquares.jl_amd/csrc/api.hip
--- a/regularizedleastsquares.jl_amd/csrc/api.hip
+++ b/regularizedleastsquares.jl_amd/csrc/api.hip
@@ -245,6 +245,7 @@
   RLS_CHECK_CTX(ctx);
   RLS_HIP(ctx, rls_enter(ctx));
   RLS_HIP(ctx, rls_stream_wait(ctx->stream));
+  ++ctx->syncs;
   return 0;
 }
 
@@ -276,6 +277,7 @@
   else if (!strcmp(key, "small")) ctx->tune.small = value;
   else if (!strcmp(key, "resident_server")) ctx->tune.resident_server = value;
   else if (!strcmp(key, "resident_ahead")) ctx->tune.resident_ahead = value ? 1 : 0;
+  else if (!strcmp(key, "resident_queue")) ctx->tune.resident_queue = value ? 1 : 0;
   else if (!strcmp(key, "resident_l2_rows")) ctx->tune.resident_l2_rows = value;
   else if (!strcmp(key, "fista_defer")) ctx->tune.fista_defer = value;
   else if (!strcmp(key, "resident_server_idle_us")) {
@@ -377,6 +379,7 @@
   RLS_HIP(ctx, rls_enter(ctx));
   RLS_HIP(ctx, hipEventRecord(ctx->ev1, ctx->stream));
   RLS_HIP(ctx, rls_event_wait(ctx->ev1));
+  ++ctx->syncs;
   RLS_HIP(ctx, hipEventElapsedTime(ms_out, ctx->ev0, ctx->ev1));
   return 0;
 }
diff --git a/regularizedleastsquares.jl_amd/csrc/normal.hip b/regularizedleastsquares.jl_amd/csrc/normal.hip
--- a/regularizedleastsquares.jl_amd/csrc/normal.hip
+++ b/regularizedleastsquares.jl_amd/csrc/normal.hip
@@ -1952,6 +1952,33 @@
   }
 }
 
+template <typename E, int G, int K, int WV, bool FULL>
+__device__ static inline void owner_adjoint(const chunk<E, elem<E>::vec> (&a)[K], const E (&tr)[G * elem<E>::vec],
+                                            __amdgpu_buffer_rsrc_t slab_rs, int64_t N, bool l2rows) {
+  using C = slab_cfg<E, G, K, WV>;
+  constexpr int NV = C::NV, EPT = C::EPT, NT = C::NT;
+  const int tid = threadIdx.x;
+#pragma unroll
+  for (int q = 0; q < EPT / NV; ++q) {
+    chunk<E, NV> out;
+#pragma unroll
+    for (int j = 0; j < NV; ++j) {
+      E sum = elem<E>::zero();
+#pragma unroll
+      for (int i = 0; i < G; ++i)
+#pragma unroll
+        for (int r = 0; r < NV; ++r) sum = elem<E>::fmac_pk(a[16 * q + j * G + i].e[r], tr[i * NV + r], sum);
+      out.e[j] = sum;
+    }
+    const int o = q * NT * NV + tid * NV;
+    if (FULL || o < N) {
+      const uint32_t off = (uint32_t)blockIdx.x * (uint32_t)(N * sizeof(E)) + (uint32_t)(o * sizeof(E));
+      if (l2rows) __builtin_amdgcn_raw_buffer_store_b128(__builtin_bit_cast(u4, out), slab_rs, off, 0, 1);
+      else __builtin_amdgcn_raw_buffer_store_b128(__builtin_bit_cast(u4, out), slab_rs, off, 0, 16);
+    }
+  }
+}
+
 __device__ static inline unsigned resident_xcc_id() {
   unsigned v;
   asm volatile("s_getreg_b32 %0, hwreg(HW_REG_XCC_ID)" : "=s"(v));
@@ -2140,7 +2167,19 @@
   chunk<E, NV> a[K];
   slab_load<E, G, K, WV, FULL>(a, A, lda, Mc, N, pair);
   __builtin_amdgcn_sched_barrier(0);
-  if (!St.enabled && (S.done || n_steps <= 0)) return;
+  constexpr bool QOK = SPEC && FULL && owner_cfg<E, G, K, WV>::ok;
+  if constexpr (!QOK) {
+    if (!St.enabled && (S.done || n_steps <= 0)) return;
+  }
+  const bool queue = QOK && (St.srv_idle_us & RLS_SRV_QUEUE);
+  if constexpr (QOK) {
+    if (!queue && !St.enabled && (S.done || n_steps <= 0)) return;
+    if (queue && blockIdx.x == 0 && tid == 0) {
+      const unsigned long long t = wall_clock64();
+      sync->q_t0[0] = (unsigned)t;
+      sync->q_t0[1] = (unsigned)(t >> 32);
+    }
+  }
   constexpr bool OWN = owner_cfg<E, G, K, WV>::ok;
   if constexpr (OWN) owner_transpose<E, G, K, WV, FULL>(a, smem_raw, Mc, N, pair);
   STAMP(1);
@@ -2373,18 +2412,70 @@
   if (!St.srv_ctl) break;
   if constexpr (SPEC) {
     credit = 0;
-    if (!S.done) {
+    if (!S.done && !queue) {
       ahead = true;
       n_steps = 1;
       continue;
     }
   }
+  if constexpr (QOK) {
+  if (queue) {
+    const rls_q_cmd qc = resident_listen_q(St.srv_ctl, srv_seq, St.srv_idle_us & ~RLS_SRV_QUEUE, sync, epoch, (unsigned)nwg, spin_limit, &R.flag);
+    if (qc.cmd == RLS_SRV_EXIT) return;
+    n_steps = (int)(qc.cmd & RLS_Q_STEPS);
+    if (qc.cmd & RLS_Q_INIT) {
+      const E* bq = reinterpret_cast<const E*>((uintptr_t)qc.b_lo | ((uintptr_t)qc.b_hi << 32));
+      E tb[G * NV];
+      const int64_t rb = row_block_of(blockIdx.x, pair) * G;
+#pragma unroll
+      for (int i = 0; i < G; ++i) {
+        const chunk<E, NV> c = load_chunk<E, NV>(bq + (rb + i) * NV);
+#pragma unroll
+        for (int r = 0; r < NV; ++r) tb[i * NV + r] = c.e[r];
+      }
+      owner_adjoint<E, G, K, WV, FULL>(a, tb, slab_rs, N, l2rows);
+      asm volatile("s_waitcnt vmcnt(0)" ::: "memory");
+      __syncthreads();
+      if (!resident_allreduce<E, G, K, WV, BAR, FULL>(R, sync, slab_rs, v, nwg, N, epoch, xchg, spin_limit, rv, [](int, E) {}, []() {})) {
+        resident_give_up(sync, nullptr);
+        if (blockIdx.x == 0 && tid == 0) __hip_atomic_store(St.srv_ctl + 17, 2u, __ATOMIC_RELAXED, __HIP_MEMORY_SCOPE_SYSTEM);
+        return;
+      }
+      if (!placed) {
+        l2rows = resident_rows_at_l2(sync);
+        placed = true;
+      }
+      double rr = 0.0;
+#pragma unroll
+      for (int e = 0; e < EPT; ++e) {
+        pv[e] = rv[e];
+        xv[e] = elem<E>::zero();
+        rr += (double)elem<E>::re(rv[e]) * (double)elem<E>::re(rv[e]) + (double)elem<E>::im(rv[e]) * (double)elem<E>::im(rv[e]);
+      }
+      if (blockIdx.x == 0) store_owned(xw, xv);
+      rr = block_sum_n<NT / 64>(rr, L.red);
+      S.rr = rr;
+      S.z0 = sqrt(rr);
+      S.zeta = 0.0;
+      S.alpha_re = S.alpha_im = S.beta_re = S.beta_im = 0.0;
+      S.lambda = __builtin_bit_cast(float, qc.lambda);
+      S.rel_tol = __builtin_bit_cast(float, qc.reltol);
+      S.iteration = 0;
+      S.max_iter = (int)qc.maxiter;
+      S.pending = 0;
+      S.cur = 0;
+      S.fresh = 0;
+      const float ratio = (float)(sqrt(rr) / sqrt(rr));
+      S.done = (ratio <= S.rel_tol) || (0 >= S.max_iter);
+    }
+    continue;
+  }
+  }
   const unsigned cmd = resident_listen(St.srv_ctl, srv_seq, St.srv_idle_us, sync, epoch, (unsigned)nwg, spin_limit, &R.flag, srv_mb, srv_seq - St.srv_seq0 + 1u);
   if (cmd == RLS_SRV_EXIT) return;
   n_steps = (int)cmd;
   }
 }
-
 
 template <typename E, int K, int BAR, bool FULL, int SRV = 0>
 __global__ __launch_bounds__(512) void cgnr_gram_resident_kernel(const E* __restrict__ Gm, int64_t ldg, E* x, E* r, E* p,
@@ -3675,6 +3766,18 @@
     const int64_t Mc = P.M / C::NV;
     const int pair = resident_pairing(G, nwg);
     constexpr size_t lds = resident_lds_bytes<E, G, K, WV>();
+    if (St.srv_ctl && (St.srv_idle_us & RLS_SRV_QUEUE)) {
+      if constexpr (!owner_cfg<E, G, K, WV>::ok) {
+        return rls_fail(ctx, RLS_E_UNSUPPORTED, "resident CGNR: no queue mode for this shape");
+      } else {
+        if (!slab_full<E, G, K, WV>(P.M, P.N, nwg)) return rls_fail(ctx, RLS_E_UNSUPPORTED, "resident CGNR: no queue mode for a ragged shape");
+        return with_bool(resident_two_level_ok<E>(ctx->tune, nwg, P.N, C::NT), [&](auto TWO) {
+          return rls_launch<cgnr_resident_kernel<E, G, K, WV, TWO ? 2 : 1, true, true>>(
+              ctx, dim3(nwg), dim3(C::NT), lds, (const E*)P.A, P.lda, (E*)P.x, (E*)P.r1, (E*)P.r0, (E*)P.p0, (E*)P.v, (E*)P.slab,
+              dout, P.sc, (resident_sync*)sync, Mc, P.N, pair, n_steps, spin_limit, St);
+        });
+      }
+    }
     const bool spec = St.srv_ctl != nullptr && ctx->tune.resident_ahead != 0;
     return with_bool(resident_two_level_ok<E>(ctx->tune, nwg, P.N, C::NT), [&](auto TWO) {
       return with_bool(slab_full<E, G, K, WV>(P.M, P.N, nwg), [&](auto FULL) {
@@ -3995,6 +4098,22 @@
   return resident_typed<float2>(ctx, P, dout, sync, n_steps, spin_limit, St);
 }
 
+bool rls_cgnr_resident_queue_ok(const rls_ctx* ctx, int32_t dtype, int64_t M, int64_t N) {
+  auto ok = [&](auto tag) {
+    using E = decltype(tag);
+    if (M % elem<E>::vec) return false;
+    fused_cfg c;
+    if (!pick_cfg<E>(ctx->tune, N, &c)) return false;
+    return with_cfg(c, [&](auto S) {
+      return resident_shape<E, S.G, S.K, S.WV>() && owner_cfg<E, S.G, S.K, S.WV>::ok &&
+             slab_full<E, S.G, S.K, S.WV>(M, N, fused_nwg<E>(ctx->tune, M, N));
+    });
+  };
+  if (dtype == RLS_F32) return ok(float());
+  if (dtype == RLS_C32) return ok(float2());
+  return false;
+}
+
 int32_t rls_fista_resident_launch(rls_ctx* ctx, int32_t dtype, const rls_fista_pipe& P, void* sync, int n_steps,
                                   unsigned spin_limit, const rls_srv_args& Sv) {
   if (dtype == RLS_F32) return fista_resident_typed<float>(ctx, P, sync, n_steps, spin_limit, Sv);
diff --git a/regularizedleastsquares.jl_amd/csrc/resident_sync.hpp b/regularizedleastsquares.jl_amd/csrc/resident_sync.hpp
--- a/regularizedleastsquares.jl_amd/csrc/resident_sync.hpp
+++ b/regularizedleastsquares.jl_amd/csrc/resident_sync.hpp
@@ -37,7 +37,9 @@
   unsigned completed;
   unsigned failed;
   unsigned srv_n, srv_mb;
-  unsigned pad[27];
+  unsigned q_w[6];
+  unsigned q_t0[2];
+  unsigned pad[19];
 };
 static_assert(sizeof(resident_sync) == (2 * 8 * 32 + 32) * sizeof(unsigned), "resident_sync layout");
 constexpr int RES_GROUPS = 8;
@@ -151,3 +153,70 @@
   srv_seq += 1;
   return cmd;
 }
+
+struct rls_q_cmd {
+  unsigned cmd, maxiter, b_lo, b_hi, lambda, reltol;
+};
+__device__ static inline bool srv_read_slot(const unsigned* slot, unsigned seq, rls_q_cmd& c) {
+  typedef unsigned u4h __attribute__((ext_vector_type(4)));
+  u4h w0, w1, w2;
+  asm volatile("global_load_dwordx4 %0, %3, off sc0 sc1\n\tglobal_load_dwordx4 %1, %3, off offset:16 sc0 sc1\n\t"
+               "global_load_dwordx4 %2, %3, off offset:32 sc0 sc1\n\ts_waitcnt vmcnt(0)"
+               : "=&v"(w0), "=&v"(w1), "=&v"(w2) : "v"(slot) : "memory");
+  c = rls_q_cmd{w0.x, w0.z, w1.x, w1.z, w2.x, w2.z};
+  return w0.y == seq && w0.w == seq && w1.y == seq && w1.w == seq && w2.y == seq && w2.w == seq;
+}
+__device__ static inline rls_q_cmd resident_listen_q(unsigned* ctl, unsigned& srv_seq, unsigned idle_us, resident_sync* sync,
+                                                    unsigned& epoch, unsigned nwg, unsigned spin_limit, int* lds_flag) {
+  const int tid = threadIdx.x;
+  if (blockIdx.x == 0 && tid == 0) {
+    __hip_atomic_store(ctl + RLS_Q_DONE, srv_seq, __ATOMIC_RELAXED, __HIP_MEMORY_SCOPE_SYSTEM);
+    const unsigned long long t0 = wall_clock64(), idle = (unsigned long long)idle_us * 100ull;
+    const unsigned long long born = (unsigned long long)sync->q_t0[0] | ((unsigned long long)sync->q_t0[1] << 32);
+    const unsigned want = srv_seq + 1u;
+    const unsigned* slot = ctl + RLS_Q_RING_OFF + (want % RLS_Q_RING) * RLS_Q_SLOT_WORDS;
+    rls_q_cmd c{RLS_SRV_EXIT, 0u, 0u, 0u, 0u, 0u};
+    if (t0 - born > RLS_Q_LIFE_TICKS) {
+      __hip_atomic_store(ctl + 16, 1u, __ATOMIC_RELAXED, __HIP_MEMORY_SCOPE_SYSTEM);
+    } else {
+      for (;;) {
+        rls_q_cmd r;
+        if (srv_read_slot(slot, want, r)) {
+          c = r;
+          break;
+        }
+        if (wall_clock64() - t0 > idle) {
+          __hip_atomic_store(ctl + 16, 1u, __ATOMIC_RELAXED, __HIP_MEMORY_SCOPE_SYSTEM);
+          asm volatile("s_waitcnt vmcnt(0)" ::: "memory");
+          if (srv_read_slot(slot, want, r)) {
+            __hip_atomic_store(ctl + 16, 0u, __ATOMIC_RELAXED, __HIP_MEMORY_SCOPE_SYSTEM);
+            c = r;
+          }
+          break;
+        }
+        __builtin_amdgcn_s_sleep(8);
+      }
+    }
+    const unsigned w[6] = {c.cmd, c.maxiter, c.b_lo, c.b_hi, c.lambda, c.reltol};
+#pragma unroll
+    for (int i = 0; i < 6; ++i) __hip_atomic_store(&sync->q_w[i], w[i], __ATOMIC_RELAXED, __HIP_MEMORY_SCOPE_AGENT);
+    asm volatile("s_waitcnt vmcnt(0)" ::: "memory");
+  }
+  __syncthreads();
+  rls_q_cmd c{RLS_SRV_EXIT, 0u, 0u, 0u, 0u, 0u};
+  if (!grid_arrive_wait(sync->cnt, ++epoch, nwg, spin_limit, lds_flag)) {
+    resident_give_up(sync, nullptr);
+    if (blockIdx.x == 0 && tid == 0) __hip_atomic_store(ctl + 17, 2u, __ATOMIC_RELAXED, __HIP_MEMORY_SCOPE_SYSTEM);
+    return c;
+  }
+  unsigned w[6];
+#pragma unroll
+  for (int i = 0; i < 6; ++i) w[i] = __hip_atomic_load(&sync->q_w[i], __ATOMIC_RELAXED, __HIP_MEMORY_SCOPE_AGENT);
+  c = rls_q_cmd{w[0], w[1], w[2], w[3], w[4], w[5]};
+  if (c.cmd == RLS_SRV_EXIT) {
+    if (blockIdx.x == 0 && tid == 0) __hip_atomic_store(ctl + 17, 1u, __ATOMIC_RELAXED, __HIP_MEMORY_SCOPE_SYSTEM);
+    return c;
+  }
+  srv_seq += 1;
+  return c;
+}
diff --git a/regularizedleastsquares.jl_amd/csrc/rls_common.hpp b/regularizedleastsquares.jl_amd/csrc/rls_common.hpp
--- a/regularizedleastsquares.jl_amd/csrc/rls_common.hpp
+++ b/regularizedleastsquares.jl_amd/csrc/rls_common.hpp
@@ -29,6 +29,7 @@
   int resident_preclear = 1;
   int resident_server = 1;
   int resident_server_idle_us = 300;
+  int resident_queue = 1;
   int resident_ahead = 1;
   int fista_defer = 1;
   int resident_l2_rows = 1;
@@ -62,6 +63,7 @@
   float* res_d = nullptr;
   float* res_h = nullptr;
   rls_tuning tune;
+  uint64_t syncs = 0;
   uint64_t tune_epoch = 0;
   int cus = 0;
   int resident_failures = 0;
@@ -85,7 +87,16 @@
 };
 rls_mailbox_slot rls_mailbox_arm(rls_ctx* ctx, void* dst_pinned);
 constexpr unsigned RLS_SRV_EXIT = 0xffffffffu;
+constexpr unsigned RLS_SRV_QUEUE = 0x40000000u;
 constexpr unsigned RLS_SRV_AHEAD = 0x80000000u;
+constexpr unsigned RLS_Q_RING = 16;
+constexpr unsigned RLS_Q_SLOT_WORDS = 16;
+constexpr unsigned RLS_Q_RING_OFF = 64;
+constexpr unsigned RLS_Q_CTL_WORDS = RLS_Q_RING_OFF + RLS_Q_RING * RLS_Q_SLOT_WORDS;
+constexpr unsigned RLS_Q_DONE = 18;
+constexpr unsigned RLS_Q_INIT = 0x40000000u;
+constexpr unsigned RLS_Q_STEPS = 0x3fffffffu;
+constexpr unsigned long long RLS_Q_LIFE_TICKS = 2000000ull;
 struct rls_srv_args {
   unsigned* ctl = nullptr;
   unsigned seq0 = 0, idle_us = 0;
@@ -745,6 +756,7 @@
 
 int32_t rls_cgnr_resident_launch(rls_ctx* ctx, int32_t dtype, const rls_cgnr_pipe& P, double* dout, void* sync,
                                  int n_steps, unsigned spin_limit, const rls_cg_start& start = rls_cg_start());
+bool rls_cgnr_resident_queue_ok(const rls_ctx* ctx, int32_t dtype, int64_t M, int64_t N);
 
 struct pgm_state {
   int iteration, done;
diff --git a/regularizedleastsquares.jl_amd/csrc/solvers.hip b/regularizedleastsquares.jl_amd/csrc/solvers.hip
--- a/regularizedleastsquares.jl_amd/csrc/solvers.hip
+++ b/regularizedleastsquares.jl_amd/csrc/solvers.hip
@@ -110,6 +110,11 @@
   int served = 0, short_lives = 0;
   unsigned seq = 0;
   bool* resident_used = nullptr;
+  bool queue = false;
+  bool q_pending = false;
+  unsigned q_pay[5] = {};
+  unsigned q_last = 0;
+  void* q_plan = nullptr;
 };
 
 struct rls_cgnr {
@@ -157,6 +162,8 @@
   void* q_b = nullptr;
   void* q_bh = nullptr;
   void* q_xh = nullptr;
+  bool q_ok = false;
+  uint64_t q_mark = ~0ull;
 };
 
 static bool cgnr_use_gram_pipeline(const rls_cgnr* s) {
@@ -1947,9 +1954,14 @@
     e = resident_alloc(ctx, op, &s->rsync, &s->rsync_h);
     if (e == hipSuccess) e = dmalloc(&s->rdots, db);
     if (e == hipSuccess) e = hipMemsetAsync(s->rdots, 0, db, ctx->stream);
-    if (e == hipSuccess && !s->srv.ctl) e = hmalloc(&s->srv.ctl, 32 * sizeof(unsigned));
+    if (e == hipSuccess && !s->srv.ctl) {
+      e = hmalloc(&s->srv.ctl, RLS_Q_CTL_WORDS * sizeof(unsigned));
+      if (e == hipSuccess) memset(s->srv.ctl, 0, RLS_Q_CTL_WORDS * sizeof(unsigned));
+      s->q_ok = e == hipSuccess && rls_cgnr_resident_queue_ok(ctx, op->dtype, op->M, op->N);
+    }
     if (e == hipSuccess) memset(s->srv.ctl, 0, 32 * sizeof(unsigned));
     s->srv.resident_used = &s->resident_used;
+    s->srv.q_plan = s;
   }
   if (e == hipSuccess && nrhs == 1 && op->G && rls_gram_pipe_ok(op->dtype, op->N, op->G, op->ldg)) {
     const size_t vb = (size_t)op->N * rls_elem_size(op->dtype);
@@ -2080,7 +2092,16 @@
 
 static int32_t cgnr_group(rls_cgnr* const* plans, const void* const* b, int32_t count, float lambda, float rel_tol, int32_t iterations,
                           int32_t n_steps);
+extern "C++" {
+static bool cgnr_listening_q(const rls_cgnr* s);
+static int32_t cgnr_queue_init(rls_cgnr* s, const void* b, float lambda, float rel_tol, int32_t iterations);
+static int32_t cgnr_queue_step(rls_cgnr* s, int32_t n_steps);
+static bool cgnr_use_queue(const rls_cgnr* s);
+static int32_t cgnr_queue_launch(rls_cgnr* s, unsigned seq0, int32_t n_steps);
+}
 int32_t rls_cgnr_init(rls_cgnr* s, const void* b, float lambda, float rel_tol, int32_t iterations) {
+  if (s && b && s->nrhs == 1 && cgnr_listening_q(s) && (reinterpret_cast<uintptr_t>(b) & 15) == 0)
+    return cgnr_queue_init(s, b, lambda, rel_tol, iterations);
   if (s && b && s->nrhs == 1 && s->op->A && cgnr_use_small(s)) return cgnr_group(&s, &b, 1, lambda, rel_tol, iterations, 0);
   RLS_TRY(rls_cgnr_init_local_a(s, b, lambda, rel_tol, iterations));
   return rls_cgnr_init_local_b(s);
@@ -2264,15 +2285,24 @@
   return run_steps(ctx, &s->graph, n_steps, [s]() { return cgnr_enqueue_iteration(s); });
 }
 
-int32_t rls_cgnr_step(rls_cgnr* s, int32_t n_steps) {
+static int32_t cgnr_step_call(rls_cgnr* s, int32_t n_steps, bool queue) {
   if (!s) return RLS_E_INVALID;
   rls_ctx* ctx = s->op->ctx;
   if (!s->initialised) return rls_fail(ctx, RLS_E_STATE, "cgnr_step before cgnr_init");
   if (n_steps < 0) return rls_fail(ctx, RLS_E_INVALID, "cgnr_step: n_steps < 0");
+  if (queue && cgnr_listening_q(s) && (unsigned)n_steps <= RLS_Q_STEPS) {
+    const int32_t r = cgnr_queue_step(s, n_steps);
+    if (r <= 0) return r;
+  }
   RLS_HIP(ctx, rls_enter(ctx));
   s->requested += n_steps;
+  if (queue && n_steps > 1 && (unsigned)n_steps <= RLS_Q_STEPS && cgnr_use_resident(s)) {
+    if (s->resident_used && s->q_mark == ctx->syncs && cgnr_use_queue(s)) return cgnr_queue_launch(s, s->srv.seq + 1u, n_steps);
+    s->q_mark = ctx->syncs;
+  }
   return cgnr_step_impl(s, n_steps);
 }
+int32_t rls_cgnr_step(rls_cgnr* s, int32_t n_steps) { return cgnr_step_call(s, n_steps, true); }
 
 static int32_t cgnr_group(rls_cgnr* const* plans, const void* const* b, int32_t count, float lambda, float rel_tol, int32_t iterations,
                           int32_t n_steps) {
@@ -2633,9 +2663,11 @@
   if (ctx->server == v) ctx->server = nullptr;
 }
 
+static void cgnr_queue_stop(rls_ctx* ctx, srv_state* v);
 void rls_server_stop(rls_ctx* ctx) {
   srv_state* v = static_cast<srv_state*>(ctx->server);
   if (!v) return;
+  if (v->queue) return cgnr_queue_stop(ctx, v);
   if (v->alive) {
     volatile unsigned* ctl = v->ctl;
     if (!ctl[17]) {
@@ -2726,6 +2758,178 @@
   return 1;
 }
 
+static bool cgnr_use_queue(const rls_cgnr* s) {
+  const rls_ctx* ctx = s->op->ctx;
+  return s->q_ok && ctx->tune.resident_queue && ctx->tune.resident_server && !s->srv.off &&
+         (ctx->server == nullptr || ctx->server == &s->srv) && cgnr_use_resident(s);
+}
+static bool cgnr_listening_q(const rls_cgnr* s) {
+  const srv_state& v = s->srv;
+  return s->op->ctx->server == &v && v.alive && v.queue && s->op->ctx->tune.resident_queue;
+}
+static int32_t cgnr_queue_launch(rls_cgnr* s, unsigned seq0, int32_t n_steps) {
+  rls_ctx* ctx = s->op->ctx;
+  srv_state* v = &s->srv;
+  volatile unsigned* ctl = v->ctl;
+  ctl[16] = ctl[17] = 0;
+  if (n_steps > 0) {
+    ctl[RLS_Q_DONE] = seq0 - 1u;
+    v->seq = v->q_last = seq0;
+  }
+  rls_cg_start St;
+  St.srv_ctl = v->ctl;
+  St.srv_seq0 = seq0;
+  St.srv_idle_us = (unsigned)(ctx->tune.resident_server_idle_us > 0 ? ctx->tune.resident_server_idle_us : 1) | RLS_SRV_QUEUE;
+  const rls_cgnr_pipe P = cgnr_pipe_desc(s);
+  s->resident_used = true;
+  RLS_TRY(resident_chain(ctx, s->rsync, [&]() {
+    return rls_cgnr_resident_launch(ctx, s->op->dtype, P, s->rdots, s->rsync, n_steps, (unsigned)ctx->tune.resident_spin, St);
+  }, &s->rsync_clean));
+  v->alive = true;
+  v->queue = true;
+  v->served = (int)(v->q_last - seq0) + (n_steps > 0 ? 1 : 0);
+  ctx->server = v;
+  return 0;
+}
+static int32_t cgnr_queue_ordinary(rls_cgnr* s, unsigned cmd, const unsigned* pay) {
+  if (cmd & RLS_Q_INIT) {
+    const void* b = reinterpret_cast<const void*>((uintptr_t)pay[1] | ((uintptr_t)pay[2] << 32));
+    const long long req = s->requested;
+    const bool off = s->srv.off;
+    RLS_TRY(rls_cgnr_init_local_a(s, b, __builtin_bit_cast(float, pay[3]), __builtin_bit_cast(float, pay[4]), (int32_t)pay[0]));
+    RLS_TRY(rls_cgnr_init_local_b(s));
+    s->requested = req;
+    s->srv.off = off;
+  }
+  const int32_t n = (int32_t)(cmd & RLS_Q_STEPS);
+  return n > 0 ? cgnr_step_impl(s, n) : 0;
+}
+static int32_t cgnr_queue_resume(rls_cgnr* s) {
+  rls_ctx* ctx = s->op->ctx;
+  srv_state* v = &s->srv;
+  volatile unsigned* ctl = v->ctl;
+  const bool gave_up = ctl[17] == 2;
+  const unsigned done = ctl[RLS_Q_DONE];
+  server_life_over(ctx, v);
+  v->queue = false;
+  if (done == v->q_last) return 0;
+  if (!gave_up && cgnr_use_queue(s)) return cgnr_queue_launch(s, done, 0);
+  if (gave_up) s->resident_off = true;
+  for (unsigned q = done + 1u; q != v->q_last + 1u; ++q) {
+    const volatile unsigned* sl = v->ctl + RLS_Q_RING_OFF + (q % RLS_Q_RING) * RLS_Q_SLOT_WORDS;
+    const unsigned pay[5] = {sl[2], sl[4], sl[6], sl[8], sl[10]};
+    RLS_TRY(cgnr_queue_ordinary(s, sl[0], pay));
+  }
+  return 0;
+}
+static int32_t cgnr_queue_post(rls_cgnr* s, unsigned cmd, const unsigned (&pay)[5]) {
+  rls_ctx* ctx = s->op->ctx;
+  srv_state* v = &s->srv;
+  volatile unsigned* ctl = v->ctl;
+  const unsigned seq = v->seq + 1u;
+  auto t0 = std::chrono::steady_clock::now();
+  for (unsigned n = 0; seq - ctl[RLS_Q_DONE] > RLS_Q_RING; ++n) {
+    if (ctl[17]) {
+      RLS_TRY(cgnr_queue_resume(s));
+      if (!v->alive) return 1;
+      t0 = std::chrono::steady_clock::now();
+      continue;
+    }
+    rls_cpu_relax();
+    if ((n & 1023) == 1023 && std::chrono::steady_clock::now() - t0 > std::chrono::seconds(2)) {
+      (void)hipSetDevice(ctx->device);
+      (void)hipStreamSynchronize(ctx->stream);
+      if (!ctl[17]) ctl[17] = 2;
+    }
+  }
+  volatile unsigned long long* sl = reinterpret_cast<volatile unsigned long long*>(v->ctl + RLS_Q_RING_OFF + (seq % RLS_Q_RING) * RLS_Q_SLOT_WORDS);
+  const unsigned w[6] = {cmd, pay[0], pay[1], pay[2], pay[3], pay[4]};
+  for (int i = 0; i < 6; ++i) sl[i] = ((unsigned long long)seq << 32) | w[i];
+  v->seq = seq;
+  if (cmd != RLS_SRV_EXIT) v->q_last = seq;
+  v->served += 1;
+  std::atomic_thread_fence(std::memory_order_seq_cst);
+  t0 = std::chrono::steady_clock::now();
+  for (unsigned n = 0; ctl[16] || ctl[17]; ++n) {
+    if (ctl[17]) return cgnr_queue_resume(s);
+    rls_cpu_relax();
+    if ((n & 1023) == 1023 && std::chrono::steady_clock::now() - t0 > std::chrono::milliseconds(500)) {
+      (void)hipSetDevice(ctx->device);
+      (void)hipStreamSynchronize(ctx->stream);
+      if (!ctl[17]) ctl[17] = 2;
+    }
+  }
+  return 0;
+}
+static int32_t cgnr_queue_init(rls_cgnr* s, const void* b, float lambda, float rel_tol, int32_t iterations) {
+  srv_state* v = &s->srv;
+  if (v->q_pending) {
+    v->q_pending = false;
+    const int32_t r = cgnr_queue_post(s, RLS_Q_INIT, v->q_pay);
+    if (r < 0) return r;
+    if (r == 1) RLS_TRY(cgnr_queue_ordinary(s, RLS_Q_INIT, v->q_pay));
+    if (!cgnr_listening_q(s)) return rls_cgnr_init(s, b, lambda, rel_tol, iterations);
+  }
+  const int max_iter = cgnr_effective_iterations(s, iterations);
+  const uintptr_t bp = reinterpret_cast<uintptr_t>(b);
+  v->q_pay[0] = (unsigned)max_iter;
+  v->q_pay[1] = (unsigned)bp;
+  v->q_pay[2] = (unsigned)(bp >> 32);
+  v->q_pay[3] = __builtin_bit_cast(unsigned, lambda);
+  v->q_pay[4] = __builtin_bit_cast(unsigned, rel_tol);
+  v->q_pending = true;
+  s->sc_h->lambda = lambda;
+  s->sc_h->rel_tol = rel_tol;
+  s->sc_h->max_iter = max_iter;
+  s->initialised = true;
+  s->requested = 0;
+  return 0;
+}
+static int32_t cgnr_queue_step(rls_cgnr* s, int32_t n_steps) {
+  srv_state* v = &s->srv;
+  static const unsigned none[5] = {0u, 0u, 0u, 0u, 0u};
+  const bool init = v->q_pending;
+  if (!init && n_steps == 0) return 0;
+  unsigned pay[5];
+  for (int i = 0; i < 5; ++i) pay[i] = init ? v->q_pay[i] : none[i];
+  const unsigned cmd = (unsigned)n_steps | (init ? RLS_Q_INIT : 0u);
+  v->q_pending = false;
+  const long long req = s->requested;
+  s->requested += n_steps;
+  const int32_t r = cgnr_queue_post(s, cmd, pay);
+  if (r != 1) return r;
+  s->requested = req;
+  if (init) RLS_TRY(cgnr_queue_ordinary(s, RLS_Q_INIT, pay));
+  return 1;
+}
+static void cgnr_queue_stop(rls_ctx* ctx, srv_state* v) {
+  rls_cgnr* s = static_cast<rls_cgnr*>(v->q_plan);
+  static const unsigned none[5] = {0u, 0u, 0u, 0u, 0u};
+  if (v->q_pending) {
+    v->q_pending = false;
+    const unsigned pay[5] = {v->q_pay[0], v->q_pay[1], v->q_pay[2], v->q_pay[3], v->q_pay[4]};
+    const int32_t r = cgnr_queue_post(s, RLS_Q_INIT, pay);
+    if (r == 1) (void)cgnr_queue_ordinary(s, RLS_Q_INIT, pay);
+    if (r != 0) return;
+  }
+  if (!v->alive) return;
+  if (cgnr_queue_post(s, RLS_SRV_EXIT, none) != 0) return;
+  volatile unsigned* ctl = v->ctl;
+  for (int lives = 0; v->alive && v->queue && lives < 1024; ++lives) {
+    const auto t0 = std::chrono::steady_clock::now();
+    for (unsigned n = 0; !ctl[17]; ++n) {
+      rls_cpu_relax();
+      if ((n & 1023) == 1023 && std::chrono::steady_clock::now() - t0 > std::chrono::milliseconds(500)) {
+        (void)hipSetDevice(ctx->device);
+        (void)hipStreamSynchronize(ctx->stream);
+        if (!ctl[17]) ctl[17] = 2;
+      }
+    }
+    if (cgnr_queue_resume(s) != 0) break;
+  }
+  if (ctx->server == v) ctx->server = nullptr;
+}
+
 extern "C" int32_t rls_cgnr_step_status(rls_cgnr* s, int32_t n_steps, rls_cgnr_status* out);
 static int32_t cgnr_step_status_server(rls_cgnr* s, int32_t n_steps, rls_cgnr_status* out) {
   rls_ctx* ctx = s->op->ctx;
@@ -2779,13 +2983,14 @@
 int32_t rls_cgnr_step_status(rls_cgnr* s, int32_t n_steps, rls_cgnr_status* out) {
   if (!s || !out) return RLS_E_INVALID;
   rls_ctx* ctx = s->op->ctx;
+  if (cgnr_listening_q(s)) rls_server_stop(ctx);
   if (s->initialised && n_steps > 0 && n_steps <= 8 && !s->resident_used && cgnr_use_server(s)) return cgnr_step_status_server(s, n_steps, out);
   if (s->initialised && s->nrhs == 1 && n_steps > 0 && !s->resident_used) {
     RLS_HIP(ctx, rls_enter(ctx));
     s->mb_arm = rls_mailbox_arm(ctx, s->sc_h);
   }
   s->mb_sent = false;
-  const int32_t st = rls_cgnr_step(s, n_steps);
+  const int32_t st = cgnr_step_call(s, n_steps, false);
   const rls_mailbox_slot mb = s->mb_arm;
   s->mb_arm = rls_mailbox_slot();
   if (st != 0) return st;
```

After: 117,900 iterations/s, median of 6. +6.0%, better.
